# consensus-shipyard/ipc-filecoin-proofs

Measured on NVIDIA H100. Metric: receipts/sec scanned, higher is better.
Workload: dtype u8

## Files before the change

include/ipcfp.h:

```cpp
#ifndef IPCFP_H
#define IPCFP_H

#include <stdint.h>
#include <stddef.h>

#ifdef __cplusplus
extern "C" {
#endif

#define IPCFP_CID_LEN 38

typedef int32_t ipcfp_status;
enum {
    IPCFP_OK = 0,
    IPCFP_ERR_INVALID_ARG = -1,
    IPCFP_ERR_MISSING_BLOCK = -2,
    IPCFP_ERR_DECODE = -3,
    IPCFP_ERR_CID_MISMATCH = -4,
    IPCFP_ERR_MISSING_EXEC = -5,
    IPCFP_ERR_CUDA = -6,
    IPCFP_ERR_NCCL = -7,
    IPCFP_ERR_STATE_ROOT_MISMATCH = -8,
    IPCFP_ERR_ACTOR_NOT_FOUND = -9,
    IPCFP_ERR_NO_DEVICE = -10,
    IPCFP_ERR_UNSUPPORTED = -11
};

const char* ipcfp_last_error(void);
uint64_t ipcfp_last_error_index(void);
const char* ipcfp_version(void);
uint64_t ipcfp_kernel_launch_count(void);

ipcfp_status ipcfp_host_alloc(size_t bytes, void** out);
void ipcfp_host_free(void* p);

typedef struct ipcfp_store ipcfp_store;

#define IPCFP_STORE_VERIFY_CIDS 0x1u

ipcfp_status ipcfp_store_create(const uint8_t* cids, const uint64_t* offsets, const uint32_t* lengths,
                                const uint8_t* blob, uint64_t blob_size, uint64_t n_blocks,
                                int device, uint32_t flags, ipcfp_store** out);
void ipcfp_store_destroy(ipcfp_store* s);
uint64_t ipcfp_store_n_blocks(const ipcfp_store* s);
ipcfp_status ipcfp_store_get(ipcfp_store* s, const uint8_t cid[IPCFP_CID_LEN], uint8_t* buf, uint32_t cap,
                             uint32_t* len, int* found);
ipcfp_status ipcfp_store_has(ipcfp_store* s, const uint8_t cid[IPCFP_CID_LEN], int* found);
uint64_t ipcfp_store_first_bad_block(const ipcfp_store* s);

ipcfp_status ipcfp_blake2b256_batch(const uint8_t* blob, uint64_t blob_size, const uint64_t* offsets,
                                    const uint32_t* lengths, uint64_t n, int device, uint8_t* out );
ipcfp_status ipcfp_keccak256_batch(const uint8_t* blob, uint64_t blob_size, const uint64_t* offsets,
                                   const uint32_t* lengths, uint64_t n, int device, uint8_t* out );
ipcfp_status ipcfp_sha256_batch(const uint8_t* blob, uint64_t blob_size, const uint64_t* offsets,
                                const uint32_t* lengths, uint64_t n, int device, uint8_t* out );
ipcfp_status ipcfp_compute_mapping_slots(const uint8_t* keys32 , const uint64_t* slot_indices, uint64_t n,
                                         int device, uint8_t* out );

typedef struct ipcfp_tipset_desc {
    int64_t parent_epoch;
    int64_t child_epoch;
    uint32_t n_parents;
    const uint8_t* parent_cids;
    const uint8_t* parent_txmeta_cids;
    const uint8_t* child_cid;
    const uint8_t* receipts_root;
    const uint8_t* child_parent_state_root;
    uint64_t n_receipts;
    const uint8_t* events_roots;
    const uint8_t* has_events_root;
} ipcfp_tipset_desc;

typedef struct ipcfp_event_spec {
    const char* event_signature;
    const char* topic_1;
    uint8_t has_actor_id_filter;
    uint64_t actor_id_filter;
} ipcfp_event_spec;

#define IPCFP_LOG_FILTER_MAX_VALUES 65536u
#define IPCFP_LOG_FILTER_MAX_EMITTERS 65536u
typedef struct ipcfp_log_filter {
    uint64_t n_emitters;
    const uint64_t* emitters;
    uint32_t n_positions;
    uint32_t _pad;
    uint64_t n_values[4];
    const uint8_t* values[4];
} ipcfp_log_filter;

typedef struct ipcfp_storage_spec {
    uint64_t actor_id;
    uint8_t slot[32];
} ipcfp_storage_spec;

typedef struct ipcfp_witness {
    uint64_t n_blocks;
    const uint8_t* cids;
    const uint64_t* offsets;
    const uint32_t* lengths;
    const uint8_t* blob;
    uint64_t blob_size;
} ipcfp_witness;

typedef struct ipcfp_event_proof {
    uint64_t exec_index;
    uint64_t event_index;
    uint64_t emitter;
    uint32_t n_topics;
    uint32_t data_len;
    uint64_t data_off;
    uint64_t topics_off;
    uint8_t message_cid[IPCFP_CID_LEN];
    uint8_t _pad[2];
} ipcfp_event_proof;

typedef struct ipcfp_event_result {
    uint64_t n_matching;
    const uint64_t* matching_indices;
    uint64_t n_proofs;
    const ipcfp_event_proof* proofs;
    const uint8_t* data_blob;
    uint64_t data_blob_size;
    ipcfp_witness witness;
    uint64_t n_exec;
    float ms_total, ms_pass1, ms_pass2, ms_txamt, ms_witness;
    uint64_t pass1_bytes;
    uint64_t pass1_nodes;
    const void* shard_exec_dev;
    uint64_t shard_exec_count;
    uint64_t shard_raw_total;
    const void* union_cids_dev;
    uint64_t n_union_cids;
    const uint8_t* union_cids;
    uint64_t total_matching;
    uint64_t total_proofs;
    float ms_exchange, ms_fetch, ms_union;
    float _pad0;
    uint64_t union_part_first;
    uint64_t n_union_part;
    const char* json;
    uint64_t json_len;
    float ms_json;
    float _pad1;
} ipcfp_event_result;

typedef struct ipcfp_storage_proof {
    uint64_t actor_id;
    uint8_t actor_state_cid[IPCFP_CID_LEN];
    uint8_t storage_root[IPCFP_CID_LEN];
    uint8_t slot[32];
    uint8_t value[32];
    uint8_t found;
    uint8_t _pad[3];
    uint32_t raw_len;
} ipcfp_storage_proof;

typedef struct ipcfp_storage_result {
    uint64_t n_proofs;
    const ipcfp_storage_proof* proofs;
    ipcfp_witness witness;
    const uint64_t* spec_witness_offsets;
    const uint32_t* spec_witness_index;
    float ms_total;
} ipcfp_storage_result;

typedef struct ipcfp_slot_result {
    uint64_t n;
    const uint8_t* found;
    const uint32_t* raw_len;
    const uint8_t* values;
    ipcfp_witness witness;
    float ms_total;
    float ms_lookup;
    uint64_t lookup_nodes;
    uint64_t lookup_bytes;
} ipcfp_slot_result;

typedef struct ipcfp_bundle {
    ipcfp_storage_result* storage;
    uint64_t n_event_results;
    ipcfp_event_result** events;
    ipcfp_witness witness;
    const char* json;
// ... 191 lines not shown
```

integration/rust/ipcfp-sys/src/lib.rs:

```rust
#![allow(non_camel_case_types)]
use std::os::raw::{c_char, c_int, c_void};

pub const IPCFP_CID_LEN: usize = 38;
pub type ipcfp_status = i32;
pub const IPCFP_OK: ipcfp_status = 0;
pub const IPCFP_ERR_INVALID_ARG: ipcfp_status = -1;
pub const IPCFP_ERR_MISSING_BLOCK: ipcfp_status = -2;
pub const IPCFP_ERR_DECODE: ipcfp_status = -3;
pub const IPCFP_ERR_CID_MISMATCH: ipcfp_status = -4;
pub const IPCFP_ERR_MISSING_EXEC: ipcfp_status = -5;
pub const IPCFP_ERR_CUDA: ipcfp_status = -6;
pub const IPCFP_ERR_NCCL: ipcfp_status = -7;
pub const IPCFP_ERR_STATE_ROOT_MISMATCH: ipcfp_status = -8;
pub const IPCFP_ERR_ACTOR_NOT_FOUND: ipcfp_status = -9;
pub const IPCFP_ERR_NO_DEVICE: ipcfp_status = -10;
pub const IPCFP_ERR_UNSUPPORTED: ipcfp_status = -11;
pub const IPCFP_STORE_VERIFY_CIDS: u32 = 0x1;
pub const IPCFP_SCAN_SKIP_TX_AMTS: u32 = 0x1;
pub const IPCFP_SHARDED_UNION_TO_HOST: u32 = 0x2;
pub const IPCFP_SHARDED_UNION_FULL: u32 = 0x4;
pub const IPCFP_WITNESS_BY_REFERENCE: u32 = 0x8;
pub const IPCFP_RESULT_JSON: u32 = 0x10;
pub const IPCFP_COMM_ID_BYTES: usize = 128;

#[repr(C)] pub struct ipcfp_store { _p: [u8; 0] }
#[repr(C)] pub struct ipcfp_tipset { _p: [u8; 0] }
#[repr(C)] pub struct ipcfp_comm { _p: [u8; 0] }

#[repr(C)]
pub struct ipcfp_tipset_desc {
    pub parent_epoch: i64,
    pub child_epoch: i64,
    pub n_parents: u32,
    pub parent_cids: *const u8,
    pub parent_txmeta_cids: *const u8,
    pub child_cid: *const u8,
    pub receipts_root: *const u8,
    pub child_parent_state_root: *const u8,
    pub n_receipts: u64,
    pub events_roots: *const u8,
    pub has_events_root: *const u8,
}
#[repr(C)]
pub struct ipcfp_event_spec { pub event_signature: *const c_char, pub topic_1: *const c_char, pub has_actor_id_filter: u8, pub actor_id_filter: u64 }
pub const IPCFP_LOG_FILTER_MAX_VALUES: u32 = 65536;
pub const IPCFP_LOG_FILTER_MAX_EMITTERS: u32 = 65536;
#[repr(C)]
pub struct ipcfp_log_filter { pub n_emitters: u64, pub emitters: *const u64, pub n_positions: u32, pub _pad: u32, pub n_values: [u64; 4],
                              pub values: [*const u8; 4] }
#[repr(C)]
pub struct ipcfp_storage_spec { pub actor_id: u64, pub slot: [u8; 32] }
#[repr(C)]
pub struct ipcfp_witness { pub n_blocks: u64, pub cids: *const u8, pub offsets: *const u64, pub lengths: *const u32, pub blob: *const u8, pub blob_size: u64 }
#[repr(C)]
pub struct ipcfp_event_proof {
    pub exec_index: u64, pub event_index: u64, pub emitter: u64, pub n_topics: u32, pub data_len: u32,
    pub data_off: u64, pub topics_off: u64, pub message_cid: [u8; IPCFP_CID_LEN], pub _pad: [u8; 2],
}
#[repr(C)]
pub struct ipcfp_event_result {
    pub n_matching: u64, pub matching_indices: *const u64, pub n_proofs: u64, pub proofs: *const ipcfp_event_proof,
    pub data_blob: *const u8, pub data_blob_size: u64, pub witness: ipcfp_witness, pub n_exec: u64,
    pub ms_total: f32, pub ms_pass1: f32, pub ms_pass2: f32, pub ms_txamt: f32, pub ms_witness: f32,
    pub pass1_bytes: u64, pub pass1_nodes: u64,
    pub shard_exec_dev: *const c_void, pub shard_exec_count: u64, pub shard_raw_total: u64,
    pub union_cids_dev: *const c_void, pub n_union_cids: u64, pub union_cids: *const u8, pub total_matching: u64, pub total_proofs: u64,
    pub ms_exchange: f32, pub ms_fetch: f32, pub ms_union: f32, pub _pad0: f32,
    pub union_part_first: u64, pub n_union_part: u64,
    pub json: *const c_char, pub json_len: u64, pub ms_json: f32, pub _pad1: f32,
}
#[repr(C)]
pub struct ipcfp_storage_proof {
    pub actor_id: u64, pub actor_state_cid: [u8; IPCFP_CID_LEN], pub storage_root: [u8; IPCFP_CID_LEN],
    pub slot: [u8; 32], pub value: [u8; 32], pub found: u8, pub _pad: [u8; 3], pub raw_len: u32,
}
#[repr(C)]
pub struct ipcfp_storage_result {
    pub n_proofs: u64, pub proofs: *const ipcfp_storage_proof, pub witness: ipcfp_witness,
    pub spec_witness_offsets: *const u64, pub spec_witness_index: *const u32, pub ms_total: f32,
}
#[repr(C)]
pub struct ipcfp_slot_result { pub n: u64, pub found: *const u8, pub raw_len: *const u32, pub values: *const u8, pub witness: ipcfp_witness, pub ms_total: f32, pub ms_lookup: f32,
                                pub lookup_nodes: u64, pub lookup_bytes: u64 }
#[repr(C)]
pub struct ipcfp_parsed_bundle { pub tipset: ipcfp_tipset_desc, pub n_storage_proofs: u64, pub storage_proofs: *const ipcfp_storage_proof,
                                 pub n_event_proofs: u64, pub event_proofs: *const ipcfp_event_proof, pub data_blob: *const u8, pub data_blob_size: u64,
                                 pub witness: ipcfp_witness }
pub type ipcfp_trusted_parent_ts_fn = Option<unsafe extern "C" fn(ctx: *mut c_void, parent_epoch: i64, parent_cids: *const u8, n_parents: u32) -> c_int>;
pub type ipcfp_trusted_child_header_fn = Option<unsafe extern "C" fn(ctx: *mut c_void, child_epoch: i64, child_cid: *const u8) -> c_int>;
#[repr(C)]
pub struct ipcfp_bundle_verdict { pub tipset: ipcfp_tipset_desc, pub n_storage_proofs: u64, pub storage_proofs: *const ipcfp_storage_proof,
                                  pub storage_results: *const u8, pub n_event_proofs: u64, pub event_proofs: *const ipcfp_event_proof,
                                  pub event_results: *const u8, pub data_blob: *const u8, pub data_blob_size: u64, pub n_blocks: u64,
                                  pub witness_bytes: u64, pub parsed_on_device: u32, pub ms_total: f32, pub ms_parse: f32, pub ms_store: f32,
                                  pub ms_verify: f32, pub _pad: u32 }
#[repr(C)]
pub struct ipcfp_parsed_tipset { pub desc: ipcfp_tipset_desc }
#[repr(C)]
pub struct ipcfp_tipset_info { pub desc: ipcfp_tipset_desc, pub parsed_on_device: u32, pub ms_parse: f32, pub ms_kernels: f32,
                               pub _pad: u32 }
#[repr(C)]
pub struct ipcfp_parsed_blocks { pub blocks: ipcfp_witness }
#[repr(C)]
pub struct ipcfp_store_json_info { pub parsed_on_device: u32, pub ms_parse: f32, pub ms_kernels: f32, pub _pad: u32 }
#[repr(C)]
pub struct ipcfp_fetch_plan { pub n_missing: u64, pub cids: *const u8, pub n_needed: u64, pub n_levels: u32, pub ms_total: f32 }
pub const IPCFP_ADDRESS_MAX: usize = 65;
#[repr(C)]
#[derive(Clone, Copy)]
pub struct ipcfp_address { pub len: u8, pub bytes: [u8; IPCFP_ADDRESS_MAX] }
#[repr(C)]
pub struct ipcfp_resolve_result { pub n: u64, pub actor_ids: *const u64, pub status: *const ipcfp_status, pub init_status: ipcfp_status, pub _pad: u32,
                                  pub n_missing: u64, pub missing_cids: *const u8, pub witness: ipcfp_witness, pub ms_total: f32, pub ms_lookup: f32 }
#[repr(C)]
pub struct ipcfp_bundle { pub storage: *mut ipcfp_storage_result, pub n_event_results: u64, pub events: *mut *mut ipcfp_event_result, pub witness: ipcfp_witness,
                          pub json: *const c_char, pub json_len: u64, pub ms_total: f32, pub ms_json: f32 }

extern "C" {
    pub fn ipcfp_last_error() -> *const c_char;
    pub fn ipcfp_last_error_index() -> u64;
    pub fn ipcfp_version() -> *const c_char;
    pub fn ipcfp_kernel_launch_count() -> u64;
    pub fn ipcfp_host_alloc(bytes: usize, out: *mut *mut c_void) -> ipcfp_status;
    pub fn ipcfp_host_free(p: *mut c_void);

    pub fn ipcfp_store_create(cids: *const u8, offsets: *const u64, lengths: *const u32, blob: *const u8, blob_size: u64,
                              n_blocks: u64, device: c_int, flags: u32, out: *mut *mut ipcfp_store) -> ipcfp_status;
    pub fn ipcfp_store_destroy(s: *mut ipcfp_store);
    pub fn ipcfp_store_n_blocks(s: *const ipcfp_store) -> u64;
    pub fn ipcfp_store_get(s: *mut ipcfp_store, cid: *const u8, buf: *mut u8, cap: u32, len: *mut u32, found: *mut c_int) -> ipcfp_status;
    pub fn ipcfp_store_has(s: *mut ipcfp_store, cid: *const u8, found: *mut c_int) -> ipcfp_status;
    pub fn ipcfp_store_first_bad_block(s: *const ipcfp_store) -> u64;
    pub fn ipcfp_store_stream(s: *mut ipcfp_store) -> *mut c_void;

    pub fn ipcfp_blake2b256_batch(blob: *const u8, blob_size: u64, offsets: *const u64, lengths: *const u32, n: u64, device: c_int, out: *mut u8) -> ipcfp_status;
    pub fn ipcfp_keccak256_batch(blob: *const u8, blob_size: u64, offsets: *const u64, lengths: *const u32, n: u64, device: c_int, out: *mut u8) -> ipcfp_status;
    pub fn ipcfp_sha256_batch(blob: *const u8, blob_size: u64, offsets: *const u64, lengths: *const u32, n: u64, device: c_int, out: *mut u8) -> ipcfp_status;
    pub fn ipcfp_compute_mapping_slots(keys32: *const u8, slot_indices: *const u64, n: u64, device: c_int, out: *mut u8) -> ipcfp_status;

    pub fn ipcfp_generate_event_proof(s: *mut ipcfp_store, t: *const ipcfp_tipset_desc, spec: *const ipcfp_event_spec, flags: u32,
                                      out: *mut *mut ipcfp_event_result) -> ipcfp_status;
    pub fn ipcfp_event_result_free(r: *mut ipcfp_event_result);
    pub fn ipcfp_tipset_upload(s: *mut ipcfp_store, t: *const ipcfp_tipset_desc, out: *mut *mut ipcfp_tipset) -> ipcfp_status;
    pub fn ipcfp_tipset_free(t: *mut ipcfp_tipset);
    pub fn ipcfp_tipset_desc_from_json(parent: *const c_char, parent_len: u64, child: *const c_char, child_len: u64, receipts: *const c_char,
                                       receipts_len: u64, out: *mut *mut ipcfp_parsed_tipset) -> ipcfp_status;
    pub fn ipcfp_parsed_tipset_free(p: *mut ipcfp_parsed_tipset);
    pub fn ipcfp_tipset_upload_json(s: *mut ipcfp_store, parent: *const c_char, parent_len: u64, child: *const c_char, child_len: u64,
                                    receipts: *const c_char, receipts_len: u64, out: *mut *mut ipcfp_tipset) -> ipcfp_status;
    pub fn ipcfp_tipset_describe(t: *mut ipcfp_tipset, with_events_roots: c_int, out: *mut ipcfp_tipset_info) -> ipcfp_status;
    pub fn ipcfp_blocks_from_rpc_json(cids: *const u8, n_blocks: u64, texts: *const *const c_char, text_lens: *const u64, n_texts: u64,
                                      out: *mut *mut ipcfp_parsed_blocks) -> ipcfp_status;
    pub fn ipcfp_parsed_blocks_free(p: *mut ipcfp_parsed_blocks);
    pub fn ipcfp_store_create_rpc_json(cids: *const u8, n_blocks: u64, texts: *const *const c_char, text_lens: *const u64, n_texts: u64,
                                       device: c_int, flags: u32, out: *mut *mut ipcfp_store, info: *mut ipcfp_store_json_info) -> ipcfp_status;
    pub fn ipcfp_generate_event_proof_resident(s: *mut ipcfp_store, t: *mut ipcfp_tipset, spec: *const ipcfp_event_spec, flags: u32,
                                               out: *mut *mut ipcfp_event_result) -> ipcfp_status;
    pub fn ipcfp_generate_log_proof_resident(s: *mut ipcfp_store, t: *mut ipcfp_tipset, filter: *const ipcfp_log_filter, flags: u32,
                                             out: *mut *mut ipcfp_event_result) -> ipcfp_status;
    pub fn ipcfp_generate_log_proof(s: *mut ipcfp_store, t: *const ipcfp_tipset_desc, filter: *const ipcfp_log_filter, flags: u32,
                                    out: *mut *mut ipcfp_event_result) -> ipcfp_status;
    pub fn ipcfp_generate_event_proof_shard(s: *mut ipcfp_store, t: *const ipcfp_tipset_desc, spec: *const ipcfp_event_spec, lo: u64, hi: u64,
                                            world_size: u32, rank: u32, flags: u32, out: *mut *mut ipcfp_event_result) -> ipcfp_status;
    pub fn ipcfp_generate_event_proof_shard_resident(s: *mut ipcfp_store, t: *mut ipcfp_tipset, spec: *const ipcfp_event_spec, lo: u64, hi: u64,
                                                     world_size: u32, rank: u32, flags: u32, out: *mut *mut ipcfp_event_result) -> ipcfp_status;

    pub fn ipcfp_read_storage_slots(s: *mut ipcfp_store, contract_state_root: *const u8, slots: *const u8, k: u64, out: *mut *mut ipcfp_slot_result) -> ipcfp_status;
    pub fn ipcfp_slot_result_free(r: *mut ipcfp_slot_result);
    pub fn ipcfp_generate_storage_proofs(s: *mut ipcfp_store, t: *const ipcfp_tipset_desc, specs: *const ipcfp_storage_spec, n_specs: u64,
                                         out: *mut *mut ipcfp_storage_result) -> ipcfp_status;
    pub fn ipcfp_storage_result_free(r: *mut ipcfp_storage_result);
    pub fn ipcfp_generate_proof_bundle(s: *mut ipcfp_store, t: *const ipcfp_tipset_desc, sspecs: *const ipcfp_storage_spec, n_sspecs: u64,
                                       especs: *const ipcfp_event_spec, n_especs: u64, out: *mut *mut ipcfp_bundle) -> ipcfp_status;
    pub fn ipcfp_generate_proof_bundle_resident(s: *mut ipcfp_store, t: *mut ipcfp_tipset, sspecs: *const ipcfp_storage_spec, n_sspecs: u64,
                                                especs: *const ipcfp_event_spec, n_especs: u64, flags: u32, out: *mut *mut ipcfp_bundle) -> ipcfp_status;
    pub fn ipcfp_generate_log_bundle_resident(s: *mut ipcfp_store, t: *mut ipcfp_tipset, sspecs: *const ipcfp_storage_spec, n_sspecs: u64,
                                              filters: *const ipcfp_log_filter, n_filters: u64, flags: u32, out: *mut *mut ipcfp_bundle) -> ipcfp_status;
    pub fn ipcfp_generate_log_bundle(s: *mut ipcfp_store, t: *const ipcfp_tipset_desc, sspecs: *const ipcfp_storage_spec, n_sspecs: u64,
                                     filters: *const ipcfp_log_filter, n_filters: u64, flags: u32, out: *mut *mut ipcfp_bundle) -> ipcfp_status;
    pub fn ipcfp_bundle_free(b: *mut ipcfp_bundle);
    pub fn ipcfp_plan_fetch_resident(s: *mut ipcfp_store, t: *mut ipcfp_tipset, sspecs: *const ipcfp_storage_spec, n_sspecs: u64,
                                     especs: *const ipcfp_event_spec, n_especs: u64, flags: u32, out: *mut *mut ipcfp_fetch_plan) -> ipcfp_status;
    pub fn ipcfp_plan_fetch(s: *mut ipcfp_store, t: *const ipcfp_tipset_desc, sspecs: *const ipcfp_storage_spec, n_sspecs: u64,
                            especs: *const ipcfp_event_spec, n_especs: u64, flags: u32, out: *mut *mut ipcfp_fetch_plan) -> ipcfp_status;
    pub fn ipcfp_plan_fetch_log_resident(s: *mut ipcfp_store, t: *mut ipcfp_tipset, filter: *const ipcfp_log_filter, flags: u32,
                                         out: *mut *mut ipcfp_fetch_plan) -> ipcfp_status;
    pub fn ipcfp_plan_fetch_log_bundle_resident(s: *mut ipcfp_store, t: *mut ipcfp_tipset, sspecs: *const ipcfp_storage_spec, n_sspecs: u64,
                                                filters: *const ipcfp_log_filter, n_filters: u64, flags: u32, out: *mut *mut ipcfp_fetch_plan) -> ipcfp_status;
    pub fn ipcfp_fetch_plan_free(p: *mut ipcfp_fetch_plan);
    pub fn ipcfp_fetch_plan_to_rpc_json(p: *const ipcfp_fetch_plan, first_id: u64, out: *mut *mut c_char, out_len: *mut u64) -> ipcfp_status;
    pub fn ipcfp_resolve_addresses(s: *mut ipcfp_store, state_root: *const u8, addrs: *const ipcfp_address, n: u64,
                                   out: *mut *mut ipcfp_resolve_result) -> ipcfp_status;
    pub fn ipcfp_resolve_result_free(r: *mut ipcfp_resolve_result);
    pub fn ipcfp_address_parse(text: *const c_char, len: u64, out: *mut ipcfp_address) -> ipcfp_status;
    pub fn ipcfp_address_from_eth(eth: *const u8, out: *mut ipcfp_address) -> ipcfp_status;

    pub fn ipcfp_bundle_to_json(b: *const ipcfp_bundle, t: *const ipcfp_tipset_desc, out: *mut *mut c_char, out_len: *mut u64) -> ipcfp_status;
    pub fn ipcfp_event_result_to_json(r: *const ipcfp_event_result, t: *const ipcfp_tipset_desc, out: *mut *mut c_char, out_len: *mut u64) -> ipcfp_status;
    pub fn ipcfp_json_free(p: *mut c_char);
    pub fn ipcfp_bundle_from_json(json: *const c_char, len: u64, out: *mut *mut ipcfp_parsed_bundle) -> ipcfp_status;
    pub fn ipcfp_parsed_bundle_free(b: *mut ipcfp_parsed_bundle);
    pub fn ipcfp_verify_event_proofs(witness_store: *mut ipcfp_store, t: *const ipcfp_tipset_desc, proofs: *const ipcfp_event_proof, n_proofs: u64,
                                     data_blob: *const u8, data_blob_size: u64, filter: *const ipcfp_event_spec, results: *mut u8) -> ipcfp_status;
    pub fn ipcfp_verify_event_proofs_log(witness_store: *mut ipcfp_store, t: *const ipcfp_tipset_desc, proofs: *const ipcfp_event_proof, n_proofs: u64,
                                         data_blob: *const u8, data_blob_size: u64, filter: *const ipcfp_log_filter, results: *mut u8) -> ipcfp_status;
    pub fn ipcfp_verify_event_proofs_any(witness_store: *mut ipcfp_store, t: *const ipcfp_tipset_desc, proofs: *const ipcfp_event_proof, n_proofs: u64,
                                         data_blob: *const u8, data_blob_size: u64, filters: *const ipcfp_log_filter, n_filters: u64,
                                         results: *mut u8) -> ipcfp_status;
    pub fn ipcfp_verify_storage_proofs(witness_store: *mut ipcfp_store, t: *const ipcfp_tipset_desc, proofs: *const ipcfp_storage_proof, n_proofs: u64,
                                       results: *mut u8) -> ipcfp_status;
    pub fn ipcfp_verify_bundle_json(json: *const c_char, len: u64, device: c_int, trusted_parent: ipcfp_trusted_parent_ts_fn,
                                    trusted_child: ipcfp_trusted_child_header_fn, trust_ctx: *mut c_void, filter: *const ipcfp_event_spec,
                                    out: *mut *mut ipcfp_bundle_verdict) -> ipcfp_status;
    pub fn ipcfp_verify_bundle_json_any(json: *const c_char, len: u64, device: c_int, trusted_parent: ipcfp_trusted_parent_ts_fn,
                                        trusted_child: ipcfp_trusted_child_header_fn, trust_ctx: *mut c_void, filters: *const ipcfp_log_filter,
                                        n_filters: u64, out: *mut *mut ipcfp_bundle_verdict) -> ipcfp_status;
    pub fn ipcfp_bundle_verdict_free(v: *mut ipcfp_bundle_verdict);
    pub fn ipcfp_comm_unique_id(id: *mut u8) -> ipcfp_status;
    pub fn ipcfp_comm_init(id: *const u8, world_size: u32, rank: u32, device: c_int, out: *mut *mut ipcfp_comm) -> ipcfp_status;
    pub fn ipcfp_comm_destroy(c: *mut ipcfp_comm);
    pub fn ipcfp_generate_event_proof_sharded(c: *mut ipcfp_comm, s: *mut ipcfp_store, t: *mut ipcfp_tipset, spec: *const ipcfp_event_spec,
                                              bounds: *const u64, flags: u32, out: *mut *mut ipcfp_event_result) -> ipcfp_status;
}
```

ipc_filecoin_proofs_b200/api.py:

```python
import ctypes as C
import os
import subprocess
from dataclasses import dataclass
from typing import Optional

import numpy as np

from . import _abi as A

_HERE = os.path.dirname(os.path.abspath(__file__))
_ROOT = os.path.dirname(_HERE)
LIB_PATH = os.path.join(_HERE, "libipcfp.so")


def build_lib(force=False, jobs=8):
    if force or not os.path.exists(LIB_PATH):
        subprocess.check_call(["make", "-C", _ROOT, "-j%d" % jobs, os.path.relpath(LIB_PATH, _ROOT)])
    else:
        subprocess.check_call(["make", "-C", _ROOT, "-j%d" % jobs, "-s", os.path.relpath(LIB_PATH, _ROOT)])
    return LIB_PATH


_lib = None

EXPORTS = [
    "ipcfp_last_error", "ipcfp_last_error_index", "ipcfp_version", "ipcfp_kernel_launch_count", "ipcfp_host_alloc", "ipcfp_host_free",
    "ipcfp_store_create", "ipcfp_store_destroy", "ipcfp_store_n_blocks", "ipcfp_store_get", "ipcfp_store_has",
    "ipcfp_store_first_bad_block", "ipcfp_blake2b256_batch", "ipcfp_keccak256_batch", "ipcfp_sha256_batch",
    "ipcfp_compute_mapping_slots", "ipcfp_generate_event_proof", "ipcfp_event_result_free", "ipcfp_read_storage_slots",
    "ipcfp_slot_result_free", "ipcfp_generate_storage_proofs", "ipcfp_storage_result_free", "ipcfp_generate_proof_bundle",
    "ipcfp_bundle_free", "ipcfp_generate_event_proof_shard",
    "ipcfp_tipset_upload", "ipcfp_tipset_free", "ipcfp_generate_event_proof_resident", "ipcfp_generate_event_proof_shard_resident",
    "ipcfp_store_stream",
    "ipcfp_comm_unique_id", "ipcfp_comm_init", "ipcfp_comm_destroy", "ipcfp_generate_event_proof_sharded",
    "ipcfp_verify_event_proofs", "ipcfp_verify_storage_proofs", "ipcfp_bundle_to_json", "ipcfp_event_result_to_json", "ipcfp_json_free",
    "ipcfp_bundle_from_json", "ipcfp_parsed_bundle_free", "ipcfp_verify_bundle_json", "ipcfp_bundle_verdict_free",
    "ipcfp_generate_proof_bundle_resident", "ipcfp_tipset_desc_from_json", "ipcfp_parsed_tipset_free", "ipcfp_tipset_upload_json",
    "ipcfp_tipset_describe", "ipcfp_blocks_from_rpc_json", "ipcfp_parsed_blocks_free", "ipcfp_store_create_rpc_json",
    "ipcfp_plan_fetch_resident", "ipcfp_plan_fetch", "ipcfp_fetch_plan_free", "ipcfp_fetch_plan_to_rpc_json",
    "ipcfp_resolve_addresses", "ipcfp_resolve_result_free", "ipcfp_address_parse", "ipcfp_address_from_eth",
    "ipcfp_generate_log_proof", "ipcfp_generate_log_proof_resident", "ipcfp_plan_fetch_log_resident", "ipcfp_verify_event_proofs_log",
    "ipcfp_generate_log_bundle", "ipcfp_generate_log_bundle_resident", "ipcfp_plan_fetch_log_bundle_resident", "ipcfp_verify_event_proofs_any",
    "ipcfp_verify_bundle_json_any",
]


def lib():
    global _lib
    if _lib is None:
        if not os.path.exists(LIB_PATH):
            raise RuntimeError(f"{LIB_PATH} is missing: run `make` (or __graft_entry__.build()). There is no CPU fallback.")
        L = C.CDLL(LIB_PATH)
        L.ipcfp_last_error.restype = C.c_char_p
        L.ipcfp_last_error_index.restype = C.c_uint64
        L.ipcfp_version.restype = C.c_char_p
        L.ipcfp_kernel_launch_count.restype = C.c_uint64
        L.ipcfp_host_alloc.restype = C.c_int32
        L.ipcfp_host_alloc.argtypes = [C.c_size_t, C.POINTER(C.c_void_p)]
        L.ipcfp_host_free.argtypes = [C.c_void_p]
        L.ipcfp_store_create.restype = C.c_int32
        L.ipcfp_store_create.argtypes = [C.c_void_p, C.c_void_p, C.c_void_p, C.c_void_p, C.c_uint64, C.c_uint64, C.c_int, C.c_uint32,
                                         C.POINTER(C.c_void_p)]
        L.ipcfp_store_destroy.argtypes = [C.c_void_p]
        L.ipcfp_store_n_blocks.restype = C.c_uint64
        L.ipcfp_store_n_blocks.argtypes = [C.c_void_p]
        L.ipcfp_store_first_bad_block.restype = C.c_uint64
        L.ipcfp_store_first_bad_block.argtypes = [C.c_void_p]
        L.ipcfp_store_get.restype = C.c_int32
        L.ipcfp_store_get.argtypes = [C.c_void_p, C.c_void_p, C.c_void_p, C.c_uint32, C.POINTER(C.c_uint32), C.POINTER(C.c_int)]
        L.ipcfp_store_has.restype = C.c_int32
        L.ipcfp_store_has.argtypes = [C.c_void_p, C.c_void_p, C.POINTER(C.c_int)]
        for name in ("ipcfp_blake2b256_batch", "ipcfp_keccak256_batch", "ipcfp_sha256_batch"):
            f = getattr(L, name)
            f.restype = C.c_int32
            f.argtypes = [C.c_void_p, C.c_uint64, C.c_void_p, C.c_void_p, C.c_uint64, C.c_int, C.c_void_p]
        L.ipcfp_compute_mapping_slots.restype = C.c_int32
        L.ipcfp_compute_mapping_slots.argtypes = [C.c_void_p, C.c_void_p, C.c_uint64, C.c_int, C.c_void_p]
        L.ipcfp_generate_event_proof.restype = C.c_int32
        L.ipcfp_generate_event_proof.argtypes = [C.c_void_p, C.POINTER(A.TipsetDesc), C.POINTER(A.EventSpec), C.c_uint32,
                                                 C.POINTER(C.POINTER(A.EventResultC))]
        L.ipcfp_generate_event_proof_shard.restype = C.c_int32
        L.ipcfp_generate_event_proof_shard.argtypes = [C.c_void_p, C.POINTER(A.TipsetDesc), C.POINTER(A.EventSpec), C.c_uint64, C.c_uint64,
                                                       C.c_uint32, C.c_uint32, C.c_uint32, C.POINTER(C.POINTER(A.EventResultC))]
        L.ipcfp_event_result_free.argtypes = [C.POINTER(A.EventResultC)]
        L.ipcfp_read_storage_slots.restype = C.c_int32
        L.ipcfp_read_storage_slots.argtypes = [C.c_void_p, C.c_void_p, C.c_void_p, C.c_uint64, C.POINTER(C.POINTER(A.SlotResultC))]
        L.ipcfp_slot_result_free.argtypes = [C.POINTER(A.SlotResultC)]
        L.ipcfp_generate_storage_proofs.restype = C.c_int32
        L.ipcfp_generate_storage_proofs.argtypes = [C.c_void_p, C.POINTER(A.TipsetDesc), C.c_void_p, C.c_uint64,
                                                    C.POINTER(C.POINTER(A.StorageResultC))]
        L.ipcfp_storage_result_free.argtypes = [C.POINTER(A.StorageResultC)]
        L.ipcfp_generate_proof_bundle.restype = C.c_int32
        L.ipcfp_generate_proof_bundle.argtypes = [C.c_void_p, C.POINTER(A.TipsetDesc), C.c_void_p, C.c_uint64, C.c_void_p, C.c_uint64,
                                                  C.POINTER(C.POINTER(A.BundleC))]
        L.ipcfp_generate_proof_bundle_resident.restype = C.c_int32
        L.ipcfp_generate_proof_bundle_resident.argtypes = [C.c_void_p, C.c_void_p, C.c_void_p, C.c_uint64, C.c_void_p, C.c_uint64, C.c_uint32,
                                                           C.POINTER(C.POINTER(A.BundleC))]
        L.ipcfp_bundle_free.argtypes = [C.POINTER(A.BundleC)]
        L.ipcfp_tipset_upload.restype = C.c_int32
        L.ipcfp_tipset_upload.argtypes = [C.c_void_p, C.POINTER(A.TipsetDesc), C.POINTER(C.c_void_p)]
        L.ipcfp_tipset_free.argtypes = [C.c_void_p]
        L.ipcfp_generate_event_proof_resident.restype = C.c_int32
        L.ipcfp_generate_event_proof_resident.argtypes = [C.c_void_p, C.c_void_p, C.POINTER(A.EventSpec), C.c_uint32,
                                                          C.POINTER(C.POINTER(A.EventResultC))]
        L.ipcfp_generate_event_proof_shard_resident.restype = C.c_int32
        L.ipcfp_generate_event_proof_shard_resident.argtypes = [C.c_void_p, C.c_void_p, C.POINTER(A.EventSpec), C.c_uint64, C.c_uint64,
                                                                C.c_uint32, C.c_uint32, C.c_uint32, C.POINTER(C.POINTER(A.EventResultC))]
        L.ipcfp_store_stream.restype = C.c_void_p
        L.ipcfp_store_stream.argtypes = [C.c_void_p]
        L.ipcfp_comm_unique_id.restype = C.c_int32
        L.ipcfp_comm_unique_id.argtypes = [C.c_void_p]
        L.ipcfp_comm_init.restype = C.c_int32
        L.ipcfp_comm_init.argtypes = [C.c_void_p, C.c_uint32, C.c_uint32, C.c_int, C.POINTER(C.c_void_p)]
        L.ipcfp_comm_destroy.argtypes = [C.c_void_p]
        L.ipcfp_generate_event_proof_sharded.restype = C.c_int32
        L.ipcfp_generate_event_proof_sharded.argtypes = [C.c_void_p, C.c_void_p, C.c_void_p, C.POINTER(A.EventSpec), C.c_void_p, C.c_uint32,
                                                         C.POINTER(C.POINTER(A.EventResultC))]
        L.ipcfp_verify_event_proofs.restype = C.c_int32
        L.ipcfp_verify_event_proofs.argtypes = [C.c_void_p, C.POINTER(A.TipsetDesc), C.c_void_p, C.c_uint64, C.c_void_p, C.c_uint64, C.c_void_p, C.c_void_p]
        L.ipcfp_generate_log_proof.restype = C.c_int32
        L.ipcfp_generate_log_proof.argtypes = [C.c_void_p, C.POINTER(A.TipsetDesc), C.POINTER(A.LogFilterC), C.c_uint32,
                                               C.POINTER(C.POINTER(A.EventResultC))]
        L.ipcfp_generate_log_proof_resident.restype = C.c_int32
        L.ipcfp_generate_log_proof_resident.argtypes = [C.c_void_p, C.c_void_p, C.POINTER(A.LogFilterC), C.c_uint32,
                                                        C.POINTER(C.POINTER(A.EventResultC))]
        L.ipcfp_plan_fetch_log_resident.restype = C.c_int32
        L.ipcfp_plan_fetch_log_resident.argtypes = [C.c_void_p, C.c_void_p, C.POINTER(A.LogFilterC), C.c_uint32, C.POINTER(C.POINTER(A.FetchPlanC))]
        L.ipcfp_verify_event_proofs_log.restype = C.c_int32
        L.ipcfp_verify_event_proofs_log.argtypes = [C.c_void_p, C.POINTER(A.TipsetDesc), C.c_void_p, C.c_uint64, C.c_void_p, C.c_uint64,
                                                    C.POINTER(A.LogFilterC), C.c_void_p]
        L.ipcfp_generate_log_bundle.restype = C.c_int32
        L.ipcfp_generate_log_bundle.argtypes = [C.c_void_p, C.POINTER(A.TipsetDesc), C.c_void_p, C.c_uint64, C.POINTER(A.LogFilterC), C.c_uint64,
                                                C.c_uint32, C.POINTER(C.POINTER(A.BundleC))]
        L.ipcfp_generate_log_bundle_resident.restype = C.c_int32
        L.ipcfp_generate_log_bundle_resident.argtypes = [C.c_void_p, C.c_void_p, C.c_void_p, C.c_uint64, C.POINTER(A.LogFilterC), C.c_uint64,
                                                         C.c_uint32, C.POINTER(C.POINTER(A.BundleC))]
        L.ipcfp_plan_fetch_log_bundle_resident.restype = C.c_int32
        L.ipcfp_plan_fetch_log_bundle_resident.argtypes = [C.c_void_p, C.c_void_p, C.c_void_p, C.c_uint64, C.POINTER(A.LogFilterC), C.c_uint64,
                                                           C.c_uint32, C.POINTER(C.POINTER(A.FetchPlanC))]
        L.ipcfp_verify_event_proofs_any.restype = C.c_int32
        L.ipcfp_verify_event_proofs_any.argtypes = [C.c_void_p, C.POINTER(A.TipsetDesc), C.c_void_p, C.c_uint64, C.c_void_p, C.c_uint64,
                                                    C.POINTER(A.LogFilterC), C.c_uint64, C.c_void_p]
        L.ipcfp_verify_bundle_json_any.restype = C.c_int32
        L.ipcfp_verify_bundle_json_any.argtypes = [C.c_char_p, C.c_uint64, C.c_int, A.TrustedParentFn, A.TrustedChildFn, C.c_void_p,
                                                   C.POINTER(A.LogFilterC), C.c_uint64, C.POINTER(C.POINTER(A.BundleVerdictC))]
        L.ipcfp_verify_storage_proofs.restype = C.c_int32
        L.ipcfp_verify_storage_proofs.argtypes = [C.c_void_p, C.POINTER(A.TipsetDesc), C.c_void_p, C.c_uint64, C.c_void_p]
        for name in ("ipcfp_bundle_to_json", "ipcfp_event_result_to_json"):
            f = getattr(L, name)
            f.restype = C.c_int32
            f.argtypes = [C.c_void_p, C.POINTER(A.TipsetDesc), C.POINTER(C.c_void_p), C.POINTER(C.c_uint64)]
        L.ipcfp_json_free.argtypes = [C.c_void_p]
        L.ipcfp_bundle_from_json.restype = C.c_int32
        L.ipcfp_bundle_from_json.argtypes = [C.c_char_p, C.c_uint64, C.POINTER(C.POINTER(A.ParsedBundleC))]
        L.ipcfp_parsed_bundle_free.argtypes = [C.POINTER(A.ParsedBundleC)]
        L.ipcfp_verify_bundle_json.restype = C.c_int32
        L.ipcfp_verify_bundle_json.argtypes = [C.c_char_p, C.c_uint64, C.c_int, A.TrustedParentFn, A.TrustedChildFn, C.c_void_p, C.c_void_p,
                                               C.POINTER(C.POINTER(A.BundleVerdictC))]
        L.ipcfp_bundle_verdict_free.argtypes = [C.POINTER(A.BundleVerdictC)]
        L.ipcfp_tipset_desc_from_json.restype = C.c_int32
        L.ipcfp_tipset_desc_from_json.argtypes = [C.c_char_p, C.c_uint64, C.c_char_p, C.c_uint64, C.c_char_p, C.c_uint64,
                                                  C.POINTER(C.POINTER(A.ParsedTipsetC))]
        L.ipcfp_parsed_tipset_free.argtypes = [C.POINTER(A.ParsedTipsetC)]
        L.ipcfp_tipset_upload_json.restype = C.c_int32
        L.ipcfp_tipset_upload_json.argtypes = [C.c_void_p, C.c_char_p, C.c_uint64, C.c_char_p, C.c_uint64, C.c_char_p, C.c_uint64,
                                               C.POINTER(C.c_void_p)]
        L.ipcfp_tipset_describe.restype = C.c_int32
        L.ipcfp_tipset_describe.argtypes = [C.c_void_p, C.c_int, C.POINTER(A.TipsetInfoC)]
        L.ipcfp_blocks_from_rpc_json.restype = C.c_int32
        L.ipcfp_blocks_from_rpc_json.argtypes = [C.c_void_p, C.c_uint64, C.POINTER(C.c_char_p), C.POINTER(C.c_uint64), C.c_uint64,
                                                 C.POINTER(C.POINTER(A.ParsedBlocksC))]
        L.ipcfp_parsed_blocks_free.argtypes = [C.POINTER(A.ParsedBlocksC)]
        L.ipcfp_store_create_rpc_json.restype = C.c_int32
        L.ipcfp_store_create_rpc_json.argtypes = [C.c_void_p, C.c_uint64, C.POINTER(C.c_char_p), C.POINTER(C.c_uint64), C.c_uint64, C.c_int,
                                                  C.c_uint32, C.POINTER(C.c_void_p), C.POINTER(A.StoreJsonInfoC)]
        L.ipcfp_plan_fetch_resident.restype = C.c_int32
        L.ipcfp_plan_fetch_resident.argtypes = [C.c_void_p, C.c_void_p, C.c_void_p, C.c_uint64, C.c_void_p, C.c_uint64, C.c_uint32,
                                                C.POINTER(C.POINTER(A.FetchPlanC))]
        L.ipcfp_plan_fetch.restype = C.c_int32
        L.ipcfp_plan_fetch.argtypes = [C.c_void_p, C.POINTER(A.TipsetDesc), C.c_void_p, C.c_uint64, C.c_void_p, C.c_uint64, C.c_uint32,
                                       C.POINTER(C.POINTER(A.FetchPlanC))]
        L.ipcfp_fetch_plan_free.argtypes = [C.POINTER(A.FetchPlanC)]
        L.ipcfp_fetch_plan_to_rpc_json.restype = C.c_int32
        L.ipcfp_fetch_plan_to_rpc_json.argtypes = [C.POINTER(A.FetchPlanC), C.c_uint64, C.POINTER(C.c_void_p), C.POINTER(C.c_uint64)]
        L.ipcfp_resolve_addresses.restype = C.c_int32
        L.ipcfp_resolve_addresses.argtypes = [C.c_void_p, C.c_void_p, C.POINTER(A.AddressC), C.c_uint64, C.POINTER(C.POINTER(A.ResolveResultC))]
        L.ipcfp_resolve_result_free.argtypes = [C.POINTER(A.ResolveResultC)]
        L.ipcfp_address_parse.restype = C.c_int32
        L.ipcfp_address_parse.argtypes = [C.c_char_p, C.c_uint64, C.POINTER(A.AddressC)]
        L.ipcfp_address_from_eth.restype = C.c_int32
        L.ipcfp_address_from_eth.argtypes = [C.c_void_p, C.POINTER(A.AddressC)]
        _lib = L
    return _lib


def _u8(x):
    if isinstance(x, (bytes, bytearray, memoryview)):
        return np.frombuffer(bytes(x), dtype=np.uint8).copy()
    return np.ascontiguousarray(x, dtype=np.uint8)


def _check(st):
    if st != A.OK:
        L = lib()
        raise A.IpcfpError(st, L.ipcfp_last_error().decode(errors="replace"), L.ipcfp_last_error_index())


def kernel_launch_count():
    return int(lib().ipcfp_kernel_launch_count())


@dataclass
class EventProofSpec:
    event_signature: str
    topic_1: str
    actor_id_filter: Optional[int] = None

    def as_c(self):
        return A.make_event_spec(self.event_signature, self.topic_1, self.actor_id_filter)


def _topic32(v):
    if isinstance(v, str):
        v = bytes.fromhex(v[2:] if v[:2] in ("0x", "0X") else v)
    v = bytes(v)
    if len(v) != 32:
        raise ValueError(f"a topic value is 32 bytes, got {len(v)}")
    return v


class LogFilter:

    def __init__(self, emitters=None, topics=()):
        topics = list(topics)
        if len(topics) > 4:
            raise ValueError("a log filter has at most 4 topic positions")
        self.emitters = [int(e) for e in (emitters or [])]
        self.topics = []
        for t in topics:
            if t is None or (isinstance(t, (list, tuple)) and not t):
                self.topics.append(None)
            elif isinstance(t, (bytes, bytearray, str)):
                self.topics.append([_topic32(t)])
            else:
                self.topics.append([_topic32(v) for v in t])

    @classmethod
    def from_spec(cls, spec, device=0):
        t1 = spec.topic_1.encode()[:32]
        t0 = bytes(keccak256_batch([spec.event_signature.encode()], device)[0])
        return cls(None if spec.actor_id_filter is None else [spec.actor_id_filter], [t0, t1 + bytes(32 - len(t1))])

    def as_c(self):
        f = A.LogFilterC()
        keep = []
        em = np.ascontiguousarray(self.emitters, dtype=np.uint64)
        keep.append(em)
        f.n_emitters = len(em)
        f.emitters = em.ctypes.data if em.size else None
        f.n_positions = len(self.topics)
        for k, vals in enumerate(self.topics):
            if vals:
                a = np.frombuffer(b"".join(vals), dtype=np.uint8).copy()
                keep.append(a)
                f.n_values[k] = len(vals)
                f.values[k] = a.ctypes.data
        return f, keep

    def matches(self, emitter, topics):
        if self.emitters and emitter not in self.emitters:
            return False
        if len(topics) < len(self.topics):
            return False
        return all(vals is None or bytes(topics[k]) in vals for k, vals in enumerate(self.topics))


def _log_filters_c(log_filters):
    cs, keep = [], []
    for f in log_filters:
        c, k = f.as_c()
        cs.append(c)
        keep.append(k)
    return (A.LogFilterC * max(len(cs), 1))(*cs), len(cs), keep


@dataclass
class StorageProofSpec:
    actor_id: int
    slot: bytes


class PinnedArray:

    def __init__(self, nbytes):
        p = C.c_void_p()
        _check(lib().ipcfp_host_alloc(max(int(nbytes), 1), C.byref(p)))
        self._p = p
        self.array = np.frombuffer((C.c_uint8 * max(int(nbytes), 1)).from_address(p.value), dtype=np.uint8)[:int(nbytes)]

    def free(self):
        if self._p:
            self.array = None
            lib().ipcfp_host_free(self._p)
            self._p = None

    def __del__(self):
        try:
            self.free()
        except Exception:
            pass


class BlockStore:

    def __init__(self, cids, offsets, lengths, blob, device=0, verify_cids=False):
        cids = np.ascontiguousarray(cids, dtype=np.uint8)
        offsets = np.ascontiguousarray(offsets, dtype=np.uint64)
        lengths = np.ascontiguousarray(lengths, dtype=np.uint32)
        blob = np.ascontiguousarray(blob, dtype=np.uint8)
        self.n_blocks = len(lengths)
        self.device = device
        h = C.c_void_p()
        st = lib().ipcfp_store_create(cids.ctypes.data if cids.size else None, offsets.ctypes.data if offsets.size else None,
                                      lengths.ctypes.data if lengths.size else None, blob.ctypes.data if blob.size else None, blob.size,
                                      self.n_blocks, device, A.STORE_VERIFY_CIDS if verify_cids else 0, C.byref(h))
        self._h = h
        if st != A.OK:
            bad = lib().ipcfp_store_first_bad_block(h) if h else None
            msg, idx = lib().ipcfp_last_error().decode(errors="replace"), lib().ipcfp_last_error_index()
            if h:
                lib().ipcfp_store_destroy(h)
                self._h = None
            e = A.IpcfpError(st, msg, idx)
            e.first_bad_block = bad
            raise e

    @classmethod
    def from_tipset(cls, ts, device=0, verify_cids=False):
        return cls(ts.cids, ts.offsets, ts.lengths, ts.blob, device, verify_cids)

    @classmethod
    def from_rpc_json(cls, cids, texts, device=0, verify_cids=False):
        cids = np.ascontiguousarray(cids, dtype=np.uint8).reshape(-1, A.CID_LEN)
        arr, lens, keep = _text_array(texts)
        self = cls.__new__(cls)
        self.n_blocks, self.device, self._h = len(cids), device, None
        h, info = C.c_void_p(), A.StoreJsonInfoC()
        st = lib().ipcfp_store_create_rpc_json(cids.ctypes.data if cids.size else None, len(cids), arr, lens, len(keep), device,
                                               A.STORE_VERIFY_CIDS if verify_cids else 0, C.byref(h), C.byref(info))
        self._h = h
        self.json_info = A.StoreJsonInfoPy(bool(info.parsed_on_device), float(info.ms_parse), float(info.ms_kernels))
        if st != A.OK:
            bad = lib().ipcfp_store_first_bad_block(h) if h else None
            msg, idx = lib().ipcfp_last_error().decode(errors="replace"), lib().ipcfp_last_error_index()
            self.close()
            e = A.IpcfpError(st, msg, idx)
            e.first_bad_block = bad
            raise e
        return self

    def get(self, cid):
        cid = _u8(cid)
        ln = C.c_uint32()
        found = C.c_int()
# ... 565 lines not shown
```

ipc_filecoin_proofs_b200/csrc/capi.cu:

```cuda
#include <atomic>
#include <cstring>

#include "engine.cuh"
#include "log_filter.cuh"

namespace ipcfp {

static thread_local std::string g_last_error;
static thread_local uint64_t g_last_index = UINT64_MAX;
static std::atomic<uint64_t> g_launches{0};

void note_launch() { g_launches.fetch_add(1, std::memory_order_relaxed); }
void set_last_error(const std::string& msg, uint64_t index) { g_last_error = msg; g_last_index = index; }

template <class F> static ipcfp_status guard(F f) {
    g_last_error.clear();
    g_last_index = UINT64_MAX;
    try { f(); return IPCFP_OK; }
    catch (const Error& e) { g_last_error = e.msg; g_last_index = e.index; return e.status; }
    catch (const std::bad_alloc&) { g_last_error = "out of host memory"; return IPCFP_ERR_INVALID_ARG; }
    catch (const std::exception& e) { g_last_error = e.what(); return IPCFP_ERR_INVALID_ARG; }
}

struct BundleBox {
    ipcfp_bundle r;
    std::vector<ipcfp_event_result*> ev;
    WitnessOut wit;
    PinnedArray json;
    ~BundleBox() {
        if (r.storage) storage_result_free(r.storage);
        for (auto* e : ev) event_result_free(e);
    }
};
struct TimingEvent {
    cudaEvent_t e = nullptr;
    TimingEvent() { IPCFP_CUDA(cudaEventCreate(&e)); }
    ~TimingEvent() { if (e) cudaEventDestroy(e); }
};

struct FetchPlanBox {
    ipcfp_fetch_plan r;
    FetchPlan plan;
    void fill() {
        r.n_missing = plan.cids.size() / 38;
        r.cids = plan.cids.data();
        r.n_needed = plan.n_needed;
        r.n_levels = plan.n_levels;
        r.ms_total = plan.ms_total;
    }
};

#define IPCFP_BUNDLE_FLAGS (IPCFP_WITNESS_BY_REFERENCE | IPCFP_RESULT_JSON)

template <class Check, class Gen>
static ipcfp_bundle* generate_proof_bundle(Store* st, TipsetDev& td, const ipcfp_storage_spec* sspecs, uint64_t n_sspecs, uint64_t n_events,
                                           uint32_t flags, Check check, Gen gen) {
    if (flags & ~(uint32_t)IPCFP_BUNDLE_FLAGS) throw Error(IPCFP_ERR_INVALID_ARG, "unknown flag bit for a proof bundle");
    if (n_sspecs && !sspecs) throw Error(IPCFP_ERR_INVALID_ARG, "null specs");
    check();
    if ((flags & IPCFP_WITNESS_BY_REFERENCE) && !st->caller_blob)
        throw Error(IPCFP_ERR_UNSUPPORTED, "IPCFP_WITNESS_BY_REFERENCE needs a store made from a caller's blob (ipcfp_store_create)");
    st->use();
    const bool by_ref = (flags & IPCFP_WITNESS_BY_REFERENCE) != 0;
    cudaStream_t stream = st->stream;
    TimingEvent t0, t1, j0, j1;
    IPCFP_CUDA(cudaEventRecord(t0.e, stream));
    std::unique_ptr<BundleBox> box(new BundleBox());
    memset(&box->r, 0, sizeof box->r);
    std::vector<const WitnessOut*> lists;
    if (n_sspecs) {
        if (!td.has_state_root) throw Error(IPCFP_ERR_INVALID_ARG, "tipset descriptor lacks child_cid / parent_state_root");
        box->r.storage = generate_storage_proofs(st, td.child_cid, td.child_state_root, sspecs, n_sspecs, by_ref);
        lists.push_back(&storage_result_witness(box->r.storage));
    }
    for (uint64_t i = 0; i < n_events; i++) {
        box->ev.push_back(gen(i));
        lists.push_back(&event_result_witness(box->ev.back()));
    }
    witness_union(st, lists, box->wit, by_ref);

    if (flags & IPCFP_RESULT_JSON) {
        IPCFP_CUDA(cudaEventRecord(j0.e, stream));
        const uint64_t ns = box->r.storage ? box->r.storage->n_proofs : 0;
        uint64_t np = 0, nb = 0;
        for (auto* e : box->ev) { np += e->n_proofs; nb += e->data_blob_size; }
        auto up16 = [](uint64_t x) { return (x + 15) & ~15ull; };
        const uint64_t o_ev = up16(ns * sizeof(ipcfp_storage_proof)), o_blob = o_ev + up16(np * sizeof(ipcfp_event_proof)),
                       o_cids = o_blob + up16(nb + 16), size = o_cids + 38ull * (2 + td.n_parents);
        PinnedArray stage(st->pool, size);
        uint8_t* h = stage.as<uint8_t>();
        if (ns) memcpy(h, box->r.storage->proofs, ns * sizeof(ipcfp_storage_proof));
        ipcfp_event_proof* hp = (ipcfp_event_proof*)(h + o_ev);
        uint64_t k = 0, base = 0;
        for (auto* e : box->ev) {
            for (uint64_t q = 0; q < e->n_proofs; q++, k++) {
                hp[k] = e->proofs[q];
                hp[k].data_off += base;
                hp[k].topics_off += base;
            }
            if (e->data_blob_size) memcpy(h + o_blob + base, e->data_blob, e->data_blob_size);
            base += e->data_blob_size;
        }
        memcpy(h + o_cids, td.child_cid, 38);
        memcpy(h + o_cids + 38, td.child_state_root, 38);
        if (td.n_parents) memcpy(h + o_cids + 76, td.parent_cids.data(), 38ull * td.n_parents);
        AsyncBuf<uint8_t> d(size, stream);
        IPCFP_CUDA(cudaMemcpyAsync(d.p, h, size, cudaMemcpyHostToDevice, stream));
        UnifiedJsonInputs ji{(const ipcfp_storage_proof*)d.p, ns, (const ipcfp_event_proof*)(d.p + o_ev), np, d.p + o_blob,
                             box->wit.cids_dev.p, box->wit.idx_dev.p, box->wit.n, td.parent_epoch, td.child_epoch, td.n_parents,
                             d.p + o_cids + 76, d.p + o_cids, d.p + o_cids + 38};
        box->r.json_len = render_unified_json(st, ji, box->json);
        IPCFP_CUDA(cudaEventRecord(j1.e, stream));
    }
    IPCFP_CUDA(cudaEventRecord(t1.e, stream));
    IPCFP_CUDA(cudaStreamSynchronize(stream));
    box->r.n_event_results = box->ev.size();
    box->r.events = box->ev.data();
    box->wit.fill(box->r.witness);
    float ms;
    IPCFP_CUDA(cudaEventElapsedTime(&ms, t0.e, t1.e)); box->r.ms_total = ms;
    if (flags & IPCFP_RESULT_JSON) {
        box->r.json = box->json.as<char>();
        IPCFP_CUDA(cudaEventElapsedTime(&ms, j0.e, j1.e)); box->r.ms_json = ms;
    }
    return &box.release()->r;
}

static ipcfp_bundle* generate_proof_bundle(Store* st, TipsetDev& td, const ipcfp_storage_spec* sspecs, uint64_t n_sspecs,
                                           const ipcfp_event_spec* especs, uint64_t n_especs, uint32_t flags) {
    return generate_proof_bundle(
        st, td, sspecs, n_sspecs, n_especs, flags,
        [&] { if (n_especs && !especs) throw Error(IPCFP_ERR_INVALID_ARG, "null specs"); },
        [&](uint64_t i) { return generate_event_proof(st, td, &especs[i], flags & IPCFP_WITNESS_BY_REFERENCE, false, 0, 0); });
}
static ipcfp_bundle* generate_log_bundle(Store* st, TipsetDev& td, const ipcfp_storage_spec* sspecs, uint64_t n_sspecs,
                                         const ipcfp_log_filter* filters, uint64_t n_filters, uint32_t flags) {
    return generate_proof_bundle(
        st, td, sspecs, n_sspecs, n_filters, flags, [&] { LogFilterSet::check(filters, n_filters); },
        [&](uint64_t k) { return generate_log_proof(st, td, &filters[k], flags & IPCFP_WITNESS_BY_REFERENCE); });
}

}

using namespace ipcfp;

struct ipcfp_store { Store s; };

extern "C" {

const char* ipcfp_last_error(void) { return g_last_error.c_str(); }
uint64_t ipcfp_last_error_index(void) { return g_last_index; }
const char* ipcfp_version(void) {
    return "ipcfp-b200 0.2 (sm_90a): k_verify_cids k_hash_batch k_build_index sort_by_cid k_pass1_stage k_pass2 k_amt_dense k_amt_expand k_dedup "
           "k_storage_proofs k_read_slots k_verify_events k_verify_storage k_scan k_witness_copy k_witness_emit k_union_mark k_json_* k_jp_* k_rj_* k_rb_* | sharded: k_xb_* k_exec_claim_seg "
           "k_exec_mark_dups k_select_positions k_fetch_positions k_part_pack k_merge_* (NCCL via dlopen)";
}
uint64_t ipcfp_kernel_launch_count(void) { return g_launches.load(); }

ipcfp_status ipcfp_host_alloc(size_t bytes, void** out) {
    return guard([&] {
        if (!out) throw Error(IPCFP_ERR_INVALID_ARG, "null out");
        int cnt = 0;
        if (cudaGetDeviceCount(&cnt) != cudaSuccess || cnt == 0) { cudaGetLastError(); throw Error(IPCFP_ERR_NO_DEVICE, "no CUDA device"); }
        int dev = 0;
        if (cudaGetDevice(&dev) != cudaSuccess) { cudaGetLastError(); dev = 0; }
        NumaPrefer numa(dev);
        IPCFP_CUDA(cudaMallocHost(out, bytes ? bytes : 1));
    });
}
void ipcfp_host_free(void* p) { if (p) cudaFreeHost(p); }

ipcfp_status ipcfp_store_create(const uint8_t* cids, const uint64_t* offsets, const uint32_t* lengths, const uint8_t* blob, uint64_t blob_size,
                                uint64_t n_blocks, int device, uint32_t flags, ipcfp_store** out) {
    return guard([&] {
        if (!out) throw Error(IPCFP_ERR_INVALID_ARG, "null out");
        *out = nullptr;
        Store* s = store_create(cids, offsets, lengths, blob, blob_size, n_blocks, device, flags);
        *out = reinterpret_cast<ipcfp_store*>(s);
        if (s->first_bad != UINT64_MAX) throw Error(IPCFP_ERR_CID_MISMATCH, "blake2b-256(block) != CID digest", s->first_bad);
    });
}
ipcfp_status ipcfp_store_create_rpc_json(const uint8_t* cids, uint64_t n_blocks, const char* const* texts, const uint64_t* text_lens, uint64_t n_texts,
                                         int device, uint32_t flags, ipcfp_store** out, ipcfp_store_json_info* info) {
    return guard([&] {
        if (!out) throw Error(IPCFP_ERR_INVALID_ARG, "null out");
        *out = nullptr;
        ipcfp_store_json_info si;
        Store* s = store_create_rpc_json(cids, n_blocks, texts, text_lens, n_texts, device, flags, si);
        *out = reinterpret_cast<ipcfp_store*>(s);
        if (info) *info = si;
        if (s->first_bad != UINT64_MAX) throw Error(IPCFP_ERR_CID_MISMATCH, "blake2b-256(block) != CID digest", s->first_bad);
    });
}
void ipcfp_store_destroy(ipcfp_store* s) { delete reinterpret_cast<Store*>(s); }
uint64_t ipcfp_store_n_blocks(const ipcfp_store* s) { return s ? reinterpret_cast<const Store*>(s)->n : 0; }
uint64_t ipcfp_store_first_bad_block(const ipcfp_store* s) { return s ? reinterpret_cast<const Store*>(s)->first_bad : UINT64_MAX; }
ipcfp_status ipcfp_store_get(ipcfp_store* s, const uint8_t cid[IPCFP_CID_LEN], uint8_t* buf, uint32_t cap, uint32_t* len, int* found) {
    return guard([&] {
        if (!s || !cid || !found) throw Error(IPCFP_ERR_INVALID_ARG, "null argument");
        store_get(reinterpret_cast<Store*>(s), cid, buf, cap, len, found);
    });
}
ipcfp_status ipcfp_store_has(ipcfp_store* s, const uint8_t cid[IPCFP_CID_LEN], int* found) {
    return guard([&] {
        if (!s || !cid || !found) throw Error(IPCFP_ERR_INVALID_ARG, "null argument");
        uint32_t len;
        store_get(reinterpret_cast<Store*>(s), cid, nullptr, 0, &len, found);
    });
}

ipcfp_status ipcfp_blake2b256_batch(const uint8_t* blob, uint64_t blob_size, const uint64_t* offsets, const uint32_t* lengths, uint64_t n, int device,
                                    uint8_t* out) {
    return guard([&] { hash_batch(0, blob, blob_size, offsets, lengths, n, device, out); });
}
ipcfp_status ipcfp_keccak256_batch(const uint8_t* blob, uint64_t blob_size, const uint64_t* offsets, const uint32_t* lengths, uint64_t n, int device,
                                   uint8_t* out) {
    return guard([&] { hash_batch(1, blob, blob_size, offsets, lengths, n, device, out); });
}
ipcfp_status ipcfp_sha256_batch(const uint8_t* blob, uint64_t blob_size, const uint64_t* offsets, const uint32_t* lengths, uint64_t n, int device,
                                uint8_t* out) {
    return guard([&] { hash_batch(2, blob, blob_size, offsets, lengths, n, device, out); });
}
ipcfp_status ipcfp_compute_mapping_slots(const uint8_t* keys32, const uint64_t* slot_indices, uint64_t n, int device, uint8_t* out) {
    return guard([&] { mapping_slots(keys32, slot_indices, n, device, out); });
}

ipcfp_status ipcfp_generate_event_proof(ipcfp_store* s, const ipcfp_tipset_desc* t, const ipcfp_event_spec* spec, uint32_t flags,
                                        ipcfp_event_result** out) {
    return guard([&] {
        if (!s || !out) throw Error(IPCFP_ERR_INVALID_ARG, "null argument");
        *out = nullptr;
        Store* st = reinterpret_cast<Store*>(s);
        TipsetDev td;
        tipset_upload(st, t, td);
        *out = generate_event_proof(st, td, spec, flags, false, 0, 0);
    });
}
ipcfp_status ipcfp_generate_event_proof_shard(ipcfp_store* s, const ipcfp_tipset_desc* t, const ipcfp_event_spec* spec, uint64_t lo, uint64_t hi,
                                              uint32_t world_size, uint32_t rank, uint32_t flags, ipcfp_event_result** out) {
    return guard([&] {
        if (!s || !out) throw Error(IPCFP_ERR_INVALID_ARG, "null argument");
        *out = nullptr;
        Store* st = reinterpret_cast<Store*>(s);
        TipsetDev td;
        tipset_upload(st, t, td);
        *out = generate_event_proof(st, td, spec, flags, true, lo, hi);
    });
}
void ipcfp_event_result_free(ipcfp_event_result* r) { if (r) event_result_free(r); }

ipcfp_status ipcfp_tipset_upload(ipcfp_store* s, const ipcfp_tipset_desc* t, ipcfp_tipset** out) {
    return guard([&] {
        if (!s || !out) throw Error(IPCFP_ERR_INVALID_ARG, "null argument");
        *out = nullptr;
        Store* st = reinterpret_cast<Store*>(s);
        std::unique_ptr<TipsetDev> td(new TipsetDev());
        tipset_upload(st, t, *td);
        IPCFP_CUDA(cudaStreamSynchronize(st->stream));
        *out = reinterpret_cast<ipcfp_tipset*>(td.release());
    });
}
void ipcfp_tipset_free(ipcfp_tipset* t) { delete reinterpret_cast<TipsetDev*>(t); }
ipcfp_status ipcfp_tipset_upload_json(ipcfp_store* s, const char* parent, uint64_t parent_len, const char* child, uint64_t child_len,
                                      const char* receipts, uint64_t receipts_len, ipcfp_tipset** out) {
    return guard([&] {
        if (!s || !out) throw Error(IPCFP_ERR_INVALID_ARG, "null argument");
        *out = nullptr;
        Store* st = reinterpret_cast<Store*>(s);
        std::unique_ptr<TipsetDev> td(new TipsetDev());
        tipset_upload_json(st, parent, parent_len, child, child_len, receipts, receipts_len, *td);
        IPCFP_CUDA(cudaStreamSynchronize(st->stream));
        *out = reinterpret_cast<ipcfp_tipset*>(td.release());
    });
}
ipcfp_status ipcfp_tipset_describe(ipcfp_tipset* t, int with_events_roots, ipcfp_tipset_info* out) {
    return guard([&] {
        if (!t || !out) throw Error(IPCFP_ERR_INVALID_ARG, "null argument");
        tipset_describe(*reinterpret_cast<TipsetDev*>(t), with_events_roots != 0, out);
    });
}
ipcfp_status ipcfp_generate_event_proof_resident(ipcfp_store* s, ipcfp_tipset* t, const ipcfp_event_spec* spec, uint32_t flags,
                                                 ipcfp_event_result** out) {
    return guard([&] {
        if (!s || !t || !out) throw Error(IPCFP_ERR_INVALID_ARG, "null argument");
        *out = nullptr;
        *out = generate_event_proof(reinterpret_cast<Store*>(s), *reinterpret_cast<TipsetDev*>(t), spec, flags, false, 0, 0);
    });
}
ipcfp_status ipcfp_generate_event_proof_shard_resident(ipcfp_store* s, ipcfp_tipset* t, const ipcfp_event_spec* spec, uint64_t lo, uint64_t hi,
                                                       uint32_t world_size, uint32_t rank, uint32_t flags, ipcfp_event_result** out) {
    return guard([&] {
        if (!s || !t || !out) throw Error(IPCFP_ERR_INVALID_ARG, "null argument");
        *out = nullptr;
        *out = generate_event_proof(reinterpret_cast<Store*>(s), *reinterpret_cast<TipsetDev*>(t), spec, flags, true, lo, hi);
    });
}
ipcfp_status ipcfp_generate_log_proof_resident(ipcfp_store* s, ipcfp_tipset* t, const ipcfp_log_filter* filter, uint32_t flags,
                                               ipcfp_event_result** out) {
    return guard([&] {
        if (!s || !t || !out) throw Error(IPCFP_ERR_INVALID_ARG, "null argument");
        *out = nullptr;
        *out = generate_log_proof(reinterpret_cast<Store*>(s), *reinterpret_cast<TipsetDev*>(t), filter, flags);
    });
}
ipcfp_status ipcfp_generate_log_proof(ipcfp_store* s, const ipcfp_tipset_desc* t, const ipcfp_log_filter* filter, uint32_t flags,
                                      ipcfp_event_result** out) {
    return guard([&] {
        if (!s || !out) throw Error(IPCFP_ERR_INVALID_ARG, "null argument");
        *out = nullptr;
        Store* st = reinterpret_cast<Store*>(s);
// ... 243 lines not shown
```

ipc_filecoin_proofs_b200/csrc/common.cuh:

```cuda
#pragma once
#include <cuda_runtime.h>
#include <stdint.h>
#include <string>
#include <vector>

#include "../../include/ipcfp.h"

namespace ipcfp {

struct Error {
    ipcfp_status status;
    std::string msg;
    uint64_t index;
    Error(ipcfp_status s, std::string m, uint64_t i = UINT64_MAX) : status(s), msg(std::move(m)), index(i) {}
};
void note_launch();

#define IPCFP_CUDA(expr)                                                                                          \
    do {                                                                                                          \
        cudaError_t _e = (expr);                                                                                  \
        if (_e != cudaSuccess)                                                                                    \
            throw ::ipcfp::Error(IPCFP_ERR_CUDA, std::string(#expr) + ": " + cudaGetErrorString(_e));             \
    } while (0)

#define IPCFP_LAUNCH_CHECK()                                                   \
    do {                                                                       \
        ::ipcfp::note_launch();                                                \
        IPCFP_CUDA(cudaGetLastError());                                        \
    } while (0)

static inline unsigned div_up(uint64_t a, uint64_t b) { return (unsigned)((a + b - 1) / b); }

void* dev_pool_take(size_t bytes, size_t* cap_out);
void dev_pool_give(void* p, size_t cap);

template <class T> struct DevBuf {
    T* p = nullptr;
    size_t n = 0;
    size_t pool_cap = 0;
    DevBuf() {}
    explicit DevBuf(size_t count) { alloc(count); }
    DevBuf(const DevBuf&) = delete;
    DevBuf& operator=(const DevBuf&) = delete;
    DevBuf(DevBuf&& o) noexcept : p(o.p), n(o.n), pool_cap(o.pool_cap) { o.p = nullptr; o.n = 0; o.pool_cap = 0; }
    DevBuf& operator=(DevBuf&& o) noexcept { if (this != &o) { release(); p = o.p; n = o.n; pool_cap = o.pool_cap; o.p = nullptr; o.n = 0; o.pool_cap = 0; } return *this; }
    ~DevBuf() { release(); }
    void alloc(size_t count) {
        release();
        n = count;
        if (count) IPCFP_CUDA(cudaMalloc((void**)&p, count * sizeof(T)));
    }
    void alloc_pooled(size_t count) {
        release();
        n = count;
        if (count) p = (T*)dev_pool_take(count * sizeof(T), &pool_cap);
    }
    void ensure(size_t count) { if (count > n) alloc(count); }
    void release() {
        if (p) { if (pool_cap) dev_pool_give(p, pool_cap); else cudaFree(p); }
        p = nullptr; n = 0; pool_cap = 0;
    }
    size_t bytes() const { return n * sizeof(T); }
};

template <class T> struct AsyncBuf {
    T* p = nullptr;
    size_t n = 0;
    cudaStream_t st = nullptr;
    AsyncBuf() {}
    AsyncBuf(size_t count, cudaStream_t s) { alloc(count, s); }
    AsyncBuf(const AsyncBuf&) = delete;
    AsyncBuf& operator=(const AsyncBuf&) = delete;
    AsyncBuf(AsyncBuf&& o) noexcept : p(o.p), n(o.n), st(o.st) { o.p = nullptr; o.n = 0; }
    AsyncBuf& operator=(AsyncBuf&& o) noexcept { if (this != &o) { release(); p = o.p; n = o.n; st = o.st; o.p = nullptr; o.n = 0; } return *this; }
    ~AsyncBuf() { release(); }
    void alloc(size_t count, cudaStream_t s) {
        release();
        st = s;
        n = count;
        if (count) IPCFP_CUDA(cudaMallocAsync((void**)&p, count * sizeof(T), s));
    }
    void release() { if (p) cudaFreeAsync(p, st); p = nullptr; n = 0; }
    void zero() { if (p) IPCFP_CUDA(cudaMemsetAsync(p, 0, n * sizeof(T), st)); }
};

template <class T> struct PinnedBuf {
    T* p = nullptr;
    T* dev = nullptr;
    size_t n = 0;
    PinnedBuf() {}
    explicit PinnedBuf(size_t count) { alloc(count); }
    PinnedBuf(const PinnedBuf&) = delete;
    PinnedBuf& operator=(const PinnedBuf&) = delete;
    ~PinnedBuf() { if (p) cudaFreeHost(p); }
    void alloc(size_t count) {
        if (p) cudaFreeHost(p);
        p = nullptr; dev = nullptr; n = count;
        if (count) {
            IPCFP_CUDA(cudaHostAlloc((void**)&p, count * sizeof(T), cudaHostAllocMapped));
            IPCFP_CUDA(cudaHostGetDevicePointer((void**)&dev, p, 0));
        }
    }
    void ensure(size_t count) { if (count > n) alloc(count); }
    void swap(PinnedBuf& o) { std::swap(p, o.p); std::swap(dev, o.dev); std::swap(n, o.n); }
};

enum Stage : uint32_t {
    ST_TXMETA = 1, ST_TXAMT = 2, ST_RECEIPTS_ROOT = 3, ST_PASS1 = 4, ST_PASS2 = 5, ST_WITNESS = 6,
    ST_STORAGE = 7, ST_INGEST = 8
};
enum DevCode : uint32_t { DC_MISSING = 1, DC_DECODE = 2, DC_MISSING_EXEC = 3, DC_STATE_MISMATCH = 4, DC_ACTOR_NOT_FOUND = 5, DC_UNSUPPORTED = 6, DC_CID_MISMATCH = 7 };

#define IPCFP_NO_ERROR 0xFFFFFFFFFFFFFFFFull

__host__ __device__ static inline uint64_t err_key(uint32_t stage, uint64_t index, uint32_t code, uint32_t detail) {
    return ((uint64_t)stage << 56) | ((index & 0xFFFFFFFFFFull) << 16) | ((uint64_t)(code & 0xff) << 8) | (detail & 0xff);
}
#define IPCFP_TX_EIDX_NONE 0xffu
__host__ __device__ static inline uint64_t tx_err_key(uint32_t eidx, uint64_t base, uint32_t level, uint32_t code, uint32_t detail) {
    const uint64_t b = base > 0xFFFFFFFFFFFull ? 0xFFFFFFFFFFFull : base;
    return ((uint64_t)(eidx & 0xff) << 56) | (b << 12) | ((uint64_t)(31u - (level > 31u ? 31u : level)) << 7) | ((uint64_t)(code & 7) << 4) | (detail & 15);
}
#ifdef __CUDACC__
__device__ static inline void report_error(unsigned long long* word, uint32_t stage, uint64_t index, uint32_t code, uint32_t detail) {
    atomicMin(word, (unsigned long long)err_key(stage, index, code, detail));
}
__device__ static inline void report_tx_error(unsigned long long* word, uint32_t eidx, uint64_t base, uint32_t level, uint32_t code, uint32_t detail) {
    atomicMin(word, (unsigned long long)tx_err_key(eidx, base, level, code, detail));
}
#endif

struct Digest { uint64_t w[4]; };

#ifdef __CUDACC__
__device__ __forceinline__ bool digest_eq(const Digest& a, const Digest& b) {
    return a.w[0] == b.w[0] && a.w[1] == b.w[1] && a.w[2] == b.w[2] && a.w[3] == b.w[3];
}
__device__ __forceinline__ uint64_t mix64(uint64_t x) {
    x ^= x >> 33; x *= 0xff51afd7ed558ccdULL; x ^= x >> 33; x *= 0xc4ceb9fe1a85ec53ULL; x ^= x >> 33;
    return x;
}
__device__ __forceinline__ uint64_t digest_hash(const Digest& d, uint32_t cls) { return mix64(d.w[0] ^ (d.w[2] * 0x9E3779B97F4A7C15ULL) ^ cls); }
__device__ __forceinline__ uint64_t load_u64_le(const uint8_t* p) {
    uint64_t v = 0;
#pragma unroll
    for (int i = 0; i < 8; i++) v |= (uint64_t)p[i] << (8 * i);
    return v;
}
__device__ __forceinline__ uint64_t load_u64_any(const uint8_t* q) {
    uintptr_t a = (uintptr_t)q;
    const uint64_t* b = (const uint64_t*)(a & ~(uintptr_t)7);
    uint32_t s = (uint32_t)(a & 7) * 8;
    uint64_t x0 = b[0], x1 = b[1];
    return (x0 >> s) | ((x1 << 1) << (63 - s));
}
__device__ __forceinline__ void win_load(const uint8_t* q, uint64_t& w0, uint64_t& w1) {
    uintptr_t a = (uintptr_t)q;
    const uint2* b = (const uint2*)(a & ~(uintptr_t)7);
    uint32_t s = (uint32_t)(a & 7) * 8;
    uint2 x0 = b[0], x1 = b[1], x2 = b[2];
    bool up = (s & 32) != 0;
    uint32_t c0 = up ? x0.y : x0.x, c1 = up ? x1.x : x0.y, c2 = up ? x1.y : x1.x, c3 = up ? x2.x : x1.y, c4 = up ? x2.y : x2.x;
    w0 = (uint64_t)__funnelshift_r(c0, c1, s) | ((uint64_t)__funnelshift_r(c1, c2, s) << 32);
    w1 = (uint64_t)__funnelshift_r(c2, c3, s) | ((uint64_t)__funnelshift_r(c3, c4, s) << 32);
}
__device__ __forceinline__ Digest load_digest(const uint8_t* p) {
    uintptr_t a = (uintptr_t)p;
    const uint64_t* b = (const uint64_t*)(a & ~(uintptr_t)7);
    uint32_t s = (uint32_t)(a & 7) * 8;
    uint64_t x0 = b[0], x1 = b[1], x2 = b[2], x3 = b[3], x4 = b[4];
    Digest d;
    d.w[0] = (x0 >> s) | ((x1 << 1) << (63 - s)); d.w[1] = (x1 >> s) | ((x2 << 1) << (63 - s));
    d.w[2] = (x2 >> s) | ((x3 << 1) << (63 - s)); d.w[3] = (x3 >> s) | ((x4 << 1) << (63 - s));
    return d;
}
__device__ __forceinline__ void prefetch_l2(const void* p) { asm volatile("prefetch.global.L2 [%0];" ::"l"(p)); }
#endif

}
```

ipc_filecoin_proofs_b200/csrc/engine.cuh:

```cuda
#pragma once
#include <array>
#include <memory>
#include <mutex>
#include <string>
#include <vector>

#include "common.cuh"
#include "store.cuh"
#include "rawcid.cuh"

namespace ipcfp {

struct NumaPrefer {
    bool on = false;
    int old_mode = 0;
    unsigned long old_mask[16] = {};
    explicit NumaPrefer(int device);
    ~NumaPrefer();
};

struct PinnedPool {
    struct Buf { void* p; size_t cap; };
    std::mutex mu;
    std::vector<Buf> free_list;
    ~PinnedPool();
    void* take(size_t bytes, size_t* cap_out);
    void give(void* p, size_t cap);
};
struct PinnedArray {
    std::shared_ptr<PinnedPool> pool;
    void* p = nullptr;
    size_t cap = 0;
    PinnedArray() {}
    PinnedArray(std::shared_ptr<PinnedPool> pl, size_t bytes) : pool(std::move(pl)) { p = pool->take(bytes ? bytes : 16, &cap); }
    PinnedArray(const PinnedArray&) = delete;
    PinnedArray& operator=(const PinnedArray&) = delete;
    PinnedArray(PinnedArray&& o) noexcept : pool(std::move(o.pool)), p(o.p), cap(o.cap) { o.p = nullptr; }
    PinnedArray& operator=(PinnedArray&& o) noexcept { release(); pool = std::move(o.pool); p = o.p; cap = o.cap; o.p = nullptr; return *this; }
    ~PinnedArray() { release(); }
    void release() { if (p && pool) pool->give(p, cap); p = nullptr; }
    template <class T> T* as() const { return (T*)p; }
};

enum DevWord : uint32_t {
    DW_ERR = 0,
    DW_FRONTIER_A = 1, DW_FRONTIER_B = 2,
    DW_UNKNOWN_CLASSES = 1,
    DW_FIRST_BAD = 2,
    DW_N_EXEC = 3,
    DW_STATS = 4,
    DW_N_MATCH = 6,
    DW_N_PROOFS = 7,
    DW_WIT_A = 8, DW_WIT_A_BYTES = 9,
    DW_WIT_B = 10, DW_WIT_B_BYTES = 11,
    DW_BLOB_BYTES = 12,
    DW_LEVEL_TOTAL = 13,
    DW_DENSE_FAIL = 14,
    DW_TX_ERR = 15,
    DW_SPLIT_IDX = 16, DW_SPLIT_BYTES = 17,
    DW_UNION_SIZE = 18,
    DW_EXEC_CHECK = 19,
    DW_JSON_TOTAL0 = 24, DW_JSON_TOTAL1 = 25, DW_JSON_OVERFLOW = 26, DW_JSON_TOTAL2 = 27,
    DW_COUNT = 64
};
constexpr uint32_t MAX_WORLD = 255;
constexpr uint32_t HW_PROLOGUE_WORDS = 230;
constexpr uint32_t HW_JSON_TOTALS_WORDS = DW_JSON_TOTAL2 - DW_JSON_TOTAL0 + 1;
constexpr uint32_t HW_ANY_SKIP_WORDS = 2;
constexpr uint32_t HW_PARKED_KEY_WORDS = 1;
constexpr uint32_t HW_EXCHANGE_WORDS = 2;
constexpr uint32_t HW_UNION_PARTS_WORDS = 2 * MAX_WORLD;
constexpr uint32_t HW_JP_META_WORDS = 17;
constexpr uint32_t HW_RJ_META_WORDS = 2;
constexpr uint32_t HW_RB_META_WORDS = 4;
enum HostWord : uint32_t {
    HW_PROLOGUE = DW_COUNT,
    HW_JSON_TOTALS = HW_PROLOGUE + HW_PROLOGUE_WORDS,
    HW_ANY_SKIP = HW_JSON_TOTALS + HW_JSON_TOTALS_WORDS,
    HW_PARKED_KEY = HW_ANY_SKIP + HW_ANY_SKIP_WORDS,
    HW_EXCH_OVERFLOW = HW_PARKED_KEY + HW_PARKED_KEY_WORDS, HW_EXCH_N_EXEC = HW_EXCH_OVERFLOW + 1,
    HW_UNION_PARTS = HW_EXCH_OVERFLOW + HW_EXCHANGE_WORDS,
    HW_JP_META = HW_UNION_PARTS + HW_UNION_PARTS_WORDS,
    HW_RJ_META = HW_JP_META + HW_JP_META_WORDS,
    HW_RB_META = HW_RJ_META + HW_RJ_META_WORDS,
    HW_END = HW_RB_META + HW_RB_META_WORDS
};
constexpr uint32_t HW_COUNT = 1024;
static_assert(DW_JSON_TOTAL2 < DW_COUNT, "a mirrored slot never reaches a host-only region (they start at DW_COUNT)");
static_assert(HW_EXCH_N_EXEC < HW_UNION_PARTS, "the exchange words fit their region");
static_assert(HW_END <= HW_COUNT, "the host-only regions fit the mapped words");
enum StoreEvent : uint32_t {
    EV_BEGIN = 0,
    EV_SETUP = 1, EV_STORAGE_END = 1,
    EV_EXEC_ORDER = 2, EV_LOOKUP_BEGIN = 2,
    EV_PASS1 = 3, EV_LOOKUP_END = 3,
    EV_PASS2 = 4,
    EV_END = 5,
    EV_WITNESS_SORTED = 6,
    EV_BLOB_COPIED = 7,
    EV_GATHER_B = 8,
    EV_RAW_LIST = 9,
    EV_JSON_BEGIN = 10, EV_JSON_END = 11,
    EV_COUNT = 12
};

struct Store {
    int device = 0;
    cudaStream_t stream = nullptr, stream2 = nullptr;
    unsigned walk_grid = 0;
    uint64_t n = 0, blob_size = 0;
    DevBuf<uint8_t> arena;
    DevBuf<uint64_t> offsets;
    DevBuf<uint32_t> lengths;
    DevBuf<Digest> digests;
    DevBuf<uint8_t> cls;
    DevBuf<uint64_t> table;
    DevBuf<BlockRec> recs;
    DevBuf<uint32_t> rank_of, block_at_rank;
    StoreView view{};
    DevBuf<StoreView> view_dev;
    std::vector<std::array<uint8_t, 6>> class_prefix;
    std::vector<uint32_t> class_rank;
    uint64_t first_bad = UINT64_MAX;
    bool caller_blob = true;
    std::shared_ptr<PinnedPool> pool;
    DevBuf<unsigned long long> dev_words;
    PinnedBuf<uint64_t> host_words;
    PinnedArray stage;
    cudaEvent_t ev[EV_COUNT] = {};
    ~Store();
    void use() const { IPCFP_CUDA(cudaSetDevice(device)); }
};

struct TipsetDev {
    int64_t parent_epoch = 0, child_epoch = 0;
    uint32_t n_parents = 0;
    std::vector<uint8_t> parent_cids, txmeta_cids;
    uint8_t child_cid[38] = {}, receipts_root[38] = {}, child_state_root[38] = {};
    bool has_state_root = false;
    uint64_t n_receipts = 0;
    DevBuf<uint8_t> events_roots;
    DevBuf<uint8_t> has_root;
    int device = 0;
    bool parsed_on_device = false;
    float ms_parse = 0.f, ms_kernels = 0.f;
    std::vector<uint8_t> host_roots, host_has;
};

struct ScopedStatus;
struct Comm;

void set_last_error(const std::string& msg, uint64_t index);
ipcfp_status status_from_devcode(uint32_t code);

Store* store_create(const uint8_t* cids, const uint64_t* offsets, const uint32_t* lengths, const uint8_t* blob, uint64_t blob_size,
                    uint64_t n, int device, uint32_t flags);
void store_get(Store* s, const uint8_t* cid, uint8_t* buf, uint32_t cap, uint32_t* len, int* found);
void hash_batch(int which, const uint8_t* blob, uint64_t blob_size, const uint64_t* offsets, const uint32_t* lengths, uint64_t n, int device,
                uint8_t* out);
void mapping_slots(const uint8_t* keys32, const uint64_t* slot_indices, uint64_t n, int device, uint8_t* out);
void check_device(int device);
Store* store_shell(int device);
void store_alloc_blocks(Store* s, uint64_t n, uint64_t blob_size, DevBuf<uint8_t>& cids_dev);
void store_index(Store* s, const uint8_t* cids_dev, const uint8_t* cids_host, const uint8_t* first_prefix, DevBuf<uint8_t>& sort_ws);
void store_verify_all(Store* s);
Store* store_create_rpc_json(const uint8_t* cids, uint64_t n_blocks, const char* const* texts, const uint64_t* text_lens, uint64_t n_texts, int device,
                             uint32_t flags, ipcfp_store_json_info& info);
void publish_words(Store* s, uint32_t dst_first, uint32_t n_words, const void* src_dev = nullptr, cudaStream_t stream = nullptr);

void tipset_upload(Store* s, const ipcfp_tipset_desc* t, TipsetDev& td);
void tipset_upload_json(Store* s, const char* parent, uint64_t parent_len, const char* child, uint64_t child_len, const char* receipts,
                        uint64_t receipts_len, TipsetDev& td);
void tipset_describe(TipsetDev& td, bool with_roots, ipcfp_tipset_info* out);
struct ExecOrderOut {
    uint64_t n_exec = 0, nraw = 0;
    AsyncBuf<RawCid> exec_raw;
    AsyncBuf<uint32_t> exec_idx;
};
ipcfp_event_result* generate_event_proof(Store* s, TipsetDev& td, const ipcfp_event_spec* spec, uint32_t flags, bool sharded, uint64_t lo, uint64_t hi,
                                         Comm* comm = nullptr, ExecOrderOut* exo = nullptr);
ipcfp_event_result* generate_log_proof(Store* s, TipsetDev& td, const ipcfp_log_filter* filter, uint32_t flags);
void verify_event_proofs(Store* s, const ipcfp_tipset_desc* t, const ipcfp_event_proof* proofs, uint64_t n, const uint8_t* data_blob, uint64_t blob_size,
                         const ipcfp_event_spec* filter, uint8_t* results, const ipcfp_log_filter* log_filters = nullptr, uint64_t n_log_filters = 0);
void verify_storage_proofs(Store* s, const ipcfp_tipset_desc* t, const ipcfp_storage_proof* proofs, uint64_t n, uint8_t* results);
void verify_event_proofs_dev(Store* s, const ipcfp_tipset_desc* t, const ipcfp_event_proof* d_proofs, uint64_t n, const uint8_t* d_blob, uint64_t blob_size,
                             const ipcfp_event_spec* filter, uint8_t* results, const ipcfp_log_filter* log_filters = nullptr, uint64_t n_log_filters = 0);
void verify_storage_proofs_dev(Store* s, const ipcfp_tipset_desc* t, const ipcfp_storage_proof* d_proofs, uint64_t n, uint8_t* results);
ipcfp_bundle_verdict* verify_bundle_json(const char* json, uint64_t len, int device, ipcfp_trusted_parent_ts_fn trusted_parent,
                                         ipcfp_trusted_child_header_fn trusted_child, void* trust_ctx, const ipcfp_event_spec* filter,
                                         const ipcfp_log_filter* log_filters = nullptr, uint64_t n_log_filters = 0);
void bundle_verdict_free(ipcfp_bundle_verdict* v);
void event_result_free(ipcfp_event_result* r);
struct WitnessOut;
const WitnessOut& event_result_witness(const ipcfp_event_result* r);
struct FetchPlan {
    std::vector<uint8_t> cids;
    uint64_t n_needed = 0;
    uint32_t n_levels = 0;
    float ms_total = 0.f;
};
void plan_fetch(Store* s, TipsetDev& td, const ipcfp_storage_spec* sspecs, uint64_t n_sspecs, const ipcfp_event_spec* especs, uint64_t n_especs,
                FetchPlan& out, const ipcfp_log_filter* log_filters = nullptr, uint64_t n_log_filters = 0);

void comm_unique_id(uint8_t* id128);
Comm* comm_init(const uint8_t* id128, uint32_t world, uint32_t rank, int device);
void comm_destroy(Comm* c);
uint32_t comm_world(const Comm* c);
uint32_t comm_rank(const Comm* c);
struct ShardExchange {
    Comm* c;
    Store* s;
    uint64_t lo, hi;
    std::vector<uint64_t> nseg_all;
    uint64_t nraw = 0, max_nseg = 0, pos0 = 0, nseg = 0;
    bool peers_ok = true;
    bool all_early = false;
    const RawCid* seg = nullptr;
    uint64_t cap = 0, nwords = 0;
    unsigned long long* n_exec_dev = nullptr;
    unsigned long long* overflow_dev = nullptr;
    uint64_t M = 0;
    const uint32_t* match_rel_dev = nullptr;
    unsigned long long* n_exec_out = nullptr;
    uint64_t g_tx = ~0ull, g_err = ~0ull;
    bool g_missing_base = false, g_overflow = false, g_stale = false;
    uint64_t M_max = 0, nw_max = 0, M_total = 0, proofs_total = 0;
    std::vector<uint64_t> nw_all;
    bool full_union = false;
    const uint8_t* wit_cids = nullptr;
    uint64_t wit_n = 0;
    uint8_t* union_dev = nullptr;
    ShardExchange(Comm* comm, Store* store, uint64_t lo_, uint64_t hi_);
    void agree_early(bool can_promise, uint64_t planned_nseg, uint64_t nraw_total);
    void agree_slices(uint64_t tx_key, uint64_t err_key, uint64_t nseg_);
    void start_exchange(const void* seg_dev);
    void positions_for(const uint32_t* match_rel, uint64_t n_match, unsigned long long* n_exec_out_);
    bool agree_results(uint64_t tx_key, uint64_t err_key, bool missing_base, uint64_t n_proofs, uint64_t n_witness, bool stale, const void* seg_dev,
                       uint64_t nseg_);
    void fetch_and_patch(ipcfp_event_proof* proofs_dev, uint64_t n_proofs, void* proofs_host);
    void witness_union(const uint8_t* cids_dev, uint64_t n_local, bool full);
    void finish();
    void fill_result(ipcfp_event_result& r) const;
    void trace_timeline(cudaEvent_t origin, const char* engine_part) const;
private:
    void gather_results(uint64_t tx_key, uint64_t err_key, bool missing_base, uint64_t n_proofs, uint64_t n_witness, uint64_t exch_overflow, bool stale);
    void patch(ipcfp_event_proof* proofs_dev, uint64_t n_proofs);
    void union_replicated(uint64_t* n_out_dev_word);
    uint64_t union_piece_cap(bool cannot_overflow) const;
    void union_partitioned(uint64_t cap);
    void timings(float* ms_exchange, float* ms_fetch, float* ms_union) const;
};

ipcfp_slot_result* read_storage_slots(Store* s, const uint8_t* root, const uint8_t* slots, uint64_t k);
void slot_result_free(ipcfp_slot_result* r);
ipcfp_storage_result* generate_storage_proofs(Store* s, const uint8_t* child_cid, const uint8_t* state_root, const ipcfp_storage_spec* specs, uint64_t n,
                                              bool by_ref = false);
void storage_result_free(ipcfp_storage_result* r);
const WitnessOut& storage_result_witness(const ipcfp_storage_result* r);

struct WitnessOut {
    PinnedArray cids, offsets, lengths, blob;
    PinnedArray sorted_idx;
    AsyncBuf<uint8_t> cids_dev;
    AsyncBuf<uint32_t> idx_dev;
    uint64_t n = 0, blob_size = 0;
    void fill(ipcfp_witness& w) const {
        w.n_blocks = n; w.cids = cids.as<uint8_t>(); w.offsets = offsets.as<uint64_t>(); w.lengths = lengths.as<uint32_t>();
        w.blob = blob.as<uint8_t>(); w.blob_size = blob_size;
    }
};
struct WitnessBuilder {
    Store* s;
    cudaStream_t st, st2;
    uint64_t nwords = 0, mA = 0, mB = 0, bytesA = 0, bytesB = 0, host_cap = 0;
    bool have_snapshot = false;
    bool by_ref = false;
    AsyncBuf<uint32_t> idx, plen, bitsA, bitsB;
    AsyncBuf<uint64_t> offs, word_prefix, word_prefixB, scratch;
    AsyncBuf<uint8_t> dblobA, dblobB_keep;
    PinnedArray host_blob;
    explicit WitnessBuilder(Store* store);
    void snapshot(const uint32_t* wbits);
    void start_copy(uint64_t mA, uint64_t bytesA, uint64_t split_idx, uint64_t split_bytes);
    void finish_enqueue(const uint32_t* wbits);
    void finish(uint64_t mB, uint64_t bytesB, WitnessOut& out, bool want_sorted_idx = false);
    void finish_start(uint64_t mB, uint64_t bytesB, WitnessOut& out, bool want_sorted_idx = false);
    void finish_join(WitnessOut& out);
};
void materialize_witness(Store* s, const uint32_t* wbits_dev, WitnessOut& out, bool by_ref = false);
void witness_union(Store* s, const std::vector<const WitnessOut*>& lists, WitnessOut& out, bool by_ref);

struct ResolveOut {
    std::vector<uint64_t> ids;
    std::vector<int32_t> status;
    int32_t init_status = IPCFP_OK;
    std::vector<uint8_t> missing;
    WitnessOut wit;
    float ms_total = 0.f, ms_lookup = 0.f;
};
void resolve_addresses(Store* s, const uint8_t* state_root, const ipcfp_address* addrs, uint64_t n, ResolveOut& out);
void address_parse(const char* text, uint64_t len, ipcfp_address& out);
void address_from_eth(const uint8_t eth[20], ipcfp_address& out);

struct JsonInputs {
    const ipcfp_event_proof* proofs;
    uint64_t n_proofs;
    const uint8_t* blob;
    const uint8_t* cids;
    const uint32_t* idx;
    uint64_t m;
    int64_t parent_epoch, child_epoch;
    uint32_t n_parents;
    const uint8_t* parent_cids;
    const uint8_t* child_cid;
};
uint64_t render_event_json(Store* s, const JsonInputs& in, PinnedArray& out);
struct UnifiedJsonInputs {
    const ipcfp_storage_proof* storage;
    uint64_t n_storage;
    const ipcfp_event_proof* proofs;
    uint64_t n_proofs;
    const uint8_t* blob;
    const uint8_t* cids;
    const uint32_t* idx;
    uint64_t m;
    int64_t parent_epoch, child_epoch;
    uint32_t n_parents;
    const uint8_t* parent_cids;
    const uint8_t* child_cid;
    const uint8_t* state_root;
};
uint64_t render_unified_json(Store* s, const UnifiedJsonInputs& in, PinnedArray& out);
size_t sort_by_cid_ws_bytes(uint64_t m);
void sort_by_cid(Store* s, const uint32_t* idx_dev, uint32_t* ord, uint64_t m, void* workspace);

}
```

ipc_filecoin_proofs_b200/csrc/events.cu:

```cuda
#include <algorithm>
#include <cstdlib>
#include <cstring>

#include <chrono>
#include <cstddef>
#include <optional>
#include <type_traits>
#include <cooperative_groups.h>
#include "engine.cuh"
#include "hashes.cuh"
#include "ipld.cuh"
#include "prims.cuh"
#include "walk.cuh"
#include "events_items.cuh"
#include "pass1_stage.cuh"
#include "rawcid.cuh"

namespace ipcfp {
namespace cg = cooperative_groups;


template <class P>
__global__ void __launch_bounds__(128) k_pass2(Pass2ArgsT<P> a) {
    uint64_t t = (uint64_t)blockIdx.x * blockDim.x + threadIdx.x;
    if (a.per_warp) { if (threadIdx.x & 31) return; t >>= 5; }
    if (t >= a.n_match) return;
    pass2_item(a, t);
}

#define IPCFP_MAX_PARENTS 64
static_assert(2 * IPCFP_MAX_PARENTS <= DENSE_MAX_AMTS, "the dense plan's tables hold every message AMT");
struct Prologue {
    uint32_t misc[64 + 2 * IPCFP_MAX_PARENTS];
    uint64_t amt_count[2 * IPCFP_MAX_PARENTS];
    uint64_t t0[4];
    DenseTables plan;
};
static constexpr uint32_t PRO_HEAD_WORDS = (uint32_t)((offsetof(Prologue, plan) + offsetof(DenseTables, per_amt)) / 8);
static_assert(PRO_HEAD_WORDS <= HW_PROLOGUE_WORDS, "the prologue's head fits its host words (HW_PROLOGUE)");
static_assert(offsetof(Prologue, misc) == 0 && 3 * sizeof(uint32_t) <= HW_ANY_SKIP_WORDS * 8, "misc[2] (any_skip) fits its host words (HW_ANY_SKIP)");
struct SetupArgs {
    StoreView store;
    uint32_t n_parents;
    const uint8_t* parent_cids;
    const uint8_t* txmeta_cids;
    const uint8_t* child_cid;
    const uint8_t* receipts_root;
    uint32_t skip_tx;
    uint32_t skip_receipts;
    uint32_t* wbits;
    unsigned long long* err;
    unsigned long long* txerr;
    Prologue* pro;
    uint32_t* f_blk; uint32_t* f_meta; uint64_t* f_base;
    unsigned long long* f_count;
    const uint8_t* sig;
    uint32_t sig_len;
    Matcher* matcher;
    uint32_t plan_dense;
    uint64_t frontier_cap, max_raw;
};

__device__ __forceinline__ void setup_receipts_root(const SetupArgs& a) {
    const StoreView& s = a.store;
    int32_t rb = store_lookup(s, a.receipts_root);
    if (rb < 0) { report_error(a.err, ST_RECEIPTS_ROOT, 0, DC_MISSING, 0); return; }
    witness_mark(s, a.wbits, (uint32_t)rb);
    a.pro->misc[0] = (uint32_t)rb;
    uint32_t len;
    const uint8_t* p = store_block(s, (uint32_t)rb, len);
    Rd r(p, len);
    uint32_t bw, h;
    uint64_t cnt;
    amt_root_begin(r, 0, bw, h, cnt);
    AmtNodeHdr hd;
    amt_node_begin(r, 3, hd);
    uint32_t nv = rd_array(r);
    for (uint32_t v = 0; v < nv && !r.err; v++) parse_receipt(r);
    amt_node_finish(r, hd, nv, h);
    if (r.err) report_error(a.err, ST_RECEIPTS_ROOT, 0, DC_DECODE, r.err);
}

__global__ void __launch_bounds__(256) k_setup(SetupArgs a) {
    const StoreView& s = a.store;
    const uint32_t t = threadIdx.x, P = a.n_parents;
    uint32_t* const amt_height = a.pro->misc + 64;
    uint64_t* const amt_count = a.pro->amt_count;
    if (t >= 128 && !a.skip_tx) {
        for (uint32_t i = t - 128; i < 2 * P + 2; i += 128) {
            const uint8_t* cid = i < P ? a.parent_cids + 38 * i : (i == P ? a.child_cid : (i == P + 1 ? a.receipts_root : a.txmeta_cids + 38 * (i - P - 2)));
            int32_t b = store_lookup(s, cid);
            if (b < 0) a.pro->misc[1] = 1; else witness_mark(s, a.wbits, (uint32_t)b);
        }
    }
    if (t == 96 && a.matcher) {
        Digest d;
        keccak256(a.sig, a.sig_len, d);
        for (int k = 0; k < 4; k++) a.matcher->t0[k] = a.pro->t0[k] = d.w[k];
    }
    if (t >= 32 && t < 96) for (uint32_t b = t - 32; b < P; b += 64) {
        for (uint32_t k = 0; k < 2; k++) { a.f_meta[2 * b + k] = AMT_SENTINEL; a.f_blk[2 * b + k] = 0; a.f_base[2 * b + k] = 0; amt_height[2 * b + k] = 0; amt_count[2 * b + k] = 0; }
        int32_t tb = store_lookup(s, a.txmeta_cids + 38 * b);
        if (tb < 0) { report_tx_error(a.txerr, 3 * b, 0, 31, DC_MISSING, 0); continue; }
        if (!a.skip_tx) witness_mark(s, a.wbits, (uint32_t)tb);
        uint32_t len;
        const uint8_t* p = store_block(s, (uint32_t)tb, len);
        Rd r(p, len);
        rd_array_exact(r, 2);
        uint32_t c0 = rd_cid(r), c1 = rd_cid(r);
        rd_end(r);
        if (r.err) { report_tx_error(a.txerr, 3 * b, 0, 31, DC_DECODE, r.err); continue; }
        for (uint32_t k = 0; k < 2; k++) {
            int32_t rb = store_lookup(s, p + (k ? c1 : c0));
            if (rb < 0) { report_tx_error(a.txerr, 3 * b + 1 + k, 0, 31, DC_MISSING, 0); break; }
            if (!a.skip_tx) witness_mark(s, a.wbits, (uint32_t)rb);
            uint32_t rl;
            const uint8_t* rp = store_block(s, (uint32_t)rb, rl);
            Rd rr(rp, rl);
            uint32_t bw, h;
            uint64_t cnt;
            amt_root_begin(rr, 0, bw, h, cnt);
            if (rr.err) { report_tx_error(a.txerr, 3 * b + 1 + k, 0, 31, DC_DECODE, rr.err); break; }
            const uint32_t amt = 2 * b + k;
            a.f_blk[amt] = (uint32_t)rb;
            a.f_meta[amt] = make_meta(amt, 1, h);
            a.f_base[amt] = 0;
            amt_height[amt] = h;
            amt_count[amt] = cnt;
        }
    }
    if (t == 0) {
        *a.f_count = 2 * P;
        if (!a.skip_receipts) setup_receipts_root(a);
    }
    if (!a.plan_dense) return;
    __syncthreads();
    if (t != 0) return;
    const uint32_t namt = 2 * P;
    DenseTables& pl = a.pro->plan;
    for (uint32_t k = 0; k < namt; k++) { pl.per_amt[2ull * namt + k] = 0; pl.per_amt[3ull * namt + k] = UINT64_MAX; }
    uint32_t rounds;
    uint64_t nraw;
    const bool ok = dense_plan(namt, amt_height, amt_count, pl.per_amt + 2ull * namt, pl.per_amt + 3ull * namt, a.frontier_cap, a.max_raw, sizeof(DenseTables),
                               pl.fofs, pl.ftot, pl.per_amt, &rounds, &nraw);
    const bool fault = *(volatile unsigned long long*)a.err != IPCFP_NO_ERROR || *(volatile unsigned long long*)a.txerr != IPCFP_NO_ERROR;
    pl.rounds = rounds;
    pl.nraw = nraw;
    pl.ok = ok && !fault;
}

__global__ void __launch_bounds__(128) k_amt_count(StoreView store, Frontier in, const unsigned long long* in_count, uint32_t round, uint32_t last_round,
                                                   uint32_t cap, uint32_t* counts, const uint64_t* rlo, const uint64_t* rhi) {
    uint64_t t = (uint64_t)blockIdx.x * blockDim.x + threadIdx.x;
    uint64_t cnt = *in_count;
    if (cnt > cap) cnt = cap;
    if (t >= cnt) { counts[t] = 0; return; }
    counts[t] = amt_item_count(store, in.blk[t], in.meta[t], in.base[t], round, last_round, rlo, rhi);
}
__global__ void __launch_bounds__(128) k_amt_expand(ExpandArgs a, const uint32_t* counts, unsigned long long* out_count, const unsigned long long* total) {
    const uint64_t g = (uint64_t)blockIdx.x * blockDim.x + threadIdx.x;
    const uint64_t t = g >> 3;
    const uint32_t j = (uint32_t)g & 7;
    uint64_t cnt = *a.in_count;
    if (cnt > a.cap) cnt = a.cap;
    if (g == 0) {
        unsigned long long n = *total;
        if (a.round < a.last_round && n > a.cap) { report_tx_error(a.err, IPCFP_TX_EIDX_NONE, 0, 0, DC_UNSUPPORTED, 1); n = a.cap; }
        *out_count = n;
    }
    if (t >= cnt) return;
    amt_item_expand(a, t, j, a.in.blk[t], a.in.meta[t], a.in.base[t], counts[t]);
}

#define TOP_CAP 1024
__global__ void __launch_bounds__(TOP_CAP) k_amt_top(ExpandArgs a0, Frontier ping, Frontier pong, unsigned long long* count_io, uint32_t first_round,
                                                      uint32_t n_rounds, uint64_t* scan_tmp) {
    __shared__ uint32_t s_cnt[TOP_CAP];
    __shared__ uint32_t s_warp[32];
    __shared__ uint32_t s_total;
    const uint32_t t = threadIdx.x, lane = t & 31, warp = t >> 5;
// ... 138 lines not shown

struct EventResultBox {
    ipcfp_event_result r;
    PinnedArray matching, proofs, blob;
    WitnessOut wit;
    PinnedArray union_host;
    PinnedArray json;
    AsyncBuf<RawCid> shard_exec;
};

static void throw_device_error(uint64_t key) {
    uint32_t stage = (uint32_t)(key >> 56), code = (uint32_t)(key >> 8) & 0xff, detail = (uint32_t)key & 0xff;
    uint64_t index = (key >> 16) & 0xFFFFFFFFFFull;
    ipcfp_status st;
    const char* what;
    switch (code) {
        case DC_MISSING: st = IPCFP_ERR_MISSING_BLOCK; what = "missing block"; break;
        case DC_DECODE: st = IPCFP_ERR_DECODE; what = "decode error"; break;
        case 0:
        case DC_MISSING_EXEC: st = IPCFP_ERR_MISSING_EXEC; what = "Missing message at index"; break;
        case DC_UNSUPPORTED: st = IPCFP_ERR_UNSUPPORTED; what = "unsupported input (frontier overflow)"; break;
        default: st = IPCFP_ERR_DECODE; what = "error"; break;
    }
    uint64_t out_index = UINT64_MAX;
    const char* stage_name = "?";
    switch (stage) {
        case ST_TXMETA:
            stage_name = "message AMTs";
            if (index != 0xFFFFFFFFFFull && index % 3 == 0 && code == DC_MISSING) out_index = index / 3;
            break;
        case ST_RECEIPTS_ROOT: stage_name = "receipts AMT root"; break;
        case ST_PASS1: stage_name = "pass 1"; out_index = index; break;
        case ST_PASS2: stage_name = "pass 2"; out_index = index; break;
        case ST_WITNESS: stage_name = "materialize"; break;
        default: break;
    }
    throw Error(st, std::string(what) + " in " + stage_name + " (detail " + std::to_string(detail) + ")", out_index);
}

static void throw_tx_error(uint64_t key) {
    const uint32_t eidx = (uint32_t)(key >> 56), code = (uint32_t)(key >> 4) & 7, detail = (uint32_t)key & 15;
    ipcfp_status st;
    const char* what;
    switch (code) {
        case DC_MISSING: st = IPCFP_ERR_MISSING_BLOCK; what = "missing block"; break;
        case DC_UNSUPPORTED: st = IPCFP_ERR_UNSUPPORTED; what = "unsupported input (frontier overflow)"; break;
        default: st = IPCFP_ERR_DECODE; what = "decode error"; break;
    }
    uint64_t out_index = UINT64_MAX;
    if (eidx != IPCFP_TX_EIDX_NONE && eidx % 3 == 0 && code == DC_MISSING) out_index = eidx / 3;
    throw Error(st, std::string(what) + " in message AMTs (detail " + std::to_string(detail) + ")", out_index);
}
static void throw_first(uint64_t tx_key, uint64_t err_key, bool missing_base = false) {
    if (tx_key != IPCFP_NO_ERROR) throw_tx_error(tx_key);
    if (err_key != IPCFP_NO_ERROR) throw_device_error(err_key);
    if (missing_base) throw Error(IPCFP_ERR_MISSING_BLOCK, "missing block (base witness CID not in the store)");
}

void tipset_upload(Store* s, const ipcfp_tipset_desc* t, TipsetDev& td) {
    s->use();
    if (!t || !t->child_cid || !t->receipts_root || (t->n_parents && (!t->parent_cids || !t->parent_txmeta_cids)))
        throw Error(IPCFP_ERR_INVALID_ARG, "tipset descriptor has null fields");
    if (t->n_parents > IPCFP_MAX_PARENTS) throw Error(IPCFP_ERR_UNSUPPORTED, "too many parent blocks");
    if (t->n_receipts >= 0xffffffffull) throw Error(IPCFP_ERR_UNSUPPORTED, "more than 2^32 receipts");
    if (t->n_receipts && (!t->events_roots || !t->has_events_root)) throw Error(IPCFP_ERR_INVALID_ARG, "events roots missing");
    td.device = s->device;
    td.parent_epoch = t->parent_epoch; td.child_epoch = t->child_epoch; td.n_parents = t->n_parents;
    td.parent_cids.assign(t->parent_cids, t->parent_cids + 38ull * t->n_parents);
    td.txmeta_cids.assign(t->parent_txmeta_cids, t->parent_txmeta_cids + 38ull * t->n_parents);
    memcpy(td.child_cid, t->child_cid, 38);
    memcpy(td.receipts_root, t->receipts_root, 38);
    td.has_state_root = t->child_parent_state_root != nullptr;
    if (td.has_state_root) memcpy(td.child_state_root, t->child_parent_state_root, 38);
    td.n_receipts = t->n_receipts;
    td.events_roots.alloc(t->n_receipts * 38 + 64);
    td.has_root.alloc(t->n_receipts + 64);
    if (t->n_receipts) {
        IPCFP_CUDA(cudaMemcpyAsync(td.events_roots.p, t->events_roots, t->n_receipts * 38, cudaMemcpyHostToDevice, s->stream));
        IPCFP_CUDA(cudaMemcpyAsync(td.has_root.p, t->has_events_root, t->n_receipts, cudaMemcpyHostToDevice, s->stream));
    }
}

namespace {
static constexpr size_t STAGE_TABLES = 32768;

template <class P>
struct EventCall {
    Store* s;
    cudaStream_t st;
    TipsetDev& td;
    const ipcfp_event_spec* spec;
    const ipcfp_log_filter* filter = nullptr;
    uint32_t flags;
    bool sharded;
    uint64_t lo, hi;
    Comm* comm;
    ExecOrderOut* exo;
    std::chrono::steady_clock::time_point t_enter;
    uint64_t N = 0, nblk = 0;
    bool skip_tx = false;
    std::unique_ptr<ShardExchange> xch;
    uint64_t pend_tx = IPCFP_NO_ERROR, pend_err = IPCFP_NO_ERROR;
    unsigned long long* dw;
    uint64_t* hw;
    P mh;
    size_t siglen = 0, tables_off = 0;
    AsyncBuf<uint8_t> small;
    uint8_t *d_sig = nullptr, *d_cids = nullptr;
    P* d_matcher = nullptr;
    AsyncBuf<uint64_t> d_sets;
    PinnedArray sets_h;
    AsyncBuf<uint32_t> wbits;
    uint32_t namt = 0;
    uint64_t cap = 0;
    AsyncBuf<uint32_t> fA_blk, fA_meta, fB_blk, fB_meta;
    AsyncBuf<uint64_t> fA_base, fB_base;
    AsyncBuf<Prologue> pro;
    uint32_t* misc = nullptr;
    uint32_t frontier_cap = 0;
    uint64_t max_raw_dev = 0;
    bool force_general = false, plan_on_device = false;
    SetupArgs sa;
    const Prologue* ph;
    bool early_fault = false, missing_base = false;
    uint32_t receipts_root_blk = 0, last_round = 0;
    std::vector<uint64_t> h_rng = std::vector<uint64_t>(4 * IPCFP_MAX_PARENTS, 0);
    uint64_t nraw_total = 0;
    AsyncBuf<uint32_t> counts;
    AsyncBuf<uint64_t> out_off, scratch;
    unsigned long long *ccount = nullptr, *ncount = nullptr, *total_dev = nullptr;
    AsyncBuf<RawCid> exec_raw;
    uint64_t raw_cap = 0;
    DensePlan plan;
    AsyncBuf<uint64_t> d_foff;
    AsyncBuf<uint32_t> d_flen;
    DenseArgs da;
    AsyncBuf<uint64_t> d_rng;
    AsyncBuf<uint32_t> g_blk[2], g_meta[2];
    AsyncBuf<uint64_t> g_base[2];
    bool dense_used = false, xch_early = false;
    std::optional<WitnessBuilder> wbuild;
    uint64_t nraw = 0;
    bool xch_stale = false;
    AsyncBuf<uint32_t> exec_idx, keep_bits;
    unsigned long long* n_exec_dev = nullptr;
    AsyncBuf<uint32_t> match_bits, cnt, nby;
    AsyncBuf<uint64_t> pbase, bbase;
    AsyncBuf<uint32_t> match_rel;
    AsyncBuf<uint64_t> wp3;
    uint64_t n_exec = 0, M = 0, pass1_nodes = 0, pass1_bytes = 0, n_proofs = 0, n_bytes = 0;
    std::unique_ptr<EventResultBox> box;
    AsyncBuf<ipcfp_event_proof> d_proofs;
    AsyncBuf<uint8_t> d_blob;
    uint64_t mB = 0;
    bool any_skip = false;
    PinnedArray rel;
    uint64_t json_len = 0;

    EventCall(Store* s_, TipsetDev& td_, const ipcfp_event_spec* spec_, uint32_t flags_, bool sharded_, uint64_t lo_, uint64_t hi_, Comm* comm_,
              ExecOrderOut* exo_)
        : s(s_), st(s_->stream), td(td_), spec(spec_), flags(flags_), sharded(sharded_), lo(lo_), hi(hi_), comm(comm_), exo(exo_),
          dw(s_->dev_words.p), hw(s_->host_words.p), ph((const Prologue*)(s_->host_words.p + HW_PROLOGUE)) {}

    void note_errors() {
        if (!xch) { throw_first(hw[DW_TX_ERR], hw[DW_ERR]); return; }
        pend_tx = std::min<uint64_t>(pend_tx, hw[DW_TX_ERR]);
        pend_err = std::min<uint64_t>(pend_err, hw[DW_ERR]);
    }
    void publish_prologue() { publish_words(s, HW_PROLOGUE, PRO_HEAD_WORDS, pro.p); }
    void read_prologue() {
        early_fault = hw[DW_ERR] != IPCFP_NO_ERROR || hw[DW_TX_ERR] != IPCFP_NO_ERROR;
        if constexpr (std::is_same_v<P, Matcher>) memcpy(mh.t0, ph->t0, 32);
        receipts_root_blk = ph->misc[0];
        missing_base = ph->misc[1] != 0;
        last_round = 0;
        for (uint32_t k = 0; k < namt; k++) last_round = std::max(last_round, ph->misc[64 + k]);
        nraw_total = shard_amt_ranges(namt, ph->amt_count, sharded, lo, hi, td.n_receipts, h_rng.data(), h_rng.data() + 2 * IPCFP_MAX_PARENTS);
    }
    void ensure_scratch(uint64_t n) {
        if (scratch.n < scan_scratch_elems(n + 64) + 64) scratch.alloc(scan_scratch_elems(n + 64) + 64, st);
    }

    void stage() {
        s->use();
        t_enter = std::chrono::steady_clock::now();
        LogFilterHost lfh;
        if constexpr (std::is_same_v<P, Matcher>) {
            if (!spec || !spec->event_signature || !spec->topic_1) throw Error(IPCFP_ERR_INVALID_ARG, "event spec has null fields");
        } else {
            log_filter_build(filter, lfh);
        }
        if (sharded && (flags & IPCFP_RESULT_JSON)) throw Error(IPCFP_ERR_UNSUPPORTED, "IPCFP_RESULT_JSON is not available for sharded calls");
        if ((flags & IPCFP_WITNESS_BY_REFERENCE) && !s->caller_blob)
            throw Error(IPCFP_ERR_UNSUPPORTED, "IPCFP_WITNESS_BY_REFERENCE needs a store made from a caller's blob (ipcfp_store_create)");
        if (!sharded) { lo = 0; hi = td.n_receipts; }
        if (lo > hi || hi > td.n_receipts) throw Error(IPCFP_ERR_INVALID_ARG, "receipt range out of bounds");
        N = hi - lo;
        nblk = s->n;
        skip_tx = (flags & IPCFP_SCAN_SKIP_TX_AMTS) != 0;
        if (comm) {
            if (!sharded) throw Error(IPCFP_ERR_INVALID_ARG, "communicator given for an unsharded call");
            if (s->class_prefix.size() > 1) throw Error(IPCFP_ERR_UNSUPPORTED, "sharded calls need a store with one CID prefix");
            xch.reset(new ShardExchange(comm, s, lo, hi));
        }

        IPCFP_CUDA(cudaEventRecord(s->ev[EV_BEGIN], st));
        IPCFP_CUDA(cudaMemsetAsync(dw + DW_ERR, 0xff, 8, st));
        IPCFP_CUDA(cudaMemsetAsync(dw + DW_FRONTIER_A, 0, 40 * 8, st));
        IPCFP_CUDA(cudaMemsetAsync(dw + DW_TX_ERR, 0xff, 8, st));

        memset(&mh, 0, sizeof mh);
        if constexpr (std::is_same_v<P, Matcher>) {
            size_t n1 = strlen(spec->topic_1);
            uint8_t t1[32];
            memset(t1, 0, 32);
            memcpy(t1, spec->topic_1, n1 < 32 ? n1 : 32);
            memcpy(mh.t1, t1, 32);
            mh.actor = spec->actor_id_filter;
            mh.has_actor = spec->has_actor_id_filter ? 1 : 0;
            siglen = strlen(spec->event_signature);
        } else {
            if (!lfh.dev.empty()) {
                sets_h = PinnedArray(s->pool, lfh.dev.size() * 8);
                memcpy(sets_h.p, lfh.dev.data(), lfh.dev.size() * 8);
                d_sets.alloc(lfh.dev.size(), st);
                IPCFP_CUDA(cudaMemcpyAsync(d_sets.p, sets_h.p, lfh.dev.size() * 8, cudaMemcpyHostToDevice, st));
            }
            lfh.place(d_sets.p);
            mh = lfh.f;
        }
        const size_t sig_cap = (siglen + 64) & ~(size_t)63;
        const size_t cids_bytes = 38ull * (2 * td.n_parents + 2);
        const size_t small_bytes = 1024 + sig_cap + cids_bytes + 64;
        static_assert(sizeof(P) <= 1024, "the predicate must fit its staging slot");
        tables_off = std::max<size_t>(STAGE_TABLES, (small_bytes + 63) & ~(size_t)63);
        if (!s->stage.p || s->stage.cap < tables_off + STAGE_TABLES) s->stage = PinnedArray(s->pool, tables_off + STAGE_TABLES);
        small.alloc(small_bytes, st);
        d_sig = small.p + 1024;
        d_cids = small.p + 1024 + sig_cap;
        d_matcher = (P*)small.p;
        uint8_t* hs = s->stage.as<uint8_t>();
        memset(hs, 0, small_bytes);
        memcpy(hs, &mh, sizeof(P));
        if (siglen) memcpy(hs + 1024, spec->event_signature, siglen);
        uint8_t* hc = hs + 1024 + sig_cap;
        memcpy(hc, td.parent_cids.data(), td.parent_cids.size()); hc += td.parent_cids.size();
        memcpy(hc, td.txmeta_cids.data(), td.txmeta_cids.size()); hc += td.txmeta_cids.size();
        memcpy(hc, td.child_cid, 38); hc += 38;
        memcpy(hc, td.receipts_root, 38);
        IPCFP_CUDA(cudaMemcpyAsync(small.p, hs, small_bytes, cudaMemcpyHostToDevice, st));
    }

    void setup() {
        wbits.alloc((nblk + 31) / 32 + 8, st);
        wbits.zero();
        namt = 2 * td.n_parents;
        cap = 4 * nblk + 1024;
        fA_blk.alloc(cap, st); fA_meta.alloc(cap, st); fB_blk.alloc(cap, st); fB_meta.alloc(cap, st);
        fA_base.alloc(cap, st); fB_base.alloc(cap, st);
        pro.alloc(1, st);
        pro.zero();
        misc = &pro.p->misc[0];
        frontier_cap = (uint32_t)std::min<uint64_t>(cap, 0xffffffffull);
        max_raw_dev = std::min<uint64_t>(8ull * cap, (uint64_t)td.n_parents * td.n_receipts + 1024);
        force_general = getenv("IPCFP_BFS_GENERAL") != nullptr;
        plan_on_device = !sharded && !exo && !force_general;
        sa.store = s->view; sa.n_parents = td.n_parents;
        sa.parent_cids = d_cids; sa.txmeta_cids = d_cids + 38ull * td.n_parents;
        sa.child_cid = d_cids + 76ull * td.n_parents; sa.receipts_root = sa.child_cid + 38;
        sa.skip_tx = skip_tx; sa.skip_receipts = exo ? 1 : 0; sa.wbits = wbits.p; sa.err = dw + DW_ERR; sa.txerr = dw + DW_TX_ERR;
        sa.pro = pro.p;
        sa.f_blk = fA_blk.p; sa.f_meta = fA_meta.p; sa.f_base = fA_base.p; sa.f_count = dw + DW_FRONTIER_A;
        sa.sig = d_sig; sa.sig_len = (uint32_t)siglen;
        if constexpr (std::is_same_v<P, Matcher>) sa.matcher = d_matcher; else sa.matcher = nullptr;
        sa.plan_dense = plan_on_device ? 1 : 0; sa.frontier_cap = frontier_cap; sa.max_raw = max_raw_dev;
        k_setup<<<1, 256, 0, st>>>(sa); IPCFP_LAUNCH_CHECK();
        IPCFP_CUDA(cudaEventRecord(s->ev[EV_SETUP], st));
    }

    void walk() {
        counts.alloc(cap + 1024, st);
        out_off.alloc(cap + 1024, st); scratch.alloc(scan_scratch_elems(std::max<uint64_t>(cap, N) + 64) + 64, st);
        ccount = dw + DW_FRONTIER_A; ncount = dw + DW_FRONTIER_B; total_dev = dw + DW_LEVEL_TOTAL;
        if (!plan_on_device) {
            publish_words(s, 0, DW_TX_ERR + 1);
            publish_prologue();
            IPCFP_CUDA(cudaStreamSynchronize(st));
            read_prologue();
            if (namt > 0 && !force_general && !early_fault)
                plan = make_dense_plan(namt, ph->misc + 64, ph->amt_count, h_rng.data(), h_rng.data() + 2 * IPCFP_MAX_PARENTS, frontier_cap, 8ull * cap,
                                       sizeof(DenseTables));
        }
        memset(&da, 0, sizeof da);
        dense_used = plan_on_device || plan.ok;
        if (dense_used) run_dense(); else run_general();
        IPCFP_CUDA(cudaEventRecord(s->ev[EV_RAW_LIST], st));
    }
    void run_dense() {
        if (!plan_on_device) {
            static_assert(sizeof(DenseTables) <= STAGE_TABLES, "the dense plan must fit its staging slot");
            DenseTables* ht = (DenseTables*)(s->stage.as<uint8_t>() + tables_off);
            memset(ht, 0, sizeof *ht);
            ht->ok = 1; ht->rounds = plan.rounds; ht->nraw = plan.nraw;
            std::copy(plan.per_amt.begin(), plan.per_amt.end(), ht->per_amt);
            std::copy(plan.fofs.begin(), plan.fofs.end(), ht->fofs);
            std::copy(plan.ftot.begin(), plan.ftot.end(), ht->ftot);
            IPCFP_CUDA(cudaMemcpyAsync(&pro.p->plan, ht, sizeof(DenseTables), cudaMemcpyHostToDevice, st));
        }
        raw_cap = plan_on_device ? max_raw_dev : plan.nraw;
        exec_raw.alloc(raw_cap + 64, st);
        if (!plan_on_device) exec_raw.zero();
        const DenseTables* tb = &pro.p->plan;
        da.store = s->view;
        da.ping = Frontier{fA_blk.p, fA_meta.p, fA_base.p}; da.pong = Frontier{fB_blk.p, fB_meta.p, fB_base.p};
        da.vals = exec_raw.p;
        da.tables = tb;
        da.vbase = tb->per_amt; da.cnt = tb->per_amt + namt; da.lo = tb->per_amt + 2ull * namt; da.hi = tb->per_amt + 3ull * namt;
        da.fofs = tb->fofs; da.ftot = tb->ftot;
        da.namt = namt; da.record = skip_tx ? 0 : 1; da.wbits = wbits.p; da.fail = (uint32_t*)(dw + DW_DENSE_FAIL);
        uint64_t fmax = 1;
        if (plan_on_device) fmax = max_raw_dev / 8 + namt + 8;
        else for (uint32_t r = 0; r < plan.rounds; r++) fmax = std::max<uint64_t>(fmax, plan.ftot[r]);
        d_foff.alloc(2 * fmax + 8, st); d_flen.alloc(2 * fmax + 8, st);
        da.f_off[0] = d_foff.p; da.f_off[1] = d_foff.p + fmax; da.f_len[0] = d_flen.p; da.f_len[1] = d_flen.p + fmax;
        if (!s->walk_grid) {
            int per_sm = 0, sms = 0;
            IPCFP_CUDA(cudaOccupancyMaxActiveBlocksPerMultiprocessor(&per_sm, k_amt_dense, DENSE_THREADS, 0));
            IPCFP_CUDA(cudaDeviceGetAttribute(&sms, cudaDevAttrMultiProcessorCount, s->device));
            s->walk_grid = (unsigned)std::max(1, per_sm * sms);
        }
        void* args[] = {&da};
        IPCFP_CUDA(cudaLaunchCooperativeKernel((const void*)k_amt_dense, s->walk_grid, DENSE_THREADS, args, 0, st)); IPCFP_LAUNCH_CHECK();
        k_amt_dense_leaf<<<s->walk_grid, DENSE_THREADS, 0, st>>>(da); IPCFP_LAUNCH_CHECK();
    }
    void run_general() {
        d_rng.alloc(4 * IPCFP_MAX_PARENTS, st);
        IPCFP_CUDA(cudaMemcpyAsync(d_rng.p, h_rng.data(), h_rng.size() * 8, cudaMemcpyHostToDevice, st));
        IPCFP_CUDA(cudaStreamSynchronize(st));
        auto ensure_g = [&](int i, uint64_t n) {
            if (g_blk[i].n < n) { g_blk[i].alloc(n, st); g_meta[i].alloc(n, st); g_base[i].alloc(n, st); }
        };
        auto gview = [&](int i) { return Frontier{g_blk[i].p, g_meta[i].p, g_base[i].p}; };
        ensure_g(0, 8 * TOP_CAP); ensure_g(1, 8 * TOP_CAP);
        IPCFP_CUDA(cudaMemcpyAsync(g_blk[0].p, fA_blk.p, namt * 4ull, cudaMemcpyDeviceToDevice, st));
        IPCFP_CUDA(cudaMemcpyAsync(g_meta[0].p, fA_meta.p, namt * 4ull, cudaMemcpyDeviceToDevice, st));
        IPCFP_CUDA(cudaMemcpyAsync(g_base[0].p, fA_base.p, namt * 8ull, cudaMemcpyDeviceToDevice, st));
        int cur = 0;
        ccount = dw + DW_FRONTIER_A; ncount = dw + DW_FRONTIER_B;
        ExpandArgs ea;
        ea.store = s->view; ea.last_round = last_round; ea.record = skip_tx ? 0 : 1; ea.wbits = wbits.p; ea.err = dw + DW_TX_ERR;
        ea.vals = nullptr; ea.cap = 8 * TOP_CAP;
        ea.rlo = d_rng.p; ea.rhi = d_rng.p + 2 * IPCFP_MAX_PARENTS;
        auto alloc_vals = [&](uint64_t n) {
            raw_cap = n;
            exec_raw.alloc(raw_cap + 64, st);
            exec_raw.zero();
            ea.vals = exec_raw.p;
        };
        auto bound_of = [&](uint32_t round) { uint64_t b = namt; for (uint32_t k = 0; k < round && b <= TOP_CAP; k++) b *= 8; return b; };
        uint32_t top_rounds = 0;
        while (top_rounds <= last_round && bound_of(top_rounds) <= TOP_CAP) top_rounds++;
        uint32_t round = 0;
        if (top_rounds) {
            if (top_rounds > last_round) alloc_vals(bound_of(last_round) * 8);
            ExpandArgs a0 = ea;
            a0.in = gview(0); a0.in_count = ccount; a0.out = gview(1); a0.round = 0; a0.out_off = out_off.p;
            k_amt_top<<<1, TOP_CAP, 0, st>>>(a0, gview(0), gview(1), ccount, 0, top_rounds, out_off.p); IPCFP_LAUNCH_CHECK();
            cur = top_rounds & 1;
            round = top_rounds;
        }
        if (round > last_round) return;
        publish_words(s, (uint32_t)(ccount - dw), 1);
        IPCFP_CUDA(cudaStreamSynchronize(st));
        uint64_t items = hw[ccount - dw];
        for (; round <= last_round; round++) {
            const uint64_t slots = (uint64_t)div_up(std::max<uint64_t>(items, 1), 128) * 128;
            if (counts.n < slots) { counts.alloc(slots, st); out_off.alloc(slots, st); }
            ensure_scratch(slots);
            k_amt_count<<<(unsigned)(slots / 128), 128, 0, st>>>(s->view, gview(cur), ccount, round, last_round, (uint32_t)items, counts.p, ea.rlo, ea.rhi);
            IPCFP_LAUNCH_CHECK();
            exclusive_scan_u32(counts.p, out_off.p, slots, (uint64_t*)total_dev, scratch.p, st);
            publish_words(s, DW_LEVEL_TOTAL, 1);
            IPCFP_CUDA(cudaStreamSynchronize(st));
            const uint64_t total = hw[DW_LEVEL_TOTAL];
            if (round == last_round) alloc_vals(total);
            ExpandArgs a = ea;
            a.in = gview(cur); a.in_count = ccount; a.round = round; a.out_off = out_off.p; a.out = gview(cur ^ 1);
            a.cap = (uint32_t)items;
            if (round < last_round) {
                if (std::max(total, items) >= 0xffffffffull) throw Error(IPCFP_ERR_UNSUPPORTED, "message-AMT walk: a level of 2^32 nodes or more");
                ensure_g(cur ^ 1, std::max(total, items) + 1);
                a.out = gview(cur ^ 1);
                a.cap = (uint32_t)(std::max(total, items) + 1);
                cur ^= 1;
            }
            k_amt_expand<<<div_up(std::max<uint64_t>(items, 1) * 8, 128), 128, 0, st>>>(a, counts.p, ncount, total_dev); IPCFP_LAUNCH_CHECK();
            std::swap(ccount, ncount);
            items = total;
        }
    }
    void snapshot_and_sync(bool with_prologue) {
        if (!exo) wbuild->snapshot(wbits.p);
        publish_words(s, 0, DW_SPLIT_BYTES + 1);
        if (with_prologue) publish_prologue();
        IPCFP_CUDA(cudaStreamSynchronize(st));
        if (with_prologue) read_prologue();
    }

    void settle_walk() {
        if (xch) {
            xch->agree_early(plan.ok && !early_fault, plan.ok ? plan.nraw : 0, nraw_total);
            xch_early = xch->all_early;
            if (xch_early) xch->start_exchange(exec_raw.p);
        }
        wbuild.emplace(s);
        wbuild->by_ref = (flags & IPCFP_WITNESS_BY_REFERENCE) != 0;
        snapshot_and_sync(plan_on_device);
        if (dense_used && hw[DW_DENSE_FAIL] != 0) {
            dense_used = false;
            k_setup<<<1, 256, 0, st>>>(sa); IPCFP_LAUNCH_CHECK();
            run_general();
            IPCFP_CUDA(cudaEventRecord(s->ev[EV_RAW_LIST], st));
            snapshot_and_sync(false);
        }
        const uint32_t ccount_idx = (uint32_t)(ccount - dw);
        if (!sharded && hw[DW_TX_ERR] != IPCFP_NO_ERROR) {
            const uint64_t key = hw[DW_TX_ERR];
            const uint32_t eidx = (uint32_t)(key >> 56), level = 31u - ((uint32_t)(key >> 7) & 31u);
            if (eidx != IPCFP_TX_EIDX_NONE && eidx % 3 != 0 && level < 31) {
                const uint32_t amt = 2 * (eidx / 3) + eidx % 3 - 1;
                if (ph->misc[64 + amt] > TX_KEY_EXACT_HEIGHT) {
                    k_amt_first_fault<<<1, 1, 0, st>>>(s->view, sa.txmeta_cids, amt, dw + DW_TX_ERR); IPCFP_LAUNCH_CHECK();
                    publish_words(s, DW_TX_ERR, 1);
                    IPCFP_CUDA(cudaStreamSynchronize(st));
                }
            }
        }
        note_errors();
        if (!dense_used && hw[ccount_idx] > raw_cap) {
            if (!xch) throw Error(IPCFP_ERR_UNSUPPORTED, "unsupported input (message list longer than the walk's capacity)");
            pend_tx = std::min<uint64_t>(pend_tx, tx_err_key(IPCFP_TX_EIDX_NONE, 0, 0, DC_UNSUPPORTED, 1));
        }
        nraw = dense_used ? (plan_on_device ? ph->plan.nraw : plan.nraw) : std::min<uint64_t>(hw[ccount_idx], raw_cap);
        xch_stale = xch_early && (!dense_used || nraw != plan.nraw);
        if (xch && !xch_early && (pend_tx != IPCFP_NO_ERROR || pend_err != IPCFP_NO_ERROR)) {
            xch->agree_slices(pend_tx, pend_err, 0);
            throw_first(xch->g_tx, xch->g_err);
        }
        if (!exo) wbuild->start_copy(hw[DW_WIT_A], hw[DW_WIT_A_BYTES], hw[DW_SPLIT_IDX], hw[DW_SPLIT_BYTES]);
        if (xch && !xch_early) {
            xch->agree_slices(IPCFP_NO_ERROR, IPCFP_NO_ERROR, nraw);
            if (!xch->peers_ok) { IPCFP_CUDA(cudaStreamSynchronize(st)); throw_first(xch->g_tx, xch->g_err); }
            xch->start_exchange(exec_raw.p);
        }
    }

    bool dedup() {
        exec_idx.alloc(nraw + 32, st); keep_bits.alloc((nraw + 31) / 32 + 8, st);
        n_exec_dev = dw + DW_N_EXEC;
        if (sharded) IPCFP_CUDA(cudaMemsetAsync(n_exec_dev, 0, 8, st));
        else if (nraw) {
            if (nraw >= 0xffffffffull) throw Error(IPCFP_ERR_UNSUPPORTED, "message list of 2^32 entries or more");
            ensure_scratch((nraw + 31) / 32);
            uint64_t slots = 64;
            while (slots < 2 * nraw) slots <<= 1;
            AsyncBuf<unsigned long long> dtab(slots, st);
            dtab.zero();
            k_dedup_insert<<<div_up(nraw, 256), 256, 0, st>>>(exec_raw.p, nraw, dtab.p, slots - 1); IPCFP_LAUNCH_CHECK();
            k_dedup_flags<<<div_up((nraw + 31) / 32 * 32, 256), 256, 0, st>>>(exec_raw.p, nraw, dtab.p, slots - 1, keep_bits.p); IPCFP_LAUNCH_CHECK();
            AsyncBuf<uint64_t> wp2((nraw + 31) / 32 + 8, st);
            bitmap_to_indices(keep_bits.p, nraw, exec_idx.p, (uint64_t*)n_exec_dev, wp2.p, scratch.p, st);
        } else IPCFP_CUDA(cudaMemsetAsync(n_exec_dev, 0, 8, st));
        IPCFP_CUDA(cudaEventRecord(s->ev[EV_EXEC_ORDER], st));
        if (!exo) return true;
        publish_words(s, DW_N_EXEC, 1);
        IPCFP_CUDA(cudaStreamSynchronize(st));
        exo->n_exec = hw[DW_N_EXEC];
        exo->nraw = nraw;
        exo->exec_raw = std::move(exec_raw);
        exo->exec_idx = std::move(exec_idx);
        return false;
    }

    void pass1() {
        match_bits.alloc((N + 31) / 32 + 8, st); cnt.alloc(N + 8, st); nby.alloc(N + 8, st);
        pbase.alloc(N + 8, st); bbase.alloc(N + 8, st);
        Pass1ArgsT<P> p1;
        p1.store = s->view; p1.store_dev = s->view_dev.p; p1.m_dev = d_matcher; p1.m = mh; p1.events_roots = td.events_roots.p; p1.has_root = td.has_root.p; p1.lo = lo; p1.hi = hi;
        p1.match_bits = match_bits.p; p1.cnt = cnt.p; p1.nbytes = nby.p; p1.err = dw + DW_ERR; p1.stats = dw + DW_STATS;
        if (N) {
            const int smem = 4 * StageGeom<128, 4, 1>::WARP_BYTES;
            IPCFP_CUDA(cudaFuncSetAttribute(k_pass1_stage<P, 128, 4, 1, 4, 3>, cudaFuncAttributeMaxDynamicSharedMemorySize, smem));
            k_pass1_stage<P, 128, 4, 1, 4, 3><<<div_up(N, 128), 128, smem, st>>>(p1); IPCFP_LAUNCH_CHECK();
        }
        IPCFP_CUDA(cudaEventRecord(s->ev[EV_PASS1], st));
        match_rel.alloc(N + 32, st);
        wp3.alloc((N + 31) / 32 + 8, st);
        bitmap_to_indices(match_bits.p, (N + 31) / 32 * 32, match_rel.p, (uint64_t*)(dw + DW_N_MATCH), wp3.p, scratch.p, st);
        exclusive_scan_u32(cnt.p, pbase.p, N, (uint64_t*)(dw + DW_N_PROOFS), scratch.p, st);
        exclusive_scan_u32(nby.p, bbase.p, N, (uint64_t*)(dw + DW_BLOB_BYTES), scratch.p, st);
        publish_words(s, 0, DW_TX_ERR + 1);
        IPCFP_CUDA(cudaStreamSynchronize(st));
        note_errors();
        n_exec = hw[DW_N_EXEC];
        M = hw[DW_N_MATCH];
        pass1_nodes = hw[DW_STATS]; pass1_bytes = hw[DW_STATS + 1];
        n_proofs = hw[DW_N_PROOFS]; n_bytes = hw[DW_BLOB_BYTES];
    }

    void pass2() {
        box.reset(new EventResultBox());
        memset(&box->r, 0, sizeof box->r);
        d_proofs.alloc(n_proofs + 1, st);
        d_blob.alloc(n_bytes + 16, st);
        if (M) {
            Pass2ArgsT<P> p2;
            p2.store = s->view; p2.store_dev = s->view_dev.p; p2.m_dev = d_matcher; p2.m = mh; p2.events_roots = td.events_roots.p; p2.lo = lo; p2.match_rel = match_rel.p; p2.n_match = M;
            p2.receipts_root_blk = receipts_root_blk; p2.exec_cids = exec_raw.p; p2.exec_idx = exec_idx.p; p2.n_exec = n_exec_dev;
            p2.wbits = wbits.p; p2.err = dw + DW_ERR; p2.cnt = cnt.p; p2.proof_base = pbase.p; p2.byte_base = bbase.p;
            p2.proofs = d_proofs.p; p2.blob = d_blob.p; p2.any_skip = misc + 2; p2.resolve_msg = sharded ? 0 : 1;
            p2.per_warp = (M <= 16384 && !getenv("IPCFP_PASS2_PER_THREAD")) ? 1 : 0;
            k_pass2<<<div_up(p2.per_warp ? M * 32 : M, 128), 128, 0, st>>>(p2); IPCFP_LAUNCH_CHECK();
        }
        if (xch) xch->positions_for(match_rel.p, M, n_exec_dev);
        wbuild->finish_enqueue(wbits.p);
        publish_words(s, 0, DW_EXEC_CHECK + 1);
        publish_words(s, HW_ANY_SKIP, HW_ANY_SKIP_WORDS, misc);
        IPCFP_CUDA(cudaStreamSynchronize(st));
        note_errors();
        if (!xch && missing_base && !skip_tx) throw_first(IPCFP_NO_ERROR, IPCFP_NO_ERROR, true);
        mB = hw[DW_WIT_B];
        any_skip = ((const uint32_t*)(hw + HW_ANY_SKIP))[2] != 0;
        IPCFP_CUDA(cudaEventRecord(s->ev[EV_PASS2], st));
    }

    void read_back() {
        box->matching = PinnedArray(s->pool, (M + 1) * 8);
        box->proofs = PinnedArray(s->pool, (n_proofs + 1) * sizeof(ipcfp_event_proof));
        box->blob = PinnedArray(s->pool, n_bytes + 16);
        rel = PinnedArray(s->pool, (M + 1) * 4);
        if (M) IPCFP_CUDA(cudaMemcpyAsync(rel.p, match_rel.p, M * 4, cudaMemcpyDeviceToHost, st));
        if (n_proofs && !xch) IPCFP_CUDA(cudaMemcpyAsync(box->proofs.p, d_proofs.p, n_proofs * sizeof(ipcfp_event_proof), cudaMemcpyDeviceToHost, st));
        if (n_bytes) IPCFP_CUDA(cudaMemcpyAsync(box->blob.p, d_blob.p, n_bytes, cudaMemcpyDeviceToHost, st));
        wbuild->finish_start(mB, hw[DW_WIT_B_BYTES], box->wit);
        if (xch) {
            if (!xch->agree_results(pend_tx, pend_err, missing_base && !skip_tx, n_proofs, hw[DW_WIT_A] + mB, xch_stale, exec_raw.p, nraw)) {
                wbuild->finish_join(box->wit);
                throw_first(xch->g_tx, xch->g_err, xch->g_missing_base);
                throw Error(IPCFP_ERR_UNSUPPORTED, "execution-order exchange: bucket overflow (skewed CID hash distribution)");
            }
            xch->fetch_and_patch(d_proofs.p, n_proofs, box->proofs.p);
            xch->witness_union(box->wit.cids_dev.p, box->wit.n, (flags & IPCFP_SHARDED_UNION_FULL) != 0);
        }
        if (flags & IPCFP_RESULT_JSON) {
            IPCFP_CUDA(cudaEventRecord(s->ev[EV_JSON_BEGIN], st));
            JsonInputs ji{d_proofs.p, n_proofs, d_blob.p, box->wit.cids_dev.p, box->wit.idx_dev.p, box->wit.n,
                          td.parent_epoch, td.child_epoch, td.n_parents, sa.parent_cids, sa.child_cid};
            json_len = render_event_json(s, ji, box->json);
            IPCFP_CUDA(cudaEventRecord(s->ev[EV_JSON_END], st));
        }
        wbuild->finish_join(box->wit);
        if (xch) xch->finish();
    }

    ipcfp_event_result* fill() {
        static thread_local std::chrono::steady_clock::time_point t_last_exit = t_enter;
        IPCFP_CUDA(cudaEventRecord(s->ev[EV_END], st));
        IPCFP_CUDA(cudaStreamSynchronize(st));
        {
            uint64_t* mo = box->matching.as<uint64_t>();
            const uint32_t* rp = rel.as<uint32_t>();
            for (uint64_t k = 0; k < M; k++) mo[k] = lo + rp[k];
        }
        if (any_skip) {
            ipcfp_event_proof* pp = box->proofs.as<ipcfp_event_proof>();
            uint64_t w = 0;
            for (uint64_t k = 0; k < n_proofs; k++) if (pp[k].exec_index != UINT64_MAX) pp[w++] = pp[k];
            n_proofs = w;
        }
        ipcfp_event_result& r = box->r;
        r.n_matching = M; r.matching_indices = box->matching.as<uint64_t>();
        r.n_proofs = n_proofs; r.proofs = box->proofs.as<ipcfp_event_proof>();
        r.data_blob = box->blob.as<uint8_t>(); r.data_blob_size = n_bytes;
        box->wit.fill(r.witness);
        r.n_exec = n_exec;
        float ms;
        IPCFP_CUDA(cudaEventElapsedTime(&ms, s->ev[EV_BEGIN], s->ev[EV_END])); r.ms_total = ms;
        IPCFP_CUDA(cudaEventElapsedTime(&ms, s->ev[EV_SETUP], s->ev[EV_EXEC_ORDER])); r.ms_txamt = ms;
        IPCFP_CUDA(cudaEventElapsedTime(&ms, s->ev[EV_EXEC_ORDER], s->ev[EV_PASS1])); r.ms_pass1 = ms;
        IPCFP_CUDA(cudaEventElapsedTime(&ms, s->ev[EV_PASS1], s->ev[EV_PASS2])); r.ms_pass2 = ms;
        IPCFP_CUDA(cudaEventElapsedTime(&ms, s->ev[EV_PASS2], s->ev[EV_END])); r.ms_witness = ms;
        r.pass1_bytes = pass1_bytes; r.pass1_nodes = pass1_nodes;
        if (flags & IPCFP_RESULT_JSON) {
            r.json = box->json.as<char>(); r.json_len = json_len;
            IPCFP_CUDA(cudaEventElapsedTime(&ms, s->ev[EV_JSON_BEGIN], s->ev[EV_JSON_END])); r.ms_json = ms;
        }
        r.shard_raw_total = nraw_total;
        if (sharded) { r.n_exec = 0; r.shard_exec_count = nraw; box->shard_exec = std::move(exec_raw); r.shard_exec_dev = box->shard_exec.p; }
        if (xch) {
            xch->fill_result(r);
            if (getenv("IPCFP_XCH_TRACE")) {
                float t[6]; char buf[384];
                const int evs[6] = {EV_EXEC_ORDER, EV_PASS1, EV_PASS2, EV_WITNESS_SORTED, EV_BLOB_COPIED, EV_END};
                for (int i = 0; i < 6; i++) cudaEventElapsedTime(&t[i], s->ev[EV_BEGIN], s->ev[evs[i]]);
                const auto t_now = std::chrono::steady_clock::now();
                const double host_call = std::chrono::duration<double, std::milli>(t_now - t_enter).count();
                const double host_gap = std::chrono::duration<double, std::milli>(t_enter - t_last_exit).count();
                snprintf(buf, sizeof buf, "host: gap since last call %.3f, in call %.3f | walk %.3f pass1 %.3f pass2 %.3f sorted %.3f blobD2H %.3f end %.3f", host_gap, host_call,
                         t[0], t[1], t[2], t[3], t[4], t[5]);
                t_last_exit = std::chrono::steady_clock::now();
                xch->trace_timeline(s->ev[EV_BEGIN], buf);
            }
            if (flags & IPCFP_SHARDED_UNION_TO_HOST) {
                box->union_host = PinnedArray(s->pool, r.n_union_part * 38 + 64);
                if (r.n_union_part) IPCFP_CUDA(cudaMemcpyAsync(box->union_host.p, r.union_cids_dev, r.n_union_part * 38, cudaMemcpyDeviceToHost, st));
                IPCFP_CUDA(cudaStreamSynchronize(st));
                r.union_cids = box->union_host.as<uint8_t>();
            }
        }
        return &box.release()->r;
    }
};
}

ipcfp_event_result* generate_event_proof(Store* s, TipsetDev& td, const ipcfp_event_spec* spec, uint32_t flags, bool sharded, uint64_t lo, uint64_t hi,
                                         Comm* comm, ExecOrderOut* exo) {
    EventCall<Matcher> c(s, td, spec, flags, sharded, lo, hi, comm, exo);
    c.stage();
    c.setup();
    c.walk();
    c.settle_walk();
    if (!c.dedup()) return nullptr;
    c.pass1();
    c.pass2();
    c.read_back();
    return c.fill();
}

ipcfp_event_result* generate_log_proof(Store* s, TipsetDev& td, const ipcfp_log_filter* filter, uint32_t flags) {
    EventCall<LogFilter> c(s, td, nullptr, flags, false, 0, 0, nullptr, nullptr);
    c.filter = filter;
    c.stage();
    c.setup();
    c.walk();
    c.settle_walk();
    c.dedup();
    c.pass1();
    c.pass2();
    c.read_back();
    return c.fill();
}

void event_result_free(ipcfp_event_result* r) { delete reinterpret_cast<EventResultBox*>(r); }
const WitnessOut& event_result_witness(const ipcfp_event_result* r) { return reinterpret_cast<const EventResultBox*>(r)->wit; }

}
```

ipc_filecoin_proofs_b200/csrc/witness.cu:

```cuda
#include "engine.cuh"
#include "prims.cuh"

namespace ipcfp {

struct ClassRanks { uint8_t r[IPCFP_MAX_CID_CLASSES]; };

__device__ __forceinline__ uint64_t bswap64(uint64_t x) {
    uint32_t lo = (uint32_t)x, hi = (uint32_t)(x >> 32);
    return ((uint64_t)__byte_perm(lo, 0, 0x0123) << 32) | (uint64_t)__byte_perm(hi, 0, 0x0123);
}
__device__ __forceinline__ int digest_cmp(const Digest& a, const Digest& b) {
#pragma unroll
    for (int k = 0; k < 4; k++) {
        uint64_t x = bswap64(a.w[k]), y = bswap64(b.w[k]);
        if (x != y) return x < y ? -1 : 1;
    }
    return 0;
}

__global__ void k_digest_keys(const uint32_t* __restrict__ idx, uint64_t m, const Digest* __restrict__ digests, uint32_t* keys, uint32_t* ord) {
    uint64_t i = (uint64_t)blockIdx.x * blockDim.x + threadIdx.x;
    if (i >= m) return;
    uint64_t w0 = digests[idx[i]].w[0];
    keys[i] = __byte_perm((uint32_t)w0, 0, 0x0123);
    ord[i] = (uint32_t)i;
}
__global__ void k_class_keys(const uint32_t* __restrict__ idx, const uint32_t* __restrict__ ord, uint64_t m, const uint8_t* __restrict__ cls,
                             ClassRanks cr, uint32_t* keys) {
    uint64_t i = (uint64_t)blockIdx.x * blockDim.x + threadIdx.x;
    if (i >= m) return;
    keys[i] = cr.r[cls[idx[ord[i]]]];
}
__global__ void k_tie_fix(const uint32_t* __restrict__ idx, uint32_t* ord, uint64_t m, const Digest* __restrict__ digests,
                          const uint8_t* __restrict__ cls, ClassRanks cr) {
    uint64_t i = (uint64_t)blockIdx.x * blockDim.x + threadIdx.x;
    if (i >= m) return;
    auto key_eq = [&](uint64_t a, uint64_t b) {
        uint32_t x = idx[ord[a]], y = idx[ord[b]];
        return cr.r[cls[x]] == cr.r[cls[y]] && (uint32_t)digests[x].w[0] == (uint32_t)digests[y].w[0];
    };
    if (i > 0 && key_eq(i - 1, i)) return;
    if (i + 1 >= m || !key_eq(i, i + 1)) return;
    uint64_t j = i + 1;
    while (j + 1 < m && key_eq(i, j + 1)) j++;
    for (uint64_t a = i + 1; a <= j; a++) {
        uint32_t v = ord[a];
        Digest dv = digests[idx[v]];
        uint64_t b = a;
        while (b > i && digest_cmp(digests[idx[ord[b - 1]]], dv) > 0) { ord[b] = ord[b - 1]; b--; }
        ord[b] = v;
    }
}

static inline size_t ws_round(size_t b) { return (b + 255) & ~(size_t)255; }
size_t sort_by_cid_ws_bytes(uint64_t m) {
    const unsigned nb = radix_blocks(m);
    return 3 * ws_round(m * 4 + 64) + ws_round(((size_t)256 * nb + 256) * 4) + ws_round(((size_t)256 * nb + 256) * 8) +
           ws_round((scan_scratch_elems((uint64_t)256 * nb) + 8) * 8);
}
void sort_by_cid(Store* s, const uint32_t* idx_dev, uint32_t* ord, uint64_t m, void* ws) {
    if (m == 0) return;
    cudaStream_t st = s->stream;
    const unsigned nb = radix_blocks(m);
    uint8_t* w = (uint8_t*)ws;
    uint32_t* keys = (uint32_t*)w; w += ws_round(m * 4 + 64);
    uint32_t* keys_alt = (uint32_t*)w; w += ws_round(m * 4 + 64);
    uint32_t* vals_alt = (uint32_t*)w; w += ws_round(m * 4 + 64);
    uint32_t* hist = (uint32_t*)w; w += ws_round(((size_t)256 * nb + 256) * 4);
    uint64_t* scan_tmp = (uint64_t*)w; w += ws_round(((size_t)256 * nb + 256) * 8);
    uint64_t* scratch = (uint64_t*)w;
    ClassRanks cr{};
    for (size_t c = 0; c < s->class_rank.size(); c++) cr.r[c] = (uint8_t)s->class_rank[c];
    k_digest_keys<<<div_up(m, 256), 256, 0, st>>>(idx_dev, m, s->digests.p, keys, ord); IPCFP_LAUNCH_CHECK();
    radix_sort_pairs(keys, ord, keys_alt, vals_alt, m, 32, hist, scan_tmp, scratch, st);
    if (s->class_prefix.size() > 1) {
        k_class_keys<<<div_up(m, 256), 256, 0, st>>>(idx_dev, ord, m, s->cls.p, cr, keys); IPCFP_LAUNCH_CHECK();
        radix_sort_pairs(keys, ord, keys_alt, vals_alt, m, 8, hist, scan_tmp, scratch, st);
    }
    k_tie_fix<<<div_up(m, 256), 256, 0, st>>>(idx_dev, ord, m, s->digests.p, s->cls.p, cr); IPCFP_LAUNCH_CHECK();
}

__global__ void k_padded_lengths(const uint32_t* __restrict__ idx, uint64_t m, const uint32_t* __restrict__ lengths, const uint32_t* __restrict__ bar, uint32_t* out) {
    uint64_t i = (uint64_t)blockIdx.x * blockDim.x + threadIdx.x;
    if (i < m) out[i] = (lengths[bar[idx[i]]] + 15u) & ~15u;
}
__global__ void k_sum_padded_dev(const uint32_t* __restrict__ idx, const unsigned long long* __restrict__ count, uint64_t n_max, const uint32_t* __restrict__ lengths,
                                 const uint32_t* __restrict__ bar, unsigned long long* out) {
    uint64_t i = (uint64_t)blockIdx.x * blockDim.x + threadIdx.x;
    unsigned long long v = (i < n_max && i < *count) ? (unsigned long long)((lengths[bar[idx[i]]] + 15u) & ~15u) : 0ull;
#pragma unroll
    for (int o = 16; o; o >>= 1) v += __shfl_down_sync(0xffffffffu, v, o);
    if ((threadIdx.x & 31) == 0 && v) atomicAdd(out, v);
}
__global__ void k_andnot(const uint32_t* __restrict__ a, const uint32_t* __restrict__ b, uint32_t* out, uint64_t nwords) {
    uint64_t i = (uint64_t)blockIdx.x * blockDim.x + threadIdx.x;
    if (i < nwords) out[i] = a[i] & ~b[i];
}
__global__ void __launch_bounds__(256) k_witness_copy(const uint32_t* __restrict__ idx, uint64_t m, StoreView v, const uint64_t* __restrict__ offsets,
                                                      uint8_t* out) {
    uint64_t w = ((uint64_t)blockIdx.x * blockDim.x + threadIdx.x) >> 5;
    uint32_t lane = threadIdx.x & 31;
    if (w >= m) return;
    uint32_t len;
    const uint8_t* src = store_block(v, v.block_at_rank[idx[w]], len);
    uint8_t* dst = out + offsets[w];
    if (((uintptr_t)src & 15) == 0) {
        uint32_t nv = (len + 15) >> 4;
        const uint4* s4 = (const uint4*)src;
        uint4* d4 = (uint4*)dst;
        for (uint32_t i = lane; i < nv; i += 32) d4[i] = __ldg(s4 + i);
    } else {
        for (uint32_t i = lane; i < len; i += 32) dst[i] = src[i];
    }
}
__device__ __forceinline__ uint32_t bits_below(const uint32_t* __restrict__ bits, const uint64_t* __restrict__ prefix, uint32_t r) {
    return (uint32_t)prefix[r >> 5] + (uint32_t)__popc(bits[r >> 5] & ((1u << (r & 31)) - 1u));
}
#define EMIT_THREADS 256
__global__ void __launch_bounds__(EMIT_THREADS) k_witness_emit(const uint32_t* __restrict__ idx, const uint64_t* __restrict__ offs, uint64_t m,
                                                               uint64_t mA, uint64_t baseB, const uint32_t* __restrict__ bitsA,
                                                               const uint64_t* __restrict__ prefixA, const uint32_t* __restrict__ bitsB,
                                                               const uint64_t* __restrict__ prefixB, StoreView v, uint8_t* cids, uint64_t* out_offs,
                                                               uint32_t* out_lens, uint32_t* out_idx, int by_ref) {
    __shared__ uint16_t rec[EMIT_THREADS][19];
    __shared__ uint64_t pos[EMIT_THREADS];
    const uint64_t i = (uint64_t)blockIdx.x * blockDim.x + threadIdx.x;
    if (i < m) {
        const uint32_t r = idx[i];
        uint64_t f;
        if (i < mA) f = i + (m > mA ? bits_below(bitsB, prefixB, r) : 0u);
        else f = (i - mA) + bits_below(bitsA, prefixA, r);
        const uint32_t b = v.block_at_rank[r];
        out_offs[f] = by_ref ? v.offsets[b] : offs[i] + (i >= mA ? baseB : 0);
        out_lens[f] = v.lengths[b];
        out_idx[f] = b;
        pos[threadIdx.x] = f;
        uint8_t* o = (uint8_t*)rec[threadIdx.x];
        uint32_t c = v.cls[b];
#pragma unroll
        for (int k = 0; k < 6; k++) o[k] = v.class_prefix[c][k];
        Digest d = v.digests[b];
#pragma unroll
        for (int w = 0; w < 4; w++)
#pragma unroll
            for (int k = 0; k < 8; k++) o[6 + 8 * w + k] = (uint8_t)(d.w[w] >> (8 * k));
    }
    __syncwarp();
    const uint32_t lane = threadIdx.x & 31, w0 = threadIdx.x - lane;
    const uint64_t first = i - lane;
    const uint32_t nrec = first < m ? (uint32_t)std::min<uint64_t>(32, m - first) : 0;
    for (uint32_t u = lane; u < nrec * 19; u += 32) {
        const uint32_t q = u / 19, k = u - 19 * q;
        ((uint16_t*)(cids + 38 * pos[w0 + q]))[k] = rec[w0 + q][k];
    }
}

WitnessBuilder::WitnessBuilder(Store* store) : s(store) {
    st = s->stream;
    if (!s->stream2) IPCFP_CUDA(cudaStreamCreateWithFlags(&s->stream2, cudaStreamNonBlocking));
    st2 = s->stream2;
    uint64_t n = s->n;
    nwords = (n + 31) / 32;
    idx.alloc(n + 64, st);
    offs.alloc(n + 64, st);
    plen.alloc(n + 64, st);
    bitsA.alloc(nwords + 8, st);
    word_prefix.alloc(nwords + 8, st);
    word_prefixB.alloc(nwords + 8, st);
    scratch.alloc(scan_scratch_elems(std::max<uint64_t>(nwords, n)) + 8, st);
}

__global__ void k_chunk_bounds(const uint64_t* __restrict__ offs, const unsigned long long* count, const unsigned long long* total, unsigned long long* out) {
    const uint64_t m = *count;
    uint64_t ia = m / 8;
    if (ia < 1024) ia = m < 1024 ? m : 1024;
    out[0] = ia;
    out[1] = ia < m ? offs[ia] : *total;
}
__global__ void k_padded_lengths_dev(const uint32_t* __restrict__ idx, const unsigned long long* __restrict__ count, uint64_t n_max,
                                     const uint32_t* __restrict__ lengths, const uint32_t* __restrict__ bar, uint32_t* out) {
    uint64_t i = (uint64_t)blockIdx.x * blockDim.x + threadIdx.x;
    if (i < n_max) out[i] = i < *count ? (lengths[bar[idx[i]]] + 15u) & ~15u : 0u;
}
void WitnessBuilder::snapshot(const uint32_t* wbits) {
    unsigned long long* dw = s->dev_words.p;
    IPCFP_CUDA(cudaMemcpyAsync(bitsA.p, wbits, nwords * 4, cudaMemcpyDeviceToDevice, st));
    bitmap_to_indices(bitsA.p, s->n, idx.p, (uint64_t*)(dw + DW_WIT_A), word_prefix.p, scratch.p, st);
    if (s->n) { k_padded_lengths_dev<<<div_up(s->n, 256), 256, 0, st>>>(idx.p, dw + DW_WIT_A, s->n, s->lengths.p, s->block_at_rank.p, plen.p); IPCFP_LAUNCH_CHECK(); }
    exclusive_scan_u32(plen.p, offs.p, s->n, (uint64_t*)(dw + DW_WIT_A_BYTES), scratch.p, st);
    k_chunk_bounds<<<1, 1, 0, st>>>(offs.p, dw + DW_WIT_A, dw + DW_WIT_A_BYTES, dw + DW_SPLIT_IDX); IPCFP_LAUNCH_CHECK();
    have_snapshot = true;
}
void WitnessBuilder::start_copy(uint64_t mA_, uint64_t bytesA_, uint64_t split_idx, uint64_t split_bytes) {
    mA = mA_;
    bytesA = bytesA_;
    if (by_ref) {
        bytesA = 0;
        IPCFP_CUDA(cudaEventRecord(s->ev[EV_BLOB_COPIED], st2));
        return;
    }
    host_cap = bytesA + bytesA / 8 + (8u << 20);
    host_blob = PinnedArray(s->pool, host_cap);
    host_cap = host_blob.cap;
    dblobA.alloc(bytesA + 64, st);
    const uint64_t ia = std::min(split_idx, mA), ba = ia == mA ? bytesA : std::min(split_bytes, bytesA);
    if (ia) { k_witness_copy<<<div_up(ia * 32, 256), 256, 0, st>>>(idx.p, ia, s->view, offs.p, dblobA.p); IPCFP_LAUNCH_CHECK(); }
    IPCFP_CUDA(cudaEventRecord(s->ev[EV_WITNESS_SORTED], st));
    IPCFP_CUDA(cudaStreamWaitEvent(st2, s->ev[EV_WITNESS_SORTED], 0));
    if (ba) IPCFP_CUDA(cudaMemcpyAsync(host_blob.p, dblobA.p, ba, cudaMemcpyDeviceToHost, st2));
    if (mA > ia) {
        k_witness_copy<<<div_up((mA - ia) * 32, 256), 256, 0, st>>>(idx.p + ia, mA - ia, s->view, offs.p + ia, dblobA.p); IPCFP_LAUNCH_CHECK();
        IPCFP_CUDA(cudaEventRecord(s->ev[EV_GATHER_B], st));
        IPCFP_CUDA(cudaStreamWaitEvent(st2, s->ev[EV_GATHER_B], 0));
        if (bytesA > ba) IPCFP_CUDA(cudaMemcpyAsync((uint8_t*)host_blob.p + ba, dblobA.p + ba, bytesA - ba, cudaMemcpyDeviceToHost, st2));
    }
    IPCFP_CUDA(cudaEventRecord(s->ev[EV_BLOB_COPIED], st2));
}
void WitnessBuilder::finish_enqueue(const uint32_t* wbits) {
    unsigned long long* dw = s->dev_words.p;
    bitsB.alloc(nwords + 8, st);
    k_andnot<<<div_up(nwords ? nwords : 1, 256), 256, 0, st>>>(wbits, bitsA.p, bitsB.p, nwords); IPCFP_LAUNCH_CHECK();
    bitmap_to_indices(bitsB.p, s->n, idx.p + mA, (uint64_t*)(dw + DW_WIT_B), word_prefixB.p, scratch.p, st);
    IPCFP_CUDA(cudaMemsetAsync(dw + DW_WIT_B_BYTES, 0, 8, st));
    const uint64_t bound = s->n > mA ? s->n - mA : 0;
    if (bound) { k_sum_padded_dev<<<div_up(bound, 256), 256, 0, st>>>(idx.p + mA, dw + DW_WIT_B, bound, s->lengths.p, s->block_at_rank.p, dw + DW_WIT_B_BYTES); IPCFP_LAUNCH_CHECK(); }
}
void WitnessBuilder::finish(uint64_t mB_, uint64_t bytesB_, WitnessOut& out, bool want_sorted_idx) {
    finish_start(mB_, bytesB_, out, want_sorted_idx);
    finish_join(out);
}
void WitnessBuilder::finish_start(uint64_t mB_, uint64_t bytesB_, WitnessOut& out, bool want_sorted_idx) {
    mB = mB_;
    bytesB = bytesB_;
    unsigned long long* dw = s->dev_words.p;
    uint64_t m = mA + mB;
    if (by_ref) { bytesB = 0; mB_ = 0; }
    if (mB_) {
        k_padded_lengths<<<div_up(mB, 256), 256, 0, st>>>(idx.p + mA, mB, s->lengths.p, s->block_at_rank.p, plen.p); IPCFP_LAUNCH_CHECK();
        exclusive_scan_u32(plen.p, offs.p + mA, mB, (uint64_t*)(dw + DW_WIT_B_BYTES), scratch.p, st);
    }
    if (bytesA + bytesB > host_cap) {
        IPCFP_CUDA(cudaStreamSynchronize(st2));
        PinnedArray bigger(s->pool, bytesA + bytesB + 64);
        memcpy(bigger.p, host_blob.p, bytesA);
        host_blob = std::move(bigger);
        host_cap = host_blob.cap;
    }
    AsyncBuf<uint8_t> dblobB(bytesB + 64, st);
    if (mB_) {
        k_witness_copy<<<div_up(mB * 32, 256), 256, 0, st>>>(idx.p + mA, mB, s->view, offs.p + mA, dblobB.p); IPCFP_LAUNCH_CHECK();
        IPCFP_CUDA(cudaMemcpyAsync((uint8_t*)host_blob.p + bytesA, dblobB.p, bytesB, cudaMemcpyDeviceToHost, st));
    }
    AsyncBuf<uint32_t> d_lens(m + 8, st), d_idx(m + 8, st);
    AsyncBuf<uint64_t> d_offs(m + 8, st);
    AsyncBuf<uint8_t> d_cids(m * 38 + 64, st);
    if (m) {
        k_witness_emit<<<div_up(m, EMIT_THREADS), EMIT_THREADS, 0, st>>>(idx.p, offs.p, m, mA, bytesA, bitsA.p, word_prefix.p, bitsB.p, word_prefixB.p, s->view, d_cids.p, d_offs.p,
                                                       d_lens.p, d_idx.p, by_ref ? 1 : 0);
        IPCFP_LAUNCH_CHECK();
    }
    IPCFP_CUDA(cudaEventRecord(s->ev[EV_WITNESS_SORTED], st));
    out.n = m;
    out.blob_size = bytesA + bytesB;
    out.cids = PinnedArray(s->pool, m * 38 + 64);
    out.offsets = PinnedArray(s->pool, (m + 1) * 8);
    out.lengths = PinnedArray(s->pool, (m + 1) * 4);
    if (want_sorted_idx) out.sorted_idx = PinnedArray(s->pool, (m + 1) * 4);
    if (m) {
        IPCFP_CUDA(cudaMemcpyAsync(out.cids.p, d_cids.p, m * 38, cudaMemcpyDeviceToHost, st));
        IPCFP_CUDA(cudaMemcpyAsync(out.offsets.p, d_offs.p, m * 8, cudaMemcpyDeviceToHost, st));
        IPCFP_CUDA(cudaMemcpyAsync(out.lengths.p, d_lens.p, m * 4, cudaMemcpyDeviceToHost, st));
        if (want_sorted_idx) IPCFP_CUDA(cudaMemcpyAsync(out.sorted_idx.p, d_idx.p, m * 4, cudaMemcpyDeviceToHost, st));
    }
    out.cids_dev = std::move(d_cids);
    out.idx_dev = std::move(d_idx);
    dblobB_keep = std::move(dblobB);
}
void WitnessBuilder::finish_join(WitnessOut& out) {
    IPCFP_CUDA(cudaStreamWaitEvent(st, s->ev[EV_BLOB_COPIED], 0));
    IPCFP_CUDA(cudaStreamSynchronize(st));
    IPCFP_CUDA(cudaStreamSynchronize(st2));
    out.blob = std::move(host_blob);
}

void materialize_witness(Store* s, const uint32_t* wbits_dev, WitnessOut& out, bool by_ref) {
    WitnessBuilder wb(s);
    wb.by_ref = by_ref;
    wb.snapshot(wbits_dev);
    publish_words(s, DW_WIT_A, 2);
    IPCFP_CUDA(cudaStreamSynchronize(s->stream));
    const uint64_t* hw = s->host_words.p;
    wb.start_copy(hw[DW_WIT_A], hw[DW_WIT_A_BYTES], hw[DW_WIT_A], hw[DW_WIT_A_BYTES]);
    wb.finish(0, 0, out, true);
}

__global__ void k_union_mark(const uint32_t* __restrict__ idx, uint64_t m, const uint32_t* __restrict__ rank_of, uint32_t* bits) {
    const uint64_t i = (uint64_t)blockIdx.x * blockDim.x + threadIdx.x;
    if (i >= m) return;
    const uint32_t r = rank_of[idx[i]];
    atomicOr(bits + (r >> 5), 1u << (r & 31));
}
void witness_union(Store* s, const std::vector<const WitnessOut*>& lists, WitnessOut& out, bool by_ref) {
    cudaStream_t st = s->stream;
    AsyncBuf<uint32_t> bits((s->n + 31) / 32 + 8, st);
    bits.zero();
    for (const WitnessOut* w : lists)
        if (w->n) { k_union_mark<<<div_up(w->n, 256), 256, 0, st>>>(w->idx_dev.p, w->n, s->rank_of.p, bits.p); IPCFP_LAUNCH_CHECK(); }
    materialize_witness(s, bits.p, out, by_ref);
}

}
```

Baseline: 661.9 million.

## Run pass2 and late witness speculatively on device to drop host syncs

Match offsets are now computed by a single-block device scan over matched receipts, replacing two full-length exclusive scans. Pass2 is launched speculatively into preallocated store-resident buffers, with device-side bounds checks that set an overflow flag, so the host no longer has to synchronize to read counts before launching. The late witness offsets, copy and emit are likewise enqueued with device-read counts and fixed capacities, falling back to the old path on overflow. A host sync counter is added for instrumentation. The trade is extra complexity, speculative over-allocation, and a single-CTA scan that could become serial for large match counts.

```diff
diff --git a/include/ipcfp.h b/include/ipcfp.h
--- a/include/ipcfp.h
+++ b/include/ipcfp.h
@@ -30,6 +30,7 @@
 uint64_t ipcfp_last_error_index(void);
 const char* ipcfp_version(void);
 uint64_t ipcfp_kernel_launch_count(void);
+uint64_t ipcfp_host_sync_count(void);
 
 ipcfp_status ipcfp_host_alloc(size_t bytes, void** out);
 void ipcfp_host_free(void* p);
diff --git a/integration/rust/ipcfp-sys/src/lib.rs b/integration/rust/ipcfp-sys/src/lib.rs
--- a/integration/rust/ipcfp-sys/src/lib.rs
+++ b/integration/rust/ipcfp-sys/src/lib.rs
@@ -121,6 +121,7 @@
     pub fn ipcfp_last_error_index() -> u64;
     pub fn ipcfp_version() -> *const c_char;
     pub fn ipcfp_kernel_launch_count() -> u64;
+    pub fn ipcfp_host_sync_count() -> u64;
     pub fn ipcfp_host_alloc(bytes: usize, out: *mut *mut c_void) -> ipcfp_status;
     pub fn ipcfp_host_free(p: *mut c_void);
 
diff --git a/ipc_filecoin_proofs_b200/api.py b/ipc_filecoin_proofs_b200/api.py
--- a/ipc_filecoin_proofs_b200/api.py
+++ b/ipc_filecoin_proofs_b200/api.py
@@ -24,7 +24,7 @@
 _lib = None
 
 EXPORTS = [
-    "ipcfp_last_error", "ipcfp_last_error_index", "ipcfp_version", "ipcfp_kernel_launch_count", "ipcfp_host_alloc", "ipcfp_host_free",
+    "ipcfp_last_error", "ipcfp_last_error_index", "ipcfp_version", "ipcfp_kernel_launch_count", "ipcfp_host_sync_count", "ipcfp_host_alloc", "ipcfp_host_free",
     "ipcfp_store_create", "ipcfp_store_destroy", "ipcfp_store_n_blocks", "ipcfp_store_get", "ipcfp_store_has",
     "ipcfp_store_first_bad_block", "ipcfp_blake2b256_batch", "ipcfp_keccak256_batch", "ipcfp_sha256_batch",
     "ipcfp_compute_mapping_slots", "ipcfp_generate_event_proof", "ipcfp_event_result_free", "ipcfp_read_storage_slots",
@@ -55,6 +55,7 @@
         L.ipcfp_last_error_index.restype = C.c_uint64
         L.ipcfp_version.restype = C.c_char_p
         L.ipcfp_kernel_launch_count.restype = C.c_uint64
+        L.ipcfp_host_sync_count.restype = C.c_uint64
         L.ipcfp_host_alloc.restype = C.c_int32
         L.ipcfp_host_alloc.argtypes = [C.c_size_t, C.POINTER(C.c_void_p)]
         L.ipcfp_host_free.argtypes = [C.c_void_p]
@@ -210,6 +211,10 @@
     return int(lib().ipcfp_kernel_launch_count())
 
 
+def host_sync_count():
+    return int(lib().ipcfp_host_sync_count())
+
+
 @dataclass
 class EventProofSpec:
     event_signature: str
diff --git a/ipc_filecoin_proofs_b200/csrc/capi.cu b/ipc_filecoin_proofs_b200/csrc/capi.cu
--- a/ipc_filecoin_proofs_b200/csrc/capi.cu
+++ b/ipc_filecoin_proofs_b200/csrc/capi.cu
@@ -8,9 +8,10 @@
 
 static thread_local std::string g_last_error;
 static thread_local uint64_t g_last_index = UINT64_MAX;
-static std::atomic<uint64_t> g_launches{0};
+static std::atomic<uint64_t> g_launches{0}, g_syncs{0};
 
 void note_launch() { g_launches.fetch_add(1, std::memory_order_relaxed); }
+void note_sync() { g_syncs.fetch_add(1, std::memory_order_relaxed); }
 void set_last_error(const std::string& msg, uint64_t index) { g_last_error = msg; g_last_index = index; }
 
 template <class F> static ipcfp_status guard(F f) {
@@ -156,6 +157,7 @@
            "k_exec_mark_dups k_select_positions k_fetch_positions k_part_pack k_merge_* (NCCL via dlopen)";
 }
 uint64_t ipcfp_kernel_launch_count(void) { return g_launches.load(); }
+uint64_t ipcfp_host_sync_count(void) { return g_syncs.load(); }
 
 ipcfp_status ipcfp_host_alloc(size_t bytes, void** out) {
     return guard([&] {
diff --git a/ipc_filecoin_proofs_b200/csrc/common.cuh b/ipc_filecoin_proofs_b200/csrc/common.cuh
--- a/ipc_filecoin_proofs_b200/csrc/common.cuh
+++ b/ipc_filecoin_proofs_b200/csrc/common.cuh
@@ -15,6 +15,7 @@
     Error(ipcfp_status s, std::string m, uint64_t i = UINT64_MAX) : status(s), msg(std::move(m)), index(i) {}
 };
 void note_launch();
+void note_sync();
 
 #define IPCFP_CUDA(expr)                                                                                          \
     do {                                                                                                          \
@@ -27,6 +28,12 @@
     do {                                                                       \
         ::ipcfp::note_launch();                                                \
         IPCFP_CUDA(cudaGetLastError());                                        \
+    } while (0)
+
+#define IPCFP_HOST_SYNC(st)                                                    \
+    do {                                                                       \
+        ::ipcfp::note_sync();                                                  \
+        IPCFP_CUDA(cudaStreamSynchronize(st));                                 \
     } while (0)
 
 static inline unsigned div_up(uint64_t a, uint64_t b) { return (unsigned)((a + b - 1) / b); }
diff --git a/ipc_filecoin_proofs_b200/csrc/engine.cuh b/ipc_filecoin_proofs_b200/csrc/engine.cuh
--- a/ipc_filecoin_proofs_b200/csrc/engine.cuh
+++ b/ipc_filecoin_proofs_b200/csrc/engine.cuh
@@ -60,6 +60,7 @@
     DW_SPLIT_IDX = 16, DW_SPLIT_BYTES = 17,
     DW_UNION_SIZE = 18,
     DW_EXEC_CHECK = 19,
+    DW_PASS2_OVERFLOW = 20,
     DW_JSON_TOTAL0 = 24, DW_JSON_TOTAL1 = 25, DW_JSON_OVERFLOW = 26, DW_JSON_TOTAL2 = 27,
     DW_COUNT = 64
 };
@@ -127,6 +128,8 @@
     DevBuf<unsigned long long> dev_words;
     PinnedBuf<uint64_t> host_words;
     PinnedArray stage;
+    DevBuf<ipcfp_event_proof> p2_proofs;
+    DevBuf<uint8_t> p2_blob;
     cudaEvent_t ev[EV_COUNT] = {};
     ~Store();
     void use() const { IPCFP_CUDA(cudaSetDevice(device)); }
@@ -278,6 +281,11 @@
     AsyncBuf<uint32_t> idx, plen, bitsA, bitsB;
     AsyncBuf<uint64_t> offs, word_prefix, word_prefixB, scratch;
     AsyncBuf<uint8_t> dblobA, dblobB_keep;
+    AsyncBuf<uint32_t> e_lens, e_idx;
+    AsyncBuf<uint64_t> e_offs;
+    AsyncBuf<uint8_t> e_cids;
+    uint64_t capB = 0, emit_cap = 0;
+    bool late_done = false;
     PinnedArray host_blob;
     explicit WitnessBuilder(Store* store);
     void snapshot(const uint32_t* wbits);
@@ -285,7 +293,7 @@
     void finish_enqueue(const uint32_t* wbits);
     void finish(uint64_t mB, uint64_t bytesB, WitnessOut& out, bool want_sorted_idx = false);
     void finish_start(uint64_t mB, uint64_t bytesB, WitnessOut& out, bool want_sorted_idx = false);
-    void finish_join(WitnessOut& out);
+    void finish_join(WitnessOut& out, cudaEvent_t end = nullptr);
 };
 void materialize_witness(Store* s, const uint32_t* wbits_dev, WitnessOut& out, bool by_ref = false);
 void witness_union(Store* s, const std::vector<const WitnessOut*>& lists, WitnessOut& out, bool by_ref);
diff --git a/ipc_filecoin_proofs_b200/csrc/events.cu b/ipc_filecoin_proofs_b200/csrc/events.cu
--- a/ipc_filecoin_proofs_b200/csrc/events.cu
+++ b/ipc_filecoin_proofs_b200/csrc/events.cu
@@ -26,6 +26,76 @@
     if (a.per_warp) { if (threadIdx.x & 31) return; t >>= 5; }
     if (t >= a.n_match) return;
     pass2_item(a, t);
+}
+
+#define PASS2_WARP_MAX 16384
+#define PASS2_SPEC_CTAS 1024
+template <class P>
+__global__ void __launch_bounds__(128) k_pass2_spec(Pass2ArgsT<P> a, const unsigned long long* n_match, const unsigned long long* n_proofs,
+                                                    const unsigned long long* n_bytes, uint64_t cap_proofs, uint64_t cap_bytes,
+                                                    unsigned long long* overflow) {
+    const uint64_t m = *n_match;
+    if (*(volatile unsigned long long*)a.err != IPCFP_NO_ERROR) return;
+    if (m > PASS2_WARP_MAX || *n_proofs > cap_proofs || *n_bytes > cap_bytes) {
+        if (blockIdx.x == 0 && threadIdx.x == 0) *overflow = 1;
+        return;
+    }
+    if (threadIdx.x & 31) return;
+    for (uint64_t w = ((uint64_t)blockIdx.x * blockDim.x + threadIdx.x) >> 5; w < m; w += ((uint64_t)gridDim.x * blockDim.x) >> 5) pass2_item(a, w);
+}
+
+#define MO_THREADS 1024
+#define MO_ITEMS 8
+__global__ void __launch_bounds__(MO_THREADS) k_match_offsets(const uint32_t* __restrict__ match_rel, const unsigned long long* n_match,
+                                                              const uint32_t* __restrict__ cnt, const uint32_t* __restrict__ nby, uint64_t* pbase,
+                                                              uint64_t* bbase, unsigned long long* n_proofs, unsigned long long* n_bytes) {
+    __shared__ uint64_t s_c[32], s_b[32], s_end[2];
+    const uint32_t t = threadIdx.x, lane = t & 31, warp = t >> 5;
+    const uint64_t m = *n_match;
+    uint64_t carry_c = 0, carry_b = 0;
+    for (uint64_t base = 0; base < m; base += MO_THREADS * MO_ITEMS) {
+        const uint64_t first = base + (uint64_t)t * MO_ITEMS;
+        uint32_t rel[MO_ITEMS];
+        uint64_t c[MO_ITEMS], b[MO_ITEMS], sc = 0, sb = 0;
+#pragma unroll
+        for (int k = 0; k < MO_ITEMS; k++) {
+            const bool in = first + k < m;
+            rel[k] = in ? match_rel[first + k] : 0;
+            c[k] = in ? cnt[rel[k]] : 0;
+            b[k] = in ? nby[rel[k]] : 0;
+            sc += c[k]; sb += b[k];
+        }
+        uint64_t xc = sc, xb = sb;
+#pragma unroll
+        for (int o = 1; o < 32; o <<= 1) {
+            const uint64_t yc = __shfl_up_sync(0xffffffffu, xc, o), yb = __shfl_up_sync(0xffffffffu, xb, o);
+            if (lane >= (uint32_t)o) { xc += yc; xb += yb; }
+        }
+        if (lane == 31) { s_c[warp] = xc; s_b[warp] = xb; }
+        __syncthreads();
+        if (warp == 0) {
+            const uint64_t vc = s_c[lane], vb = s_b[lane];
+            uint64_t wc = vc, wb = vb;
+#pragma unroll
+            for (int o = 1; o < 32; o <<= 1) {
+                const uint64_t yc = __shfl_up_sync(0xffffffffu, wc, o), yb = __shfl_up_sync(0xffffffffu, wb, o);
+                if (lane >= (uint32_t)o) { wc += yc; wb += yb; }
+            }
+            s_c[lane] = wc - vc; s_b[lane] = wb - vb;
+        }
+        __syncthreads();
+        uint64_t oc = carry_c + s_c[warp] + xc - sc, ob = carry_b + s_b[warp] + xb - sb;
+#pragma unroll
+        for (int k = 0; k < MO_ITEMS; k++) {
+            if (first + k < m) { pbase[rel[k]] = oc; bbase[rel[k]] = ob; }
+            oc += c[k]; ob += b[k];
+        }
+        if (t == MO_THREADS - 1) { s_end[0] = oc; s_end[1] = ob; }
+        __syncthreads();
+        carry_c = s_end[0]; carry_b = s_end[1];
+        __syncthreads();
+    }
+    if (t == 0) { *n_proofs = carry_c; *n_bytes = carry_b; }
 }
 
 #define IPCFP_MAX_PARENTS 64
@@ -470,6 +540,9 @@
     std::unique_ptr<EventResultBox> box;
     AsyncBuf<ipcfp_event_proof> d_proofs;
     AsyncBuf<uint8_t> d_blob;
+    bool spec2 = false;
+    ipcfp_event_proof* proofs_dev = nullptr;
+    uint8_t* blob_dev = nullptr;
     uint64_t mB = 0;
     bool any_skip = false;
     PinnedArray rel;
@@ -603,7 +676,7 @@
         if (!plan_on_device) {
             publish_words(s, 0, DW_TX_ERR + 1);
             publish_prologue();
-            IPCFP_CUDA(cudaStreamSynchronize(st));
+            IPCFP_HOST_SYNC(st);
             read_prologue();
             if (namt > 0 && !force_general && !early_fault)
                 plan = make_dense_plan(namt, ph->misc + 64, ph->amt_count, h_rng.data(), h_rng.data() + 2 * IPCFP_MAX_PARENTS, frontier_cap, 8ull * cap,
@@ -654,7 +727,7 @@
     void run_general() {
         d_rng.alloc(4 * IPCFP_MAX_PARENTS, st);
         IPCFP_CUDA(cudaMemcpyAsync(d_rng.p, h_rng.data(), h_rng.size() * 8, cudaMemcpyHostToDevice, st));
-        IPCFP_CUDA(cudaStreamSynchronize(st));
+        IPCFP_HOST_SYNC(st);
         auto ensure_g = [&](int i, uint64_t n) {
             if (g_blk[i].n < n) { g_blk[i].alloc(n, st); g_meta[i].alloc(n, st); g_base[i].alloc(n, st); }
         };
@@ -689,7 +762,7 @@
         }
         if (round > last_round) return;
         publish_words(s, (uint32_t)(ccount - dw), 1);
-        IPCFP_CUDA(cudaStreamSynchronize(st));
+        IPCFP_HOST_SYNC(st);
         uint64_t items = hw[ccount - dw];
         for (; round <= last_round; round++) {
             const uint64_t slots = (uint64_t)div_up(std::max<uint64_t>(items, 1), 128) * 128;
@@ -699,7 +772,7 @@
             IPCFP_LAUNCH_CHECK();
             exclusive_scan_u32(counts.p, out_off.p, slots, (uint64_t*)total_dev, scratch.p, st);
             publish_words(s, DW_LEVEL_TOTAL, 1);
-            IPCFP_CUDA(cudaStreamSynchronize(st));
+            IPCFP_HOST_SYNC(st);
             const uint64_t total = hw[DW_LEVEL_TOTAL];
             if (round == last_round) alloc_vals(total);
             ExpandArgs a = ea;
@@ -721,7 +794,7 @@
         if (!exo) wbuild->snapshot(wbits.p);
         publish_words(s, 0, DW_SPLIT_BYTES + 1);
         if (with_prologue) publish_prologue();
-        IPCFP_CUDA(cudaStreamSynchronize(st));
+        IPCFP_HOST_SYNC(st);
         if (with_prologue) read_prologue();
     }
 
@@ -750,7 +823,7 @@
                 if (ph->misc[64 + amt] > TX_KEY_EXACT_HEIGHT) {
                     k_amt_first_fault<<<1, 1, 0, st>>>(s->view, sa.txmeta_cids, amt, dw + DW_TX_ERR); IPCFP_LAUNCH_CHECK();
                     publish_words(s, DW_TX_ERR, 1);
-                    IPCFP_CUDA(cudaStreamSynchronize(st));
+                    IPCFP_HOST_SYNC(st);
                 }
             }
         }
@@ -768,7 +841,7 @@
         if (!exo) wbuild->start_copy(hw[DW_WIT_A], hw[DW_WIT_A_BYTES], hw[DW_SPLIT_IDX], hw[DW_SPLIT_BYTES]);
         if (xch && !xch_early) {
             xch->agree_slices(IPCFP_NO_ERROR, IPCFP_NO_ERROR, nraw);
-            if (!xch->peers_ok) { IPCFP_CUDA(cudaStreamSynchronize(st)); throw_first(xch->g_tx, xch->g_err); }
+            if (!xch->peers_ok) { IPCFP_HOST_SYNC(st); throw_first(xch->g_tx, xch->g_err); }
             xch->start_exchange(exec_raw.p);
         }
     }
@@ -792,7 +865,7 @@
         IPCFP_CUDA(cudaEventRecord(s->ev[EV_EXEC_ORDER], st));
         if (!exo) return true;
         publish_words(s, DW_N_EXEC, 1);
-        IPCFP_CUDA(cudaStreamSynchronize(st));
+        IPCFP_HOST_SYNC(st);
         exo->n_exec = hw[DW_N_EXEC];
         exo->nraw = nraw;
         exo->exec_raw = std::move(exec_raw);
@@ -815,10 +888,15 @@
         match_rel.alloc(N + 32, st);
         wp3.alloc((N + 31) / 32 + 8, st);
         bitmap_to_indices(match_bits.p, (N + 31) / 32 * 32, match_rel.p, (uint64_t*)(dw + DW_N_MATCH), wp3.p, scratch.p, st);
-        exclusive_scan_u32(cnt.p, pbase.p, N, (uint64_t*)(dw + DW_N_PROOFS), scratch.p, st);
-        exclusive_scan_u32(nby.p, bbase.p, N, (uint64_t*)(dw + DW_BLOB_BYTES), scratch.p, st);
+        k_match_offsets<<<1, MO_THREADS, 0, st>>>(match_rel.p, dw + DW_N_MATCH, cnt.p, nby.p, pbase.p, bbase.p, dw + DW_N_PROOFS, dw + DW_BLOB_BYTES);
+        IPCFP_LAUNCH_CHECK();
+        spec2 = !xch && !getenv("IPCFP_PASS2_PER_THREAD");
+        if (spec2) return;
         publish_words(s, 0, DW_TX_ERR + 1);
-        IPCFP_CUDA(cudaStreamSynchronize(st));
+        IPCFP_HOST_SYNC(st);
+        read_counts();
+    }
+    void read_counts() {
         note_errors();
         n_exec = hw[DW_N_EXEC];
         M = hw[DW_N_MATCH];
@@ -826,26 +904,55 @@
         n_proofs = hw[DW_N_PROOFS]; n_bytes = hw[DW_BLOB_BYTES];
     }
 
+    void launch_pass2(bool spec) {
+        if (!spec && !M) return;
+        Pass2ArgsT<P> p2;
+        p2.store = s->view; p2.store_dev = s->view_dev.p; p2.m_dev = d_matcher; p2.m = mh; p2.events_roots = td.events_roots.p; p2.lo = lo; p2.match_rel = match_rel.p; p2.n_match = M;
+        p2.receipts_root_blk = receipts_root_blk; p2.exec_cids = exec_raw.p; p2.exec_idx = exec_idx.p; p2.n_exec = n_exec_dev;
+        p2.wbits = wbits.p; p2.err = dw + DW_ERR; p2.cnt = cnt.p; p2.proof_base = pbase.p; p2.byte_base = bbase.p;
+        p2.proofs = proofs_dev; p2.blob = blob_dev; p2.any_skip = misc + 2; p2.resolve_msg = sharded ? 0 : 1;
+        if (spec) {
+            p2.per_warp = 1;
+            k_pass2_spec<<<PASS2_SPEC_CTAS, 128, 0, st>>>(p2, dw + DW_N_MATCH, dw + DW_N_PROOFS, dw + DW_BLOB_BYTES, s->p2_proofs.n - 1, s->p2_blob.n - 16,
+                                                        dw + DW_PASS2_OVERFLOW);
+        } else {
+            p2.per_warp = (M <= PASS2_WARP_MAX && !getenv("IPCFP_PASS2_PER_THREAD")) ? 1 : 0;
+            k_pass2<<<div_up(p2.per_warp ? M * 32 : M, 128), 128, 0, st>>>(p2);
+        }
+        IPCFP_LAUNCH_CHECK();
+    }
+    void late_witness_and_sync() {
+        wbuild->finish_enqueue(wbits.p);
+        publish_words(s, 0, DW_PASS2_OVERFLOW + 1);
+        publish_words(s, HW_ANY_SKIP, HW_ANY_SKIP_WORDS, misc);
+        IPCFP_HOST_SYNC(st);
+    }
     void pass2() {
         box.reset(new EventResultBox());
         memset(&box->r, 0, sizeof box->r);
-        d_proofs.alloc(n_proofs + 1, st);
-        d_blob.alloc(n_bytes + 16, st);
-        if (M) {
-            Pass2ArgsT<P> p2;
-            p2.store = s->view; p2.store_dev = s->view_dev.p; p2.m_dev = d_matcher; p2.m = mh; p2.events_roots = td.events_roots.p; p2.lo = lo; p2.match_rel = match_rel.p; p2.n_match = M;
-            p2.receipts_root_blk = receipts_root_blk; p2.exec_cids = exec_raw.p; p2.exec_idx = exec_idx.p; p2.n_exec = n_exec_dev;
-            p2.wbits = wbits.p; p2.err = dw + DW_ERR; p2.cnt = cnt.p; p2.proof_base = pbase.p; p2.byte_base = bbase.p;
-            p2.proofs = d_proofs.p; p2.blob = d_blob.p; p2.any_skip = misc + 2; p2.resolve_msg = sharded ? 0 : 1;
-            p2.per_warp = (M <= 16384 && !getenv("IPCFP_PASS2_PER_THREAD")) ? 1 : 0;
-            k_pass2<<<div_up(p2.per_warp ? M * 32 : M, 128), 128, 0, st>>>(p2); IPCFP_LAUNCH_CHECK();
-        }
-        if (xch) xch->positions_for(match_rel.p, M, n_exec_dev);
-        wbuild->finish_enqueue(wbits.p);
-        publish_words(s, 0, DW_EXEC_CHECK + 1);
-        publish_words(s, HW_ANY_SKIP, HW_ANY_SKIP_WORDS, misc);
-        IPCFP_CUDA(cudaStreamSynchronize(st));
-        note_errors();
+        if (spec2) {
+            if (!s->p2_proofs.p) { s->p2_proofs.alloc(4096 + 1); s->p2_blob.alloc((1u << 20) + 16); }
+            proofs_dev = s->p2_proofs.p; blob_dev = s->p2_blob.p;
+            launch_pass2(true);
+            late_witness_and_sync();
+            read_counts();
+            if (hw[DW_PASS2_OVERFLOW]) {
+                if (s->p2_proofs.n < n_proofs + 1) s->p2_proofs.alloc(n_proofs + n_proofs / 4 + 1);
+                if (s->p2_blob.n < n_bytes + 16) s->p2_blob.alloc(n_bytes + n_bytes / 4 + 16);
+                proofs_dev = s->p2_proofs.p; blob_dev = s->p2_blob.p;
+                launch_pass2(false);
+                late_witness_and_sync();
+                note_errors();
+            }
+        } else {
+            d_proofs.alloc(n_proofs + 1, st);
+            d_blob.alloc(n_bytes + 16, st);
+            proofs_dev = d_proofs.p; blob_dev = d_blob.p;
+            launch_pass2(false);
+            if (xch) xch->positions_for(match_rel.p, M, n_exec_dev);
+            late_witness_and_sync();
+            note_errors();
+        }
         if (!xch && missing_base && !skip_tx) throw_first(IPCFP_NO_ERROR, IPCFP_NO_ERROR, true);
         mB = hw[DW_WIT_B];
         any_skip = ((const uint32_t*)(hw + HW_ANY_SKIP))[2] != 0;
@@ -858,8 +965,8 @@
         box->blob = PinnedArray(s->pool, n_bytes + 16);
         rel = PinnedArray(s->pool, (M + 1) * 4);
         if (M) IPCFP_CUDA(cudaMemcpyAsync(rel.p, match_rel.p, M * 4, cudaMemcpyDeviceToHost, st));
-        if (n_proofs && !xch) IPCFP_CUDA(cudaMemcpyAsync(box->proofs.p, d_proofs.p, n_proofs * sizeof(ipcfp_event_proof), cudaMemcpyDeviceToHost, st));
-        if (n_bytes) IPCFP_CUDA(cudaMemcpyAsync(box->blob.p, d_blob.p, n_bytes, cudaMemcpyDeviceToHost, st));
+        if (n_proofs && !xch) IPCFP_CUDA(cudaMemcpyAsync(box->proofs.p, proofs_dev, n_proofs * sizeof(ipcfp_event_proof), cudaMemcpyDeviceToHost, st));
+        if (n_bytes) IPCFP_CUDA(cudaMemcpyAsync(box->blob.p, blob_dev, n_bytes, cudaMemcpyDeviceToHost, st));
         wbuild->finish_start(mB, hw[DW_WIT_B_BYTES], box->wit);
         if (xch) {
             if (!xch->agree_results(pend_tx, pend_err, missing_base && !skip_tx, n_proofs, hw[DW_WIT_A] + mB, xch_stale, exec_raw.p, nraw)) {
@@ -867,24 +974,28 @@
                 throw_first(xch->g_tx, xch->g_err, xch->g_missing_base);
                 throw Error(IPCFP_ERR_UNSUPPORTED, "execution-order exchange: bucket overflow (skewed CID hash distribution)");
             }
-            xch->fetch_and_patch(d_proofs.p, n_proofs, box->proofs.p);
+            xch->fetch_and_patch(proofs_dev, n_proofs, box->proofs.p);
             xch->witness_union(box->wit.cids_dev.p, box->wit.n, (flags & IPCFP_SHARDED_UNION_FULL) != 0);
         }
         if (flags & IPCFP_RESULT_JSON) {
             IPCFP_CUDA(cudaEventRecord(s->ev[EV_JSON_BEGIN], st));
-            JsonInputs ji{d_proofs.p, n_proofs, d_blob.p, box->wit.cids_dev.p, box->wit.idx_dev.p, box->wit.n,
+            JsonInputs ji{proofs_dev, n_proofs, blob_dev, box->wit.cids_dev.p, box->wit.idx_dev.p, box->wit.n,
                           td.parent_epoch, td.child_epoch, td.n_parents, sa.parent_cids, sa.child_cid};
             json_len = render_event_json(s, ji, box->json);
             IPCFP_CUDA(cudaEventRecord(s->ev[EV_JSON_END], st));
         }
-        wbuild->finish_join(box->wit);
-        if (xch) xch->finish();
+        if (xch) {
+            wbuild->finish_join(box->wit);
+            xch->finish();
+            IPCFP_CUDA(cudaEventRecord(s->ev[EV_END], st));
+            IPCFP_HOST_SYNC(st);
+        } else {
+            wbuild->finish_join(box->wit, s->ev[EV_END]);
+        }
     }
 
     ipcfp_event_result* fill() {
         static thread_local std::chrono::steady_clock::time_point t_last_exit = t_enter;
-        IPCFP_CUDA(cudaEventRecord(s->ev[EV_END], st));
-        IPCFP_CUDA(cudaStreamSynchronize(st));
         {
             uint64_t* mo = box->matching.as<uint64_t>();
             const uint32_t* rp = rel.as<uint32_t>();
@@ -932,7 +1043,7 @@
             if (flags & IPCFP_SHARDED_UNION_TO_HOST) {
                 box->union_host = PinnedArray(s->pool, r.n_union_part * 38 + 64);
                 if (r.n_union_part) IPCFP_CUDA(cudaMemcpyAsync(box->union_host.p, r.union_cids_dev, r.n_union_part * 38, cudaMemcpyDeviceToHost, st));
-                IPCFP_CUDA(cudaStreamSynchronize(st));
+                IPCFP_HOST_SYNC(st);
                 r.union_cids = box->union_host.as<uint8_t>();
             }
         }
diff --git a/ipc_filecoin_proofs_b200/csrc/witness.cu b/ipc_filecoin_proofs_b200/csrc/witness.cu
--- a/ipc_filecoin_proofs_b200/csrc/witness.cu
+++ b/ipc_filecoin_proofs_b200/csrc/witness.cu
@@ -84,26 +84,50 @@
     uint64_t i = (uint64_t)blockIdx.x * blockDim.x + threadIdx.x;
     if (i < m) out[i] = (lengths[bar[idx[i]]] + 15u) & ~15u;
 }
-__global__ void k_sum_padded_dev(const uint32_t* __restrict__ idx, const unsigned long long* __restrict__ count, uint64_t n_max, const uint32_t* __restrict__ lengths,
-                                 const uint32_t* __restrict__ bar, unsigned long long* out) {
-    uint64_t i = (uint64_t)blockIdx.x * blockDim.x + threadIdx.x;
-    unsigned long long v = (i < n_max && i < *count) ? (unsigned long long)((lengths[bar[idx[i]]] + 15u) & ~15u) : 0ull;
-#pragma unroll
-    for (int o = 16; o; o >>= 1) v += __shfl_down_sync(0xffffffffu, v, o);
-    if ((threadIdx.x & 31) == 0 && v) atomicAdd(out, v);
+#define LO_THREADS 1024
+#define LO_ITEMS 8
+__global__ void __launch_bounds__(LO_THREADS) k_late_offsets(const uint32_t* __restrict__ idx, const unsigned long long* count, const uint32_t* __restrict__ lengths,
+                                                             const uint32_t* __restrict__ bar, uint64_t* offs, unsigned long long* total) {
+    __shared__ uint64_t s_w[32], s_end;
+    const uint32_t t = threadIdx.x, lane = t & 31, warp = t >> 5;
+    const uint64_t m = *count;
+    uint64_t carry = 0;
+    for (uint64_t base = 0; base < m; base += LO_THREADS * LO_ITEMS) {
+        const uint64_t first = base + (uint64_t)t * LO_ITEMS;
+        uint32_t v[LO_ITEMS];
+        uint64_t sum = 0;
+#pragma unroll
+        for (int k = 0; k < LO_ITEMS; k++) { v[k] = first + k < m ? (lengths[bar[idx[first + k]]] + 15u) & ~15u : 0u; sum += v[k]; }
+        uint64_t x = sum;
+#pragma unroll
+        for (int o = 1; o < 32; o <<= 1) { const uint64_t y = __shfl_up_sync(0xffffffffu, x, o); if (lane >= (uint32_t)o) x += y; }
+        if (lane == 31) s_w[warp] = x;
+        __syncthreads();
+        if (warp == 0) {
+            const uint64_t a = s_w[lane];
+            uint64_t w = a;
+#pragma unroll
+            for (int o = 1; o < 32; o <<= 1) { const uint64_t y = __shfl_up_sync(0xffffffffu, w, o); if (lane >= (uint32_t)o) w += y; }
+            s_w[lane] = w - a;
+        }
+        __syncthreads();
+        uint64_t o = carry + s_w[warp] + x - sum;
+#pragma unroll
+        for (int k = 0; k < LO_ITEMS; k++) { if (first + k < m) offs[first + k] = o; o += v[k]; }
+        if (t == LO_THREADS - 1) s_end = o;
+        __syncthreads();
+        carry = s_end;
+        __syncthreads();
+    }
+    if (t == 0) *total = carry;
 }
 __global__ void k_andnot(const uint32_t* __restrict__ a, const uint32_t* __restrict__ b, uint32_t* out, uint64_t nwords) {
     uint64_t i = (uint64_t)blockIdx.x * blockDim.x + threadIdx.x;
     if (i < nwords) out[i] = a[i] & ~b[i];
 }
-__global__ void __launch_bounds__(256) k_witness_copy(const uint32_t* __restrict__ idx, uint64_t m, StoreView v, const uint64_t* __restrict__ offsets,
-                                                      uint8_t* out) {
-    uint64_t w = ((uint64_t)blockIdx.x * blockDim.x + threadIdx.x) >> 5;
-    uint32_t lane = threadIdx.x & 31;
-    if (w >= m) return;
+__device__ __forceinline__ void copy_block(const StoreView& v, uint32_t rank, uint8_t* dst, uint32_t lane) {
     uint32_t len;
-    const uint8_t* src = store_block(v, v.block_at_rank[idx[w]], len);
-    uint8_t* dst = out + offsets[w];
+    const uint8_t* src = store_block(v, v.block_at_rank[rank], len);
     if (((uintptr_t)src & 15) == 0) {
         uint32_t nv = (len + 15) >> 4;
         const uint4* s4 = (const uint4*)src;
@@ -113,6 +137,18 @@
         for (uint32_t i = lane; i < len; i += 32) dst[i] = src[i];
     }
 }
+__global__ void __launch_bounds__(256) k_witness_copy(const uint32_t* __restrict__ idx, uint64_t m, StoreView v, const uint64_t* __restrict__ offsets,
+                                                      uint8_t* out) {
+    const uint64_t w = ((uint64_t)blockIdx.x * blockDim.x + threadIdx.x) >> 5;
+    if (w < m) copy_block(v, idx[w], out + offsets[w], threadIdx.x & 31);
+}
+__global__ void __launch_bounds__(256) k_witness_copy_dev(const uint32_t* __restrict__ idx, const unsigned long long* count, const unsigned long long* bytes,
+                                                          uint64_t cap, StoreView v, const uint64_t* __restrict__ offsets, uint8_t* out) {
+    const uint64_t m = *count;
+    if (*bytes > cap) return;
+    for (uint64_t w = ((uint64_t)blockIdx.x * blockDim.x + threadIdx.x) >> 5; w < m; w += ((uint64_t)gridDim.x * blockDim.x) >> 5)
+        copy_block(v, idx[w], out + offsets[w], threadIdx.x & 31);
+}
 __device__ __forceinline__ uint32_t bits_below(const uint32_t* __restrict__ bits, const uint64_t* __restrict__ prefix, uint32_t r) {
     return (uint32_t)prefix[r >> 5] + (uint32_t)__popc(bits[r >> 5] & ((1u << (r & 31)) - 1u));
 }
@@ -121,9 +157,13 @@
                                                                uint64_t mA, uint64_t baseB, const uint32_t* __restrict__ bitsA,
                                                                const uint64_t* __restrict__ prefixA, const uint32_t* __restrict__ bitsB,
                                                                const uint64_t* __restrict__ prefixB, StoreView v, uint8_t* cids, uint64_t* out_offs,
-                                                               uint32_t* out_lens, uint32_t* out_idx, int by_ref) {
+                                                               uint32_t* out_lens, uint32_t* out_idx, int by_ref, const unsigned long long* mB_dev) {
     __shared__ uint16_t rec[EMIT_THREADS][19];
     __shared__ uint64_t pos[EMIT_THREADS];
+    if (mB_dev) {
+        if (mA + *mB_dev > m) return;
+        m = mA + *mB_dev;
+    }
     const uint64_t i = (uint64_t)blockIdx.x * blockDim.x + threadIdx.x;
     if (i < m) {
         const uint32_t r = idx[i];
@@ -221,9 +261,23 @@
     bitsB.alloc(nwords + 8, st);
     k_andnot<<<div_up(nwords ? nwords : 1, 256), 256, 0, st>>>(wbits, bitsA.p, bitsB.p, nwords); IPCFP_LAUNCH_CHECK();
     bitmap_to_indices(bitsB.p, s->n, idx.p + mA, (uint64_t*)(dw + DW_WIT_B), word_prefixB.p, scratch.p, st);
-    IPCFP_CUDA(cudaMemsetAsync(dw + DW_WIT_B_BYTES, 0, 8, st));
-    const uint64_t bound = s->n > mA ? s->n - mA : 0;
-    if (bound) { k_sum_padded_dev<<<div_up(bound, 256), 256, 0, st>>>(idx.p + mA, dw + DW_WIT_B, bound, s->lengths.p, s->block_at_rank.p, dw + DW_WIT_B_BYTES); IPCFP_LAUNCH_CHECK(); }
+    k_late_offsets<<<1, LO_THREADS, 0, st>>>(idx.p + mA, dw + DW_WIT_B, s->lengths.p, s->block_at_rank.p, offs.p + mA, dw + DW_WIT_B_BYTES);
+    IPCFP_LAUNCH_CHECK();
+    capB = by_ref ? 0 : host_cap - bytesA;
+    if (!by_ref) {
+        dblobB_keep.alloc(capB + 64, st);
+        k_witness_copy_dev<<<1024, 256, 0, st>>>(idx.p + mA, dw + DW_WIT_B, dw + DW_WIT_B_BYTES, capB, s->view, offs.p + mA, dblobB_keep.p);
+        IPCFP_LAUNCH_CHECK();
+    }
+    const uint64_t bound = mA + std::min<uint64_t>(s->n - mA, std::max<uint64_t>(mA / 8, 65536));
+    emit_cap = bound;
+    e_lens.alloc(bound + 8, st); e_idx.alloc(bound + 8, st); e_offs.alloc(bound + 8, st); e_cids.alloc(bound * 38 + 64, st);
+    if (bound) {
+        k_witness_emit<<<div_up(bound, EMIT_THREADS), EMIT_THREADS, 0, st>>>(idx.p, offs.p, bound, mA, bytesA, bitsA.p, word_prefix.p, bitsB.p, word_prefixB.p, s->view,
+                                                                           e_cids.p, e_offs.p, e_lens.p, e_idx.p, by_ref ? 1 : 0, dw + DW_WIT_B);
+        IPCFP_LAUNCH_CHECK();
+    }
+    late_done = true;
 }
 void WitnessBuilder::finish(uint64_t mB_, uint64_t bytesB_, WitnessOut& out, bool want_sorted_idx) {
     finish_start(mB_, bytesB_, out, want_sorted_idx);
@@ -235,30 +289,35 @@
     unsigned long long* dw = s->dev_words.p;
     uint64_t m = mA + mB;
     if (by_ref) { bytesB = 0; mB_ = 0; }
-    if (mB_) {
+    const bool gathered = late_done && bytesB <= capB;
+    const bool emitted = late_done && m <= emit_cap;
+    if (mB_ && !late_done) {
         k_padded_lengths<<<div_up(mB, 256), 256, 0, st>>>(idx.p + mA, mB, s->lengths.p, s->block_at_rank.p, plen.p); IPCFP_LAUNCH_CHECK();
         exclusive_scan_u32(plen.p, offs.p + mA, mB, (uint64_t*)(dw + DW_WIT_B_BYTES), scratch.p, st);
     }
     if (bytesA + bytesB > host_cap) {
-        IPCFP_CUDA(cudaStreamSynchronize(st2));
+        IPCFP_HOST_SYNC(st2);
         PinnedArray bigger(s->pool, bytesA + bytesB + 64);
         memcpy(bigger.p, host_blob.p, bytesA);
         host_blob = std::move(bigger);
         host_cap = host_blob.cap;
     }
-    AsyncBuf<uint8_t> dblobB(bytesB + 64, st);
-    if (mB_) {
-        k_witness_copy<<<div_up(mB * 32, 256), 256, 0, st>>>(idx.p + mA, mB, s->view, offs.p + mA, dblobB.p); IPCFP_LAUNCH_CHECK();
-        IPCFP_CUDA(cudaMemcpyAsync((uint8_t*)host_blob.p + bytesA, dblobB.p, bytesB, cudaMemcpyDeviceToHost, st));
-    }
-    AsyncBuf<uint32_t> d_lens(m + 8, st), d_idx(m + 8, st);
-    AsyncBuf<uint64_t> d_offs(m + 8, st);
-    AsyncBuf<uint8_t> d_cids(m * 38 + 64, st);
-    if (m) {
-        k_witness_emit<<<div_up(m, EMIT_THREADS), EMIT_THREADS, 0, st>>>(idx.p, offs.p, m, mA, bytesA, bitsA.p, word_prefix.p, bitsB.p, word_prefixB.p, s->view, d_cids.p, d_offs.p,
-                                                       d_lens.p, d_idx.p, by_ref ? 1 : 0);
-        IPCFP_LAUNCH_CHECK();
-    }
+    if (mB_ && !gathered) {
+        dblobB_keep.alloc(bytesB + 64, st);
+        k_witness_copy<<<div_up(mB * 32, 256), 256, 0, st>>>(idx.p + mA, mB, s->view, offs.p + mA, dblobB_keep.p); IPCFP_LAUNCH_CHECK();
+    }
+    if (mB_) IPCFP_CUDA(cudaMemcpyAsync((uint8_t*)host_blob.p + bytesA, dblobB_keep.p, bytesB, cudaMemcpyDeviceToHost, st));
+    if (!emitted) {
+        e_lens.alloc(m + 8, st); e_idx.alloc(m + 8, st); e_offs.alloc(m + 8, st); e_cids.alloc(m * 38 + 64, st);
+        if (m) {
+            k_witness_emit<<<div_up(m, EMIT_THREADS), EMIT_THREADS, 0, st>>>(idx.p, offs.p, m, mA, bytesA, bitsA.p, word_prefix.p, bitsB.p, word_prefixB.p, s->view,
+                                                                           e_cids.p, e_offs.p, e_lens.p, e_idx.p, by_ref ? 1 : 0, nullptr);
+            IPCFP_LAUNCH_CHECK();
+        }
+    }
+    AsyncBuf<uint32_t> d_lens = std::move(e_lens), d_idx = std::move(e_idx);
+    AsyncBuf<uint64_t> d_offs = std::move(e_offs);
+    AsyncBuf<uint8_t> d_cids = std::move(e_cids);
     IPCFP_CUDA(cudaEventRecord(s->ev[EV_WITNESS_SORTED], st));
     out.n = m;
     out.blob_size = bytesA + bytesB;
@@ -274,11 +333,11 @@
     }
     out.cids_dev = std::move(d_cids);
     out.idx_dev = std::move(d_idx);
-    dblobB_keep = std::move(dblobB);
-}
-void WitnessBuilder::finish_join(WitnessOut& out) {
+}
+void WitnessBuilder::finish_join(WitnessOut& out, cudaEvent_t end) {
     IPCFP_CUDA(cudaStreamWaitEvent(st, s->ev[EV_BLOB_COPIED], 0));
-    IPCFP_CUDA(cudaStreamSynchronize(st));
+    if (end) IPCFP_CUDA(cudaEventRecord(end, st));
+    IPCFP_HOST_SYNC(st);
     IPCFP_CUDA(cudaStreamSynchronize(st2));
     out.blob = std::move(host_blob);
 }
```

Measured after the change: 691.7 million, median of 6. 4.5% higher.
